# py-lidbox/lidbox

Hardware: AMD Instinct MI355X
Metric: utterances/sec (16kHz x 2s) log-mel + x-vector train step (higher is better)
Workload: dtype f32; 1 GPU; log-mel + x-vector 4-lang train step, bs=256 per GPU, fp32 (BASELINE configs[1]); reference_model=lidbox.models.xvector, global_batch=256, per_gpu_batch=256, samples_per_utt=32000, frames=198, mel=40, languages=4, optimizer=Adam(1e-3, eps=1e-7), parallelism=dp1, grad_buckets=1, grad_sync=none, hip_graph=True, resident_batches=4, feature_prefetch=False

## Files before the change

### include/lidbox_hip.h

```cpp
#ifndef LIDBOX_HIP_H
#define LIDBOX_HIP_H

#include <stddef.h>
#include <stdint.h>

#ifdef __cplusplus
extern "C" {
#endif

#define LIDBOX_HIP_ABI_VERSION 1

#define LIDBOX_OK            0
#define LIDBOX_E_INVALID    -1
#define LIDBOX_E_LAUNCH     -2
#define LIDBOX_E_ALLOC      -3

typedef void* lidbox_stream_t;
typedef struct lidbox_feat_plan lidbox_feat_plan;

int         lidbox_hip_abi_version(void);
const char* lidbox_hip_last_error(void);


int lidbox_ms_to_frames(int sample_rate, int ms);
// ... 6 lines not shown
int lidbox_hann_window(int window_length, float* out_host);


enum {
    LIDBOX_FEAT_SPECTROGRAM = 0,
    LIDBOX_FEAT_MEL         = 1,
    LIDBOX_FEAT_LOGMEL      = 2,
    LIDBOX_FEAT_MFCC        = 3
};

int  lidbox_feat_plan_create(int sample_rate, int frame_length, int frame_step, int fft_length,
                             float power, int num_mel_bins, float fmin, float fmax,
                             int coef_begin, int coef_end, lidbox_feat_plan** out_plan);
void lidbox_feat_plan_destroy(lidbox_feat_plan* plan);

int  lidbox_feat_plan_channels(const lidbox_feat_plan* plan, int kind);
int  lidbox_feat_plan_is_fused(const lidbox_feat_plan* plan, int kind, const float* signals,
                               long sig_stride);
size_t lidbox_extract_features_workspace(const lidbox_feat_plan* plan, int kind, int B, int N,
                                         const float* signals, long sig_stride);

int lidbox_extract_features_fwd(const lidbox_feat_plan* plan, int kind, const float* signals,
                                int B, int N, long sig_stride, float* out, long out_batch_stride,
                                void* workspace, size_t workspace_bytes, lidbox_stream_t stream);
int lidbox_extract_features_fwd_shadow(const lidbox_feat_plan* plan, int kind, const float* signals,
                                       int B, int N, long sig_stride, float* out, long out_batch_stride, void* out16,
                                       void* workspace, size_t workspace_bytes, lidbox_stream_t stream);

enum { LIDBOX_SRC_F32 = 0, LIDBOX_SRC_PCM16 = 1 };
int lidbox_extract_features_fwd_ex(const lidbox_feat_plan* plan, int kind, const void* signals, int src_format,
                                   int B, int N, long sig_stride, float* out, long out_batch_stride, void* out16,
                                   int* nonfinite, void* workspace, size_t workspace_bytes, lidbox_stream_t stream);
int lidbox_extract_features_fwd_pcm16(const lidbox_feat_plan* plan, int kind, const int16_t* pcm, int B, int N, long sig_stride,
                                      float* out, long out_batch_stride, int* nonfinite, lidbox_stream_t stream);


int lidbox_cmvn_fwd(const float* x, long outer, long R, long inner, int normalize_variance,
                    float* out, lidbox_stream_t stream);
int lidbox_cmvn_strided_fwd(const float* x, long outer, long R, long inner, long x_outer_stride,
                            int normalize_variance, float* out, long out_outer_stride, lidbox_stream_t stream);

int lidbox_window_norm_fwd(const float* x, int B, int T, int C, int window_len,
                           int normalize_variance, float* out, lidbox_stream_t stream);

int lidbox_minmax(const float* x, long n, float* out2, float* scratch, lidbox_stream_t stream);

int lidbox_feature_scaling_fwd(const float* x, long n, const float* minmax2, float lo, float hi,
                               float* out, lidbox_stream_t stream);
int lidbox_feature_scaling_axis_fwd(const float* x, long outer, long R, long inner, float lo, float hi, float* out,
                                    lidbox_stream_t stream);
int lidbox_log10_fwd(const float* x, long n, float* out, lidbox_stream_t stream);

int lidbox_power_to_db_fwd(const float* S, long n, const float* minmax2, float amin, float top_db,
                           float* out, lidbox_stream_t stream);


typedef struct {
    const float* base;
    long  batch_stride;
    long  row_stride;
    int   batch;
    int   rows_per_batch;
} lidbox_rows_t;

typedef struct {
    float* base;
    long  batch_stride;
    long  row_stride;
    int   batch;
    int   rows_per_batch;
} lidbox_rows_out_t;

enum {
    LIDBOX_EPI_NONE      = 0,
    LIDBOX_EPI_BIAS      = 1,
    LIDBOX_EPI_BIAS_RELU = 2,
    LIDBOX_EPI_RELU_MASK = 3,
    LIDBOX_EPI_ACCUM     = 4,
    LIDBOX_EPI_ACCUM_RELU_MASK = 5,
    LIDBOX_EPI_ACCUM_RELU = 6,
    LIDBOX_EPI_RELU      = 7,
    LIDBOX_EPI_MASK_BF16 = 0x100
};

int lidbox_gemm_plan_query(int kind, long M, int N, int K, size_t workspace_bytes, int* out4);

int lidbox_gemm_plan_waves(int kind, long M, int N, int K, size_t workspace_bytes);

int lidbox_gemm_plan_is_stream_k(int kind, long M, int N, int K, size_t workspace_bytes);

int lidbox_gemm_last_launches(int* out3);
int lidbox_gemm_last_family(void);
int lidbox_gemm_plan_stream_tail(int kind, long M, int N, int K, size_t workspace_bytes);

size_t lidbox_gemm_rows_workspace(long M, int N, int K);

int lidbox_gemm_nn(lidbox_rows_t A, const float* Bm, long ldb, lidbox_rows_out_t C,
                   int K, int N, int epilogue, const float* aux,
                   void* workspace, size_t workspace_bytes, lidbox_stream_t stream);

int lidbox_gemm_nt(lidbox_rows_t A, const float* Bm, long ldb, lidbox_rows_out_t C,
                   int K, int N, int epilogue, const float* aux,
                   void* workspace, size_t workspace_bytes, lidbox_stream_t stream);

size_t lidbox_gemm_tn_workspace(int M, int K1, int N);
int lidbox_gemm_tn(lidbox_rows_t A, lidbox_rows_t Bm, float* C, long ldc, int K1, int N,
                   int accumulate, float* bias_grad, void* workspace, size_t workspace_bytes,
                   lidbox_stream_t stream);

typedef struct lidbox_reduce_job {
    const float* partials;
    const float* bias_partials;
    float* C;
    float* bias_grad;
    long n, ldc;
    int splits, N, accumulate;
    unsigned nblocks;
} lidbox_reduce_job_t;
int lidbox_gemm_tn_partial(lidbox_rows_t A, lidbox_rows_t Bm, float* C, long ldc, int K1, int N, int accumulate,
                           float* bias_grad, void* workspace, size_t workspace_bytes, lidbox_reduce_job_t* job,
                           lidbox_stream_t stream);
int lidbox_gemm_nt_carry(lidbox_rows_t A, const float* Bm, long ldb, lidbox_rows_out_t C, int K, int N, int epilogue,
                         const float* aux, void* workspace, size_t workspace_bytes, const lidbox_reduce_job_t* jobs, int njobs,
                         lidbox_stream_t stream);
int lidbox_gemm_nt_tn_carry(lidbox_rows_t dY, const float* W, long ldb, lidbox_rows_out_t dX, int Co, int N, int epilogue,
                            const float* aux, void* ws_nt, size_t ws_nt_bytes, lidbox_rows_t X, float* dW, long ldc, int K1,
                            int accumulate, float* bias_grad, void* ws_tn, size_t ws_tn_bytes,
                            const lidbox_reduce_job_t* jobs, int njobs, lidbox_reduce_job_t* job_out, lidbox_stream_t stream);
int lidbox_reduce_jobs_run(const lidbox_reduce_job_t* jobs, int njobs, lidbox_stream_t stream);
int lidbox_gemm_last_carried(void);
int lidbox_zero_job(float* base, long batch_stride, long row_floats, int batch, lidbox_reduce_job_t* job);

int lidbox_gemm_plan_is_pair(long M, int Co, int N, int K1, size_t ws_nt_bytes, size_t ws_tn_bytes);
int lidbox_gemm_nt_tn(lidbox_rows_t dY, const float* W, long ldb, lidbox_rows_out_t dX, int Co, int N, int epilogue,
                      const float* aux, void* ws_nt, size_t ws_nt_bytes, lidbox_rows_t X, float* dW, long ldc, int K1,
                      int accumulate, float* bias_grad, void* ws_tn, size_t ws_tn_bytes, lidbox_stream_t stream);

size_t lidbox_gemm_bf16_rows_workspace(long M, int N, int K);
int lidbox_gemm_bf16_nn(lidbox_rows_t A, const float* Bm, long ldb, lidbox_rows_out_t C,
                        int K, int N, int epilogue, const float* aux,
                        void* workspace, size_t workspace_bytes, lidbox_stream_t stream);
int lidbox_gemm_bf16_nt(lidbox_rows_t A, const float* Bm, long ldb, lidbox_rows_out_t C,
                        int K, int N, int epilogue, const float* aux,
                        void* workspace, size_t workspace_bytes, lidbox_stream_t stream);
size_t lidbox_gemm_bf16_tn_workspace(int M, int K1, int N);
int lidbox_gemm_bf16_tn(lidbox_rows_t A, lidbox_rows_t Bm, float* C, long ldc, int K1, int N,
                        int accumulate, float* bias_grad, void* workspace, size_t workspace_bytes,
                        lidbox_stream_t stream);

int lidbox_gemm_bf16s_nt(lidbox_rows_t A16, const void* B16, long ldb, lidbox_rows_out_t C, void* C16,
                         int K, int N, int epilogue, const float* aux,
                         void* workspace, size_t workspace_bytes, lidbox_stream_t stream);
int lidbox_gemm_bf16s_last_variant(int* out3);
size_t lidbox_gemm_bf16s_tn_workspace(int M, int K1, int N);
int lidbox_gemm_bf16s_tn(lidbox_rows_t A16, lidbox_rows_t B16, float* C, long ldc, int K1, int N,
                         int accumulate, float* bias_grad, void* workspace, size_t workspace_bytes,
                         lidbox_stream_t stream);
int lidbox_gemm_bf16s_tn_partial(lidbox_rows_t A16, lidbox_rows_t B16, float* C, long ldc, int K1, int N, int accumulate,
                                 float* bias_grad, void* workspace, size_t workspace_bytes, lidbox_reduce_job_t* job,
                                 lidbox_stream_t stream);
int lidbox_gemm_bf16s_nt_carry(lidbox_rows_t A16, const void* B16, long ldb, lidbox_rows_out_t C, void* C16, int K, int N,
                               int epilogue, const float* aux, void* workspace, size_t workspace_bytes,
                               const lidbox_reduce_job_t* jobs, int njobs, lidbox_stream_t stream);
int lidbox_gemm_bf16s_last_carried(void);
int lidbox_gemm_bf16s_nt_pair_carry(lidbox_rows_t A16_0, const void* B16_0, long ldb0, lidbox_rows_out_t C0, void* C16_0, int K0, int N0,
                                    int epilogue0, const float* aux0, lidbox_rows_t A16_1, const void* B16_1, long ldb1,
// ... 255 lines not shown
```

### lidbox_amd/_native.py

```python
import ctypes as C
import os

import torch

_HERE = os.path.dirname(os.path.abspath(__file__))
LIB_PATH = os.environ.get("LIDBOX_HIP_LIB") or os.path.join(_HERE, "csrc", "liblidbox_hip.so")

ABI_VERSION = 1

FEAT_SPECTROGRAM, FEAT_MEL, FEAT_LOGMEL, FEAT_MFCC = 0, 1, 2, 3
SRC_F32, SRC_PCM16 = 0, 1
EPI_NONE, EPI_BIAS, EPI_BIAS_RELU, EPI_RELU_MASK, EPI_ACCUM, EPI_ACCUM_RELU_MASK, EPI_ACCUM_RELU, EPI_RELU = range(8)
EPI_MASK_BF16 = 0x100


class LidboxHipError(RuntimeError):
    pass


class Rows(C.Structure):
    _fields_ = [("base", C.c_void_p), ("batch_stride", C.c_long), ("row_stride", C.c_long),
                ("batch", C.c_int), ("rows_per_batch", C.c_int)]


class ReduceJob(C.Structure):
    _fields_ = [("partials", C.c_void_p), ("bias_partials", C.c_void_p), ("C", C.c_void_p), ("bias_grad", C.c_void_p),
                ("n", C.c_long), ("ldc", C.c_long), ("splits", C.c_int), ("N", C.c_int), ("accumulate", C.c_int),
                ("nblocks", C.c_uint)]


class WeightShadow(C.Structure):
    _fields_ = [("offset", C.c_long), ("rows", C.c_int), ("cols", C.c_int), ("dst", C.c_void_p), ("ld_dst", C.c_long),
                ("transpose", C.c_int)]


class Conv2DTaps(C.Structure):
    _fields_ = [("kt", C.c_int), ("kf", C.c_int), ("sf", C.c_int), ("pt0", C.c_int), ("pt1", C.c_int), ("pf0", C.c_int),
                ("pf1", C.c_int), ("time_first", C.c_int)]


def _load():
    if not os.path.exists(LIB_PATH):
        raise LidboxHipError(
            "liblidbox_hip.so not found at %s -- build it with `python -m lidbox_amd.build` "
            "(lidbox_amd has no CPU fallback)" % LIB_PATH)
    try:
        lib = C.CDLL(LIB_PATH)
    except OSError as e:
        raise LidboxHipError("cannot load %s: %s" % (LIB_PATH, e)) from e
    return lib


lib = _load()

_vp, _i, _l, _f, _sz = C.c_void_p, C.c_int, C.c_long, C.c_float, C.c_size_t

_SIGS = {
    "lidbox_hip_abi_version": (_i, []),
    "lidbox_hip_last_error": (C.c_char_p, []),
    "lidbox_ms_to_frames": (_i, [_i, _i]),
    "lidbox_num_frames": (_i, [_i, _i, _i]),
    "lidbox_mel_weight_matrix": (_i, [_i, _i, _i, _f, _f, _vp]),
    "lidbox_hann_window": (_i, [_i, _vp]),
    "lidbox_feat_plan_create": (_i, [_i, _i, _i, _i, _f, _i, _f, _f, _i, _i, C.POINTER(_vp)]),
    "lidbox_feat_plan_destroy": (None, [_vp]),
    "lidbox_feat_plan_channels": (_i, [_vp, _i]),
    "lidbox_feat_plan_is_fused": (_i, [_vp, _i, _vp, _l]),
    "lidbox_extract_features_workspace": (_sz, [_vp, _i, _i, _i, _vp, _l]),
    "lidbox_extract_features_fwd": (_i, [_vp, _i, _vp, _i, _i, _l, _vp, _l, _vp, _sz, _vp]),
    "lidbox_extract_features_fwd_shadow": (_i, [_vp, _i, _vp, _i, _i, _l, _vp, _l, _vp, _vp, _sz, _vp]),
    "lidbox_extract_features_fwd_ex": (_i, [_vp, _i, _vp, _i, _i, _i, _l, _vp, _l, _vp, _vp, _vp, _sz, _vp]),
    "lidbox_extract_features_fwd_pcm16": (_i, [_vp, _i, _vp, _i, _i, _l, _vp, _l, _vp, _vp]),
    "lidbox_cmvn_fwd": (_i, [_vp, _l, _l, _l, _i, _vp, _vp]),
    "lidbox_cmvn_strided_fwd": (_i, [_vp, _l, _l, _l, _l, _i, _vp, _l, _vp]),
    "lidbox_window_norm_fwd": (_i, [_vp, _i, _i, _i, _i, _i, _vp, _vp]),
    "lidbox_minmax": (_i, [_vp, _l, _vp, _vp, _vp]),
    "lidbox_feature_scaling_fwd": (_i, [_vp, _l, _vp, _f, _f, _vp, _vp]),
    "lidbox_feature_scaling_axis_fwd": (_i, [_vp, _l, _l, _l, _f, _f, _vp, _vp]),
    "lidbox_log10_fwd": (_i, [_vp, _l, _vp, _vp]),
    "lidbox_power_to_db_fwd": (_i, [_vp, _l, _vp, _f, _f, _vp, _vp]),
    "lidbox_gemm_plan_query": (_i, [_i, _l, _i, _i, _sz, _vp]),
    "lidbox_gemm_last_launches": (_i, [_vp]),
    "lidbox_gemm_last_family": (_i, []),
    "lidbox_gemm_bf16s_last_variant": (_i, [_vp]),
    "lidbox_gemm_plan_stream_tail": (_i, [_l, _i, _i, _i, _sz]),
    "lidbox_gemm_plan_waves": (_i, [_i, _l, _i, _i, _sz]),
    "lidbox_gemm_plan_is_stream_k": (_i, [_i, _l, _i, _i, _sz]),
    "lidbox_gemm_rows_workspace": (_sz, [_l, _i, _i]),
    "lidbox_gemm_nn": (_i, [Rows, _vp, _l, Rows, _i, _i, _i, _vp, _vp, _sz, _vp]),
    "lidbox_gemm_nt": (_i, [Rows, _vp, _l, Rows, _i, _i, _i, _vp, _vp, _sz, _vp]),
    "lidbox_gemm_tn_workspace": (_sz, [_i, _i, _i]),
    "lidbox_gemm_tn": (_i, [Rows, Rows, _vp, _l, _i, _i, _i, _vp, _vp, _sz, _vp]),
    "lidbox_gemm_plan_is_pair": (_i, [_l, _i, _i, _i, _sz, _sz]),
    "lidbox_gemm_nt_tn": (_i, [Rows, _vp, _l, Rows, _i, _i, _i, _vp, _vp, _sz, Rows, _vp, _l, _i, _i, _vp, _vp, _sz, _vp]),
    "lidbox_gemm_tn_partial": (_i, [Rows, Rows, _vp, _l, _i, _i, _i, _vp, _vp, _sz, C.POINTER(ReduceJob), _vp]),
    "lidbox_gemm_nt_carry": (_i, [Rows, _vp, _l, Rows, _i, _i, _i, _vp, _vp, _sz, C.POINTER(ReduceJob), _i, _vp]),
# ... 166 lines not shown
```

### lidbox_amd/csrc/gemm.hip

```cpp
#include <stdlib.h>

#include <atomic>

#include "gemm_shared.h"
#include "gemm_sk.h"
#include <string.h>
#include "gemm_dma.h"
#include "gemm_dma8.h"
#include "gemm_tuned.h"

namespace {

constexpr int BK = 16;
#define LBX_ROWS_BOUNDS(BM, BN) __launch_bounds__(256, ((BM) * (BN) >= 16384 ? 3 : ((BM) * (BN) >= 8192 ? 6 : 8)))
#define LBX_TN_BOUNDS(BM, BN) __launch_bounds__(256, ((BM) * (BN) >= 16384 ? 3 : 1))

template <int ROWS, bool ALIGNED, int NT = 256>
struct KInnerLoader {
    static constexpr int F4R = BK / 4;
    static constexpr int RPP = NT / F4R;
    static constexpr int PASSES = ROWS >= RPP ? ROWS / RPP : 1;
    static constexpr bool PARTIAL = ROWS < RPP;
    static constexpr int LD = ROWS + 8 / F4R;
    float4 v[PASSES];
// ... 546 lines not shown
    if (wgs > NUM_CU && wgs % NUM_CU != 0) {
        const double fluid = (double)wgs / NUM_CU + 0.12;
        if (fluid < per_cu) per_cu = fluid;
    }
    const double conc = per_cu < RESIDENT[c] ? (double)wgs / NUM_CU : (double)RESIDENT[c];
    return per_cu * tile_t / conc_eff(conc < 1.0 ? 1.0 : conc);
}

RowsChoice choose_rows(int kind, long M, int N, int K, size_t ws_bytes) {
    if (const TunedGemm* t = tuned_gemm(kind, M, N, K)) {
        const int kps = (int)(lbx_cdiv(lbx_cdiv(K, t->splits), BK) * BK);
        const int splits = (int)lbx_cdiv(K, kps);
        if (splits == 1 || (size_t)splits * M * N * sizeof(float) <= ws_bytes)
            return RowsChoice{t->bm, t->bn, splits, kps, t->no_tail_split != 0, (t->waves == 8 && t->bm == 128) ? 8 : 4};
    }
    RowsChoice best{128, 128, 1, K};
    double best_cost = 1e30;
    for (int c = 0; c < 4; ++c) {
        const int bm = CAND[c][0], bn = CAND[c][1];
        const long tiles = lbx_cdiv(M, bm) * lbx_cdiv(N, bn);
        for (int s = 1; s <= 64; s *= 2) {
            int kps = (int)(lbx_cdiv(lbx_cdiv(K, s), BK) * BK);
            const int splits = (int)lbx_cdiv(K, kps);
            if (s > 1 && (splits < 2 || kps < 4 * BK)) break;
            if (splits > 1 && (size_t)splits * M * N * sizeof(float) > ws_bytes) break;
            double cost = launch_cost(c, tiles * splits, (double)kps / BK);
            if (splits > 1) cost += 5.0 + (double)M * N * 4.0 * (splits + 1) / 3.0e6;
            if (cost < best_cost) { best_cost = cost; best = RowsChoice{bm, bn, splits, kps}; }
            if (splits < s) break;
        }
    }
    return best;
}

RowsChoice choose_rows_env(int kind, long M, int N, int K, size_t wsb) {
    RowsChoice ch = choose_rows(kind, M, N, K, wsb);
    if (M >= 4096) {
        if (const char* f = getenv(kind == 1 ? "LIDBOX_GEMM_NT8" : "LIDBOX_GEMM_NN8")) {
            const int bn = atoi(f);
            if (bn == 64 || bn == 128) return RowsChoice{128, bn, 1, K, false, 8};
        }
    }
    if (const char* f = getenv("LIDBOX_GEMM_PLAN")) {
        int bm = 0, bn = 0, sp = 0, wv = 4;
        if (sscanf(f, "%d,%d,%d,%d", &bm, &bn, &sp, &wv) >= 3 && (bm == 64 || bm == 128) && (bn == 64 || bn == 128) && sp >= 1) {
            const int kps = (int)(lbx_cdiv(lbx_cdiv(K, sp), BK) * BK);
            const int splits = (int)lbx_cdiv(K, kps);
            if (splits == 1 || (size_t)splits * M * N * sizeof(float) <= wsb)
                ch = RowsChoice{bm, bn, splits, kps, false, (wv == 8 && bm == 128) ? 8 : 4};
        }
    }
    return ch;
}

template <int BM, int BN, bool B_KINNER>
void launch_rows8_t(bool al, dim3 grid, hipStream_t st, RowsD Ad, const float* Bm, long ldb, RowsOutD Co, float* P,
                    long m_beg, long m_end, int K, int N, int epi, const float* aux, int tiles_n, unsigned ntiles, int kps) {
    if (al)
        hipLaunchKernelGGL((gemm_rows8_kernel<BM, BN, B_KINNER, true>), grid, dim3(512), 0, st, Ad, Bm, ldb, Co, P, m_beg,
                           m_end, K, N, epi, aux, tiles_n, ntiles, kps);
    else
        hipLaunchKernelGGL((gemm_rows8_kernel<BM, BN, B_KINNER, false>), grid, dim3(512), 0, st, Ad, Bm, ldb, Co, P, m_beg,
                           m_end, K, N, epi, aux, tiles_n, ntiles, kps);
}

template <int BM, int BN, bool B_KINNER>
void launch_rows_t(bool al, dim3 grid, hipStream_t st, RowsD Ad, const float* Bm, long ldb, RowsOutD Co, float* P,
                   long m_beg, long m_end, int K, int N, int epi, const float* aux, int tiles_n, unsigned ntiles, int kps) {
    if (al)
        hipLaunchKernelGGL((gemm_rows_kernel<BM, BN, B_KINNER, true>), grid, dim3(256), 0, st, Ad, Bm, ldb, Co, P, m_beg,
                           m_end, K, N, epi, aux, tiles_n, ntiles, kps);
    else
        hipLaunchKernelGGL((gemm_rows_kernel<BM, BN, B_KINNER, false>), grid, dim3(256), 0, st, Ad, Bm, ldb, Co, P, m_beg,
                           m_end, K, N, epi, aux, tiles_n, ntiles, kps);
}

inline int dma_mode() {
    if (const char* e = getenv("LIDBOX_GEMM_DMA")) return atoi(e);
    return 1;
}

template <int BM, int BN, bool B_KINNER>
void launch_rows_dma_t(dim3 grid, hipStream_t st, RowsD Ad, const float* Bm, long ldb, RowsOutD Co, float* P, long m_beg, long m_end,
                       int K, int N, int epi, const float* aux, int tiles_n, unsigned ntiles, int kps, const DmaStream& sp, const ReduceJobs& rj) {
    hipLaunchKernelGGL((gemm_rows_dma_kernel<BM, BN, B_KINNER>), grid, dim3(256), 0, st, Ad, Bm, ldb, Co, P, m_beg, m_end, K, N, epi,
                       aux, tiles_n, ntiles, kps, sp, rj);
}

inline long carry_cap() {
    if (const char* e = getenv("LIDBOX_GEMM_CARRY_BLOCKS")) { const long v = atol(e); if (v >= 8) return v; }
    return 96;
}
struct Carry {
    const ReduceJob* jobs = nullptr;
    int njobs = 0;
    bool carried = false;
};

constexpr int DMA_STREAM_MIN_STEPS = 8;
constexpr int DMA_STREAM_MAX_G = 8;
struct DmaStreamPlan {
    int g = 0;
    long whole = 0, rem = 0;
    size_t ws_need = 0;
};
inline DmaStreamPlan dma_stream_plan(int bm, int bn, long M, int N, int K) {
    DmaStreamPlan pl;
    int force = -1;
    if (const char* e = getenv("LIDBOX_GEMM_STREAM_TAIL")) force = atoi(e);
    if (force == 0) return pl;
    const long tiles = lbx_cdiv(M, bm) * lbx_cdiv(N, bn);
    const long rem = tiles % NUM_CU;
    if (tiles < NUM_CU || rem == 0) return pl;
    const int nk = (int)lbx_cdiv(K, SK_BK);
    int best = 1;
    double best_cost = 1.0;
    for (int g = 2; g <= DMA_STREAM_MAX_G && nk / g >= DMA_STREAM_MIN_STEPS; ++g) {
        const double cost = (double)lbx_cdiv(rem * g, (long)NUM_CU) / g + 0.03 + 0.01 * g;
        if (cost < best_cost - 1e-9) { best_cost = cost; best = g; }
    }
    if (force > 1 && nk / force >= 2 && force <= 64) best = force;
    else if (best_cost > 0.9) return pl;
    if (best < 2) return pl;
    pl.g = best; pl.rem = rem; pl.whole = tiles - rem;
    pl.ws_need = SK_COUNTER_BYTES + (size_t)rem * best * bm * bn * sizeof(float);
    return pl;
}

template <bool B_KINNER>
int launch_rows_range(const RowsChoice& ch, bool al, RowsD Ad, const float* Bm, long ldb, RowsOutD Co, long m_beg,
                      long m_end, int K, int N, int epi, const float* aux, float* P, hipStream_t st, bool dma_ok = false,
                      const DmaStreamPlan* stream = nullptr, void* ws = nullptr, Carry* carry = nullptr) {
    const long Msub = m_end - m_beg;
    if (Msub <= 0) return LIDBOX_OK;
    const int tiles_n = (int)lbx_cdiv(N, ch.bn);
    const long ntiles = lbx_cdiv(Msub, ch.bm) * tiles_n;
    dim3 grid((unsigned)ntiles, (unsigned)ch.splits);
    if (g_last_launches[0] == 0) { g_first_tile[0] = ch.bm; g_first_tile[1] = ch.bn; }
    ++g_last_launches[(ch.bm == g_first_tile[0] && ch.bn == g_first_tile[1]) ? 0 : 1];
    if (ch.splits > 1) ++g_last_launches[2];
#define LBX_ROWS(BM_, BN_) launch_rows_t<BM_, BN_, B_KINNER>(al, grid, st, Ad, Bm, ldb, Co, P, m_beg, m_end, K, N, epi, aux, tiles_n, (unsigned)ntiles, ch.k_per_split)
#define LBX_ROWS8(BM_, BN_) launch_rows8_t<BM_, BN_, B_KINNER>(al, grid, st, Ad, Bm, ldb, Co, P, m_beg, m_end, K, N, epi, aux, tiles_n, (unsigned)ntiles, ch.k_per_split)
#define LBX_ROWS_DMA(BM_, BN_) launch_rows_dma_t<BM_, BN_, B_KINNER>(grid, st, Ad, Bm, ldb, Co, P, m_beg, m_end, K, N, epi, aux, tiles_n, ntiles_k, ch.k_per_split, sp, rj)
    if (dma_ok && al && dma_mode() != 0) {
        g_last_family = 1;
        DmaStream sp;
        const bool dma8 = ch.waves == 8 && ch.bm == 128;
        ReduceJobs rj;
        if (carry && !carry->carried && carry->njobs > 0) {
            rj = pack_carry(carry->jobs, carry->njobs, carry_cap());
            carry->carried = rj.total > 0;
        }
        unsigned ntiles_k = (unsigned)ntiles;
        if (stream && stream->g > 1 && ch.splits == 1) {
            sp.pieces = (unsigned)(stream->rem * stream->g);
            sp.npad = (sp.pieces + 7u) & ~7u;
            sp.g = stream->g;
            sp.first_tile = (unsigned)stream->whole;
            sp.epoch = sk_next_epoch();
            sp.counters = (unsigned*)ws;
            sp.slabs = (float*)((char*)ws + SK_COUNTER_BYTES);
            ntiles_k = (unsigned)stream->whole;
            grid.x = sp.npad + ntiles_k;
        }
        grid.x += rj.total;
        if (dma8) {
            g_last_family = 3;
            if (ch.bn == 128)
                hipLaunchKernelGGL((gemm_rows_dma8_kernel<128, B_KINNER>), grid, dim3(512), 0, st, Ad, Bm, ldb, Co, P, m_beg, m_end, K, N, epi, aux, tiles_n,
                                   ntiles_k, ch.k_per_split, sp, rj);
            else
                hipLaunchKernelGGL((gemm_rows_dma8_kernel<64, B_KINNER>), grid, dim3(512), 0, st, Ad, Bm, ldb, Co, P, m_beg, m_end, K, N, epi, aux, tiles_n,
                                   ntiles_k, ch.k_per_split, sp, rj);
        } else
        if (ch.bm == 128 && ch.bn == 128) LBX_ROWS_DMA(128, 128);
        else if (ch.bm == 128) LBX_ROWS_DMA(128, 64);
        else if (ch.bn == 128) LBX_ROWS_DMA(64, 128);
        else LBX_ROWS_DMA(64, 64);
    } else
    if (ch.waves == 8 && ch.bm == 128 && ch.bn == 128) LBX_ROWS8(128, 128);
    else if (ch.waves == 8 && ch.bm == 128 && ch.bn == 64) LBX_ROWS8(128, 64);
    else if (ch.bm == 128 && ch.bn == 128) LBX_ROWS(128, 128);
    else if (ch.bm == 128) LBX_ROWS(128, 64);
    else if (ch.bn == 128) LBX_ROWS(64, 128);
    else LBX_ROWS(64, 64);
#undef LBX_ROWS
#undef LBX_ROWS8
    LBX_LAUNCH_OK();
    if (ch.splits > 1) {
        long g = lbx_cdiv(Msub * N, 256);
        if (g > 2048) g = 2048;
        hipLaunchKernelGGL(rows_reduce_kernel, dim3((unsigned)g), dim3(256), 0, st, (const float*)P, ch.splits, m_beg,
                           Msub, N, Co, epi, aux);
        LBX_LAUNCH_OK();
    }
    return LIDBOX_OK;
}

inline int cand_index(int bm, int bn) { return bm == 128 ? (bn == 128 ? 0 : 1) : (bn == 128 ? 2 : 3); }

template <bool B_KINNER>
int launch_rows(lidbox_rows_t A, const float* Bm, long ldb, lidbox_rows_out_t Cd, int K, int N, int epi,
                const float* aux, void* ws, size_t ws_bytes, hipStream_t st, Carry* carry = nullptr) {
    const long M = (long)A.batch * A.rows_per_batch;
    g_last_launches[0] = g_last_launches[1] = g_last_launches[2] = 0;
    g_last_family = 0;
    if (M == 0 || N == 0) return LIDBOX_OK;
    const size_t wsb = ws ? ws_bytes : 0;
    const RowsChoice ch = choose_rows_env(B_KINNER ? 1 : 0, M, N, K, wsb);
    const bool al = rows_aligned(A) && K % 4 == 0 && aligned16(Bm) && ldb % 4 == 0 &&
                    (B_KINNER ? true : N % 4 == 0);
    RowsD Ad = to_dev(A);
    RowsOutD Co{Cd.base, Cd.batch_stride, Cd.row_stride, Cd.batch, Cd.rows_per_batch};
    float* P = (float*)ws;

    if (al && !getenv("LIDBOX_GEMM_PLAN") && aligned16(ws) && !sk_tuned_out(B_KINNER ? 1 : 0, M, N, K) &&
        sk_b_extent_ok(B_KINNER, K, N, ldb)) {
        const bool has_mask_ = epi == LIDBOX_EPI_RELU_MASK || epi == LIDBOX_EPI_ACCUM_RELU_MASK;
        const bool skp_ok = skp_mode() != 0 && (Cd.batch == 1 || Cd.rows_per_batch >= 32) && N % 4 == 0 && aligned16(Cd.base) &&
                            Cd.row_stride % 4 == 0 && (Cd.batch == 1 || Cd.batch_stride % 4 == 0) && (!has_mask_ || aligned16(aux)) &&
                            skp_policy(B_KINNER ? 1 : 0, M, N, K);
        if (skp_ok) {
            const SkRows sk = sk_rows_plan(B_KINNER ? 1 : 0, M, N, K, true);
            if (sk.ok && wsb >= sk.ws_need && sk_extent_ok(A, K)) {
                sk_set_lds_attr();
                g_last_launches[0] = 1;
                g_last_family = 2;
                g_first_tile[0] = SK_BM; g_first_tile[1] = SK_BN;
                unsigned* counters = (unsigned*)ws;
                float* slabs = (float*)((char*)ws + SK_COUNTER_BYTES);
                float* dummy = slabs + (size_t)sk.P * 2 * SK_SLAB;
                const bool has_mask = epi == LIDBOX_EPI_RELU_MASK || epi == LIDBOX_EPI_ACCUM_RELU_MASK;
                const bool accum = epi == LIDBOX_EPI_ACCUM || epi == LIDBOX_EPI_ACCUM_RELU_MASK || epi == LIDBOX_EPI_ACCUM_RELU;
                const unsigned ep = sk_next_epoch();
#define LBX_SKP(MASK_, ACC_)                                                                                                \
    hipLaunchKernelGGL((gemm_skp_rows_kernel<B_KINNER, MASK_, ACC_>), dim3(sk.P), dim3(256), (MASK_ || ACC_) ? SKP_LDS_BYTES : SK_LDS_BYTES, st, Ad, Bm, ldb, Co, M, K, \
                       N, epi, aux, sk.pl, ep, counters, slabs, dummy)
                if (has_mask && accum) LBX_SKP(true, true);
                else if (has_mask) LBX_SKP(true, false);
                else if (accum) LBX_SKP(false, true);
                else LBX_SKP(false, false);
#undef LBX_SKP
                LBX_LAUNCH_OK();
                return LIDBOX_OK;
            }
        }
        const SkRows sk = sk_rows_plan(B_KINNER ? 1 : 0, M, N, K);
        if (sk.ok && wsb >= sk.ws_need && sk_extent_ok(A, K)) {
            sk_set_lds_attr();
            g_last_launches[0] = 1;
            g_last_family = 2;
            g_first_tile[0] = SK_BM; g_first_tile[1] = SK_BN;
            unsigned* counters = (unsigned*)ws;
            float* slabs = (float*)((char*)ws + SK_COUNTER_BYTES);
            hipLaunchKernelGGL((gemm_sk_rows_kernel<B_KINNER>), dim3(sk.P), dim3(256), SK_LDS_BYTES, st, Ad, Bm, ldb, Co, M, K, N, epi,
                               aux, sk.pl, sk_next_epoch(), counters, slabs);
            LBX_LAUNCH_OK();
            return LIDBOX_OK;
        }
    }

    const bool dma_ok = al && sk_extent_ok(A, K) && sk_b_extent_ok(B_KINNER, K, N, ldb);
    if (dma_ok && dma_mode() != 0 && ch.splits == 1 && aligned16(ws)) {
        const DmaStreamPlan spl = dma_stream_plan(ch.bm, ch.bn, M, N, K);
        if (spl.g > 1 && wsb >= spl.ws_need)
            return launch_rows_range<B_KINNER>(ch, al, Ad, Bm, ldb, Co, 0, M, K, N, epi, aux, P, st, dma_ok, &spl, ws, carry);
    }
    const bool no_tail_split = ch.no_tail_split || getenv("LIDBOX_GEMM_NO_TAIL_SPLIT") != nullptr;
    if (!no_tail_split && ch.splits == 1) {
        const int tiles_n = (int)lbx_cdiv(N, ch.bn);
        const long tiles_m = lbx_cdiv(M, ch.bm);
        const long wgs = tiles_m * tiles_n;
        const long rounds = wgs / NUM_CU;
        if (rounds >= 1 && wgs % NUM_CU != 0) {
            const long main_tiles_m = rounds * NUM_CU / tiles_n;
            const long m_main = main_tiles_m * ch.bm;
            const long m_rem = M - m_main;
            if (main_tiles_m >= 1 && m_rem > 0) {
                const RowsChoice rem = choose_rows(B_KINNER ? 1 : 0, m_rem, N, K, wsb);
                const int c = cand_index(ch.bm, ch.bn), cr = cand_index(rem.bm, rem.bn);
                const double ksteps = (double)lbx_cdiv(K, BK);
                const double whole = launch_cost(c, wgs, ksteps);
                double split = launch_cost(c, main_tiles_m * tiles_n, ksteps) + 4.0 +
                               launch_cost(cr, lbx_cdiv(m_rem, rem.bm) * lbx_cdiv(N, rem.bn) * rem.splits,
                                           (double)rem.k_per_split / BK);
                if (rem.splits > 1) split += 5.0 + (double)m_rem * N * 4.0 * (rem.splits + 1) / 3.0e6;
                if (split < 0.97 * whole) {
                    int rc = launch_rows_range<B_KINNER>(ch, al, Ad, Bm, ldb, Co, 0, m_main, K, N, epi, aux, P, st, dma_ok, nullptr, nullptr, carry);
                    if (rc) return rc;
                    return launch_rows_range<B_KINNER>(rem, al, Ad, Bm, ldb, Co, m_main, M, K, N, epi, aux, P, st, dma_ok);
                }
            }
        }
    }
    return launch_rows_range<B_KINNER>(ch, al, Ad, Bm, ldb, Co, 0, M, K, N, epi, aux, P, st, dma_ok, nullptr, nullptr, carry);
}

struct TnPlan {
    int bm, bn, splits;
    long rows_per_split;
};

TnPlan tn_plan(long M, int K1, int N) {
    if (const char* f = getenv("LIDBOX_GEMM_TN_PLAN")) {
        int bm = 0, bn = 0;
        long sp = 0;
        if (sscanf(f, "%d,%d,%ld", &bm, &bn, &sp) == 3 && (bm == 64 || bm == 128) && (bn == 64 || bn == 128) && sp >= 1) {
            const long rps = lbx_cdiv(lbx_cdiv(M, sp), BK) * BK;
            return TnPlan{bm, bn, (int)lbx_cdiv(M, rps), rps};
        }
    }
    if (const TunedGemm* t = tuned_gemm(2, M, N, K1)) {
        const long rps = lbx_cdiv(lbx_cdiv(M, (long)t->splits), BK) * BK;
        return TnPlan{t->bm, t->bn, (int)lbx_cdiv(M, rps), rps};
    }
    TnPlan best{128, 128, 1, M};
    double best_cost = 1e30;
    for (int c = 0; c < 4; ++c) {
        const int bm = CAND[c][0], bn = CAND[c][1];
        const long tiles = lbx_cdiv(K1, bm) * lbx_cdiv(N, bn);
        for (long target = NUM_CU; target <= 8 * NUM_CU; target += NUM_CU / 2) {
            long s = target / tiles;
            if (s < 1) s = 1;
            const long max_s = lbx_cdiv(M, 4 * BK);
            if (s > max_s) s = max_s;
            if (s < 1) s = 1;
            long rps = lbx_cdiv(lbx_cdiv(M, s), BK) * BK;
            s = lbx_cdiv(M, rps);
            double cost = launch_cost(c, tiles * s, (double)rps / BK);
            cost += 5.0 + (double)K1 * N * 4.0 * (s + 1) / 3.0e6;
            if (cost < best_cost) { best_cost = cost; best = TnPlan{bm, bn, (int)s, rps}; }
        }
    }
    return best;
}

template <int BM, int BN>
void launch_tn_t(bool al, unsigned grid, hipStream_t st, RowsD A, RowsD Bd, float* P, float* Pc, long M, int K1, int N,
                 int tiles_n, int ntiles, long rps) {
    if (al)
        hipLaunchKernelGGL((gemm_tn_kernel<BM, BN, true>), dim3(grid), dim3(256), 0, st, A, Bd, P, Pc, M, K1, N, tiles_n,
                           ntiles, rps);
    else
        hipLaunchKernelGGL((gemm_tn_kernel<BM, BN, false>), dim3(grid), dim3(256), 0, st, A, Bd, P, Pc, M, K1, N, tiles_n,
                           ntiles, rps);
}

}

extern "C" int lidbox_gemm_plan_query(int kind, long M, int N, int K, size_t workspace_bytes, int* out4) {
    LBX_ARG(out4 && M > 0 && N > 0 && K > 0 && kind >= 0 && kind <= 2, "kind in {0 nn, 1 nt, 2 tn}, positive sizes");
    if (kind == 2) {
        const TnPlan pl = tn_plan(M, K, N);
        out4[0] = pl.bm; out4[1] = pl.bn; out4[2] = pl.splits; out4[3] = (int)pl.rows_per_split;
    } else {
        const RowsChoice ch = choose_rows_env(kind, M, N, K, workspace_bytes);
        out4[0] = ch.bm; out4[1] = ch.bn; out4[2] = ch.splits; out4[3] = ch.k_per_split;
    }
    return LIDBOX_OK;
}

extern "C" int lidbox_gemm_plan_is_stream_k(int kind, long M, int N, int K, size_t workspace_bytes) {
    if (M <= 0 || N <= 0 || K <= 0 || kind < 0 || kind > 2) return 0;
    if (kind == 2) {
        const SkTn t = sk_tn_plan(M, K, N);
        return t.ok && workspace_bytes >= t.ws_need && !sk_tuned_out(2, M, N, K);
    }
    {
        const SkRows r = sk_rows_plan(kind, M, N, K);
        return r.ok && workspace_bytes >= r.ws_need && (kind == 1 || N % 4 == 0) && !sk_tuned_out(kind, M, N, K);
    }
    return LIDBOX_OK;
}

extern "C" int lidbox_gemm_plan_waves(int kind, long M, int N, int K, size_t workspace_bytes) {
    if (M <= 0 || N <= 0 || K <= 0 || kind < 0 || kind > 1) return 4;
    return choose_rows_env(kind, M, N, K, workspace_bytes).waves;
}

extern "C" int lidbox_gemm_last_family(void) { return g_last_family; }

extern "C" int lidbox_gemm_plan_stream_tail(int kind, long M, int N, int K, size_t workspace_bytes) {
    if (M <= 0 || N <= 0 || K <= 0 || kind < 0 || kind > 1 || dma_mode() == 0) return 0;
    if (!getenv("LIDBOX_GEMM_PLAN") && lidbox_gemm_plan_is_stream_k(kind, M, N, K, workspace_bytes)) return 0;
    const RowsChoice ch = choose_rows_env(kind, M, N, K, workspace_bytes);
    if (ch.splits != 1) return 0;
    const DmaStreamPlan spl = dma_stream_plan(ch.bm, ch.bn, M, N, K);
    return (spl.g > 1 && workspace_bytes >= spl.ws_need) ? spl.g : 0;
}

extern "C" int lidbox_gemm_last_launches(int* out3) {
    LBX_ARG(out3, "out3 != NULL");
    out3[0] = g_last_launches[0]; out3[1] = g_last_launches[1]; out3[2] = g_last_launches[2];
    return LIDBOX_OK;
}

extern "C" size_t lidbox_gemm_rows_workspace(long M, int N, int K) {
    if (M <= 0 || N <= 0 || K <= 0) return 0;
    size_t need = 0;
    for (int kind = 0; kind < 2; ++kind) {
        const RowsChoice ch = choose_rows(kind, M, N, K, (size_t)64 << 20);
        if (ch.splits > 1 && (size_t)ch.splits * M * N * sizeof(float) > need) need = (size_t)ch.splits * M * N * sizeof(float);
    }
    for (int bm = 64; bm <= 128; bm += 64)
        for (int bn = 64; bn <= 128; bn += 64) {
            const DmaStreamPlan spl = dma_stream_plan(bm, bn, M, N, K);
            if (spl.g > 1 && spl.ws_need > need) need = spl.ws_need;
        }
    for (int kind = 0; kind < 2; ++kind) {
        const SkRows sk = sk_rows_plan(kind, M, N, K);
        if (sk.ok && sk.ws_need > need) need = sk.ws_need;
        if (skp_mode() != 0 && skp_policy(kind, M, N, K)) {
            const SkRows skp = sk_rows_plan(kind, M, N, K, true);
            if (skp.ok && skp.ws_need > need) need = skp.ws_need;
        }
    }
    return need;
}

extern "C" int lidbox_gemm_nn(lidbox_rows_t A, const float* Bm, long ldb, lidbox_rows_out_t C, int K, int N,
                              int epilogue, const float* aux, void* workspace, size_t workspace_bytes,
                              lidbox_stream_t stream) {
    if (validate_rows_call(__func__, A, Bm, ldb, C, K, N, epilogue, aux, N)) return LIDBOX_E_INVALID;
    return launch_rows<false>(A, Bm, ldb, C, K, N, epilogue, aux, workspace, workspace_bytes, (hipStream_t)stream);
}


extern "C" int lidbox_gemm_nt(lidbox_rows_t A, const float* Bm, long ldb, lidbox_rows_out_t C, int K, int N,
                              int epilogue, const float* aux, void* workspace, size_t workspace_bytes,
                              lidbox_stream_t stream) {
    if (validate_rows_call(__func__, A, Bm, ldb, C, K, N, epilogue, aux, K)) return LIDBOX_E_INVALID;
    return launch_rows<true>(A, Bm, ldb, C, K, N, epilogue, aux, workspace, workspace_bytes, (hipStream_t)stream);
}

extern "C" size_t lidbox_gemm_tn_workspace(int M, int K1, int N) {
    if (M <= 0 || K1 <= 0 || N <= 0) return 0;
    const TnPlan pl = tn_plan(M, K1, N);
    size_t need = ((size_t)pl.splits * K1 * N + (size_t)pl.splits * N) * sizeof(float);
    const SkTn sk = sk_tn_plan(M, K1, N);
    if (sk.ok && sk.ws_need > need) need = sk.ws_need;
    return need;
}

namespace {

int tn_partial_launch(const char* fn, lidbox_rows_t A, lidbox_rows_t Bd, float* Cm, long ldc, int K1, int N, int accumulate,
                      float* bias_grad, void* workspace, size_t workspace_bytes, hipStream_t st, ReduceJob* job) {
    *job = ReduceJob{};
    if (check_rows(fn, A.base, A.batch_stride, A.row_stride, A.batch, A.rows_per_batch)) return LIDBOX_E_INVALID;
    if (check_rows(fn, Bd.base, Bd.batch_stride, Bd.row_stride, Bd.batch, Bd.rows_per_batch)) return LIDBOX_E_INVALID;
    LBX_ARG(Cm && K1 >= 1 && N >= 1 && ldc >= N, "C != NULL, K1, N >= 1, ldc >= N");
    const long M = (long)A.batch * A.rows_per_batch;
    LBX_ARG(M == (long)Bd.batch * Bd.rows_per_batch, "A and B row counts differ");
    LBX_ARG(M >= 1, "M >= 1");
    auto finish = [&](const float* P, const float* Pc, int splits) {
        const long n = (long)K1 * N;
        if (reduce_job_vec_ok(P, Pc, splits, n, N, Cm, ldc, bias_grad)) *job = make_reduce_job(P, Pc, splits, n, N, Cm, ldc, accumulate, bias_grad);
        else launch_splitk_reduce(P, Pc, splits, n, N, Cm, ldc, accumulate, bias_grad, st);
    };
    {
        const SkTn sk = sk_tn_plan(M, K1, N);
        if (sk.ok && !getenv("LIDBOX_GEMM_TN_PLAN") && !sk_tuned_out(2, M, N, K1) && workspace && aligned16(workspace) && workspace_bytes >= sk.ws_need &&
            rows_aligned(A) && rows_aligned(Bd) && sk_extent_ok(A, K1) && sk_extent_ok(Bd, N)) {
            sk_set_lds_attr();
            g_last_launches[0] = 1; g_last_launches[1] = 0; g_last_launches[2] = 1;
            g_last_family = 2;
            float* P = (float*)workspace;
            float* Pc = bias_grad ? P + (size_t)sk.splits * K1 * N : nullptr;
            hipLaunchKernelGGL(gemm_sk_tn_kernel, dim3((unsigned)(sk.ntiles * sk.splits)), dim3(256), SK_LDS_BYTES, st, to_dev(A),
                               to_dev(Bd), P, Pc, M, K1, N, sk.tiles_n, sk.ntiles, sk.rows_per_split);
            LBX_LAUNCH_OK();
            finish(P, Pc, sk.splits);
            LBX_LAUNCH_OK();
            return LIDBOX_OK;
        }
    }
    const TnPlan pl = tn_plan(M, K1, N);
    const size_t need = ((size_t)pl.splits * K1 * N + (size_t)pl.splits * N) * sizeof(float);
    LBX_ARG(workspace && workspace_bytes >= need, "workspace too small (lidbox_gemm_tn_workspace)");
    g_last_launches[0] = 1; g_last_launches[1] = 0; g_last_launches[2] = 1;
    g_last_family = 0;
    const int tiles_n = (int)lbx_cdiv(N, pl.bn);
    const int ntiles = (int)(lbx_cdiv(K1, pl.bm) * tiles_n);
    const bool al = rows_aligned(A) && rows_aligned(Bd) && K1 % 4 == 0 && N % 4 == 0;
    float* P = (float*)workspace;
    float* Pc = bias_grad ? P + (size_t)pl.splits * K1 * N : nullptr;
    const unsigned grid = (unsigned)(ntiles * pl.splits);
    if (al && dma_mode() != 0 && sk_extent_ok(A, K1) && sk_extent_ok(Bd, N) && pl.rows_per_split % SK_BK == 0) {
        g_last_family = 1;
#define LBX_TN_DMA(BM_, BN_) hipLaunchKernelGGL((gemm_tn_dma_kernel<BM_, BN_>), dim3(grid), dim3(256), 0, st, to_dev(A), to_dev(Bd), P, Pc, M, K1, N, tiles_n, ntiles, pl.rows_per_split)
        if (pl.bm == 128 && pl.bn == 128) LBX_TN_DMA(128, 128);
        else if (pl.bm == 128) LBX_TN_DMA(128, 64);
        else if (pl.bn == 128) LBX_TN_DMA(64, 128);
        else LBX_TN_DMA(64, 64);
#undef LBX_TN_DMA
        LBX_LAUNCH_OK();
        finish(P, Pc, pl.splits);
        LBX_LAUNCH_OK();
        return LIDBOX_OK;
    }
#define LBX_TN(BM_, BN_) launch_tn_t<BM_, BN_>(al, grid, st, to_dev(A), to_dev(Bd), P, Pc, M, K1, N, tiles_n, ntiles, pl.rows_per_split)
    if (pl.bm == 128 && pl.bn == 128) LBX_TN(128, 128);
    else if (pl.bm == 128) LBX_TN(128, 64);
    else if (pl.bn == 128) LBX_TN(64, 128);
    else LBX_TN(64, 64);
#undef LBX_TN
    LBX_LAUNCH_OK();
    finish(P, Pc, pl.splits);
    LBX_LAUNCH_OK();
    return LIDBOX_OK;
}

static_assert(sizeof(lidbox_reduce_job_t) == sizeof(ReduceJob), "lidbox_reduce_job_t mirrors ReduceJob");
inline ReduceJob job_in(const lidbox_reduce_job_t* j) {
    ReduceJob r;
    if (j) memcpy(&r, j, sizeof r);
    return r;
}
inline int jobs_in(const lidbox_reduce_job_t* jobs, int njobs, ReduceJob (&out)[MAX_CARRY]) {
    int m = 0;
    for (int i = 0; jobs && i < njobs; ++i) {
        if (jobs[i].nblocks == 0) continue;
        if (m == MAX_CARRY) return -1;
        out[m++] = job_in(jobs + i);
    }
    return m;
}

int run_reduce_jobs(const ReduceJob* jobs, int njobs, hipStream_t st) {
    ReduceJobs js;
    for (int i = 0, m = 0; i < njobs && m < MAX_CARRY; ++i) {
        if (jobs[i].nblocks == 0) continue;
        js.j[m++] = jobs[i];
        js.total += jobs[i].nblocks;
    }
    if (js.total == 0) return LIDBOX_OK;
    hipLaunchKernelGGL(splitk_reduce4_kernel, dim3(js.total), dim3(256), 0, st, js);
    LBX_LAUNCH_OK();
    return LIDBOX_OK;
}

}

extern "C" int lidbox_gemm_tn(lidbox_rows_t A, lidbox_rows_t Bd, float* Cm, long ldc, int K1, int N,
                              int accumulate, float* bias_grad, void* workspace, size_t workspace_bytes,
                              lidbox_stream_t stream) {
    ReduceJob job;
    int rc = tn_partial_launch(__func__, A, Bd, Cm, ldc, K1, N, accumulate, bias_grad, workspace, workspace_bytes, (hipStream_t)stream, &job);
    if (rc) return rc;
    return run_reduce_jobs(&job, 1, (hipStream_t)stream);
}

extern "C" int lidbox_gemm_tn_partial(lidbox_rows_t A, lidbox_rows_t Bd, float* Cm, long ldc, int K1, int N, int accumulate,
                                      float* bias_grad, void* workspace, size_t workspace_bytes, lidbox_reduce_job_t* job,
                                      lidbox_stream_t stream) {
    LBX_ARG(job, "job != NULL");
    ReduceJob j;
    int rc = tn_partial_launch(__func__, A, Bd, Cm, ldc, K1, N, accumulate, bias_grad, workspace, workspace_bytes, (hipStream_t)stream, &j);
    memcpy(job, &j, sizeof j);
    return rc;
}

extern "C" int lidbox_zero_job(float* base, long batch_stride, long row_floats, int batch, lidbox_reduce_job_t* job) {
    LBX_ARG(job && base && batch >= 1 && row_floats >= 4 && batch_stride >= row_floats, "base, job != NULL; batch >= 1; row_floats >= 4");
    LBX_ARG(aligned16(base) && row_floats % 4 == 0 && batch_stride % 4 == 0 && row_floats <= 0x7fffffffL,
            "16-byte aligned base, row_floats and batch_stride multiples of 4");
    ReduceJob j;
    j.Cm = base; j.n = (long)batch * row_floats; j.N = (int)row_floats; j.ldc = batch_stride; j.splits = 0; j.accumulate = 0;
    long g = lbx_cdiv(j.n / 4, 256);
    if (g > 2048) g = 2048;
    j.nblocks = (unsigned)g;
    memcpy(job, &j, sizeof j);
    return LIDBOX_OK;
}

extern "C" int lidbox_reduce_jobs_run(const lidbox_reduce_job_t* jobs, int njobs, lidbox_stream_t stream) {
    LBX_ARG(njobs >= 0 && (jobs || njobs == 0), "jobs != NULL");
    ReduceJob js[MAX_CARRY];
    const int m = jobs_in(jobs, njobs, js);
    LBX_ARG(m >= 0, "at most 2 non-empty jobs per call");
    return run_reduce_jobs(js, m, (hipStream_t)stream);
}

extern "C" int lidbox_gemm_nt_carry(lidbox_rows_t A, const float* Bm, long ldb, lidbox_rows_out_t C, int K, int N, int epilogue,
                                    const float* aux, void* workspace, size_t workspace_bytes, const lidbox_reduce_job_t* jobs,
                                    int njobs, lidbox_stream_t stream) {
    if (validate_rows_call(__func__, A, Bm, ldb, C, K, N, epilogue, aux, K)) return LIDBOX_E_INVALID;
    ReduceJob js[MAX_CARRY];
    const int m = jobs_in(jobs, njobs, js);
    LBX_ARG(m >= 0, "at most 2 non-empty jobs per call");
    for (int i = 0; i < m; ++i) LBX_ARG(js[i].splits >= 0, "an optimizer-prepare job runs through lidbox_reduce_jobs_run only");
    for (int i = 0; i < m; ++i) LBX_ARG((const void*)js[i].P != workspace, "a job's slices live in this call's workspace");
    Carry carry;
    carry.jobs = js;
    carry.njobs = (m > 0 && getenv("LIDBOX_GEMM_NO_CARRY") == nullptr) ? m : 0;
    int rc = launch_rows<true>(A, Bm, ldb, C, K, N, epilogue, aux, workspace, workspace_bytes, (hipStream_t)stream, &carry);
    if (rc) return rc;
    g_last_carried = carry.carried ? m : 0;
    if (!carry.carried) return run_reduce_jobs(js, m, (hipStream_t)stream);
    return LIDBOX_OK;
}

extern "C" int lidbox_gemm_last_carried(void) { return g_last_carried; }

inline long pair_max_blocks() {
    if (const char* e = getenv("LIDBOX_GEMM_PAIR_MAX_BLOCKS")) return atol(e);
    return 12L * NUM_CU;
}

bool pair_plan(long M, int Co, int N, int K1, size_t ws_nt_bytes, size_t ws_tn_bytes, RowsChoice* ch_out, TnPlan* pl_out) {
    if (dma_mode() == 0 || getenv("LIDBOX_GEMM_NO_PAIR") != nullptr || M < 1 || N < 1 || K1 < 1 || Co < 1) return false;
    if (Co % 4 != 0 || K1 % 4 != 0) return false;
    const RowsChoice ch = choose_rows_env(1, M, N, Co, ws_nt_bytes);
    const TnPlan pl = tn_plan(M, K1, Co);
    const SkTn sk = sk_tn_plan(M, K1, Co);
    const bool sk_rows = !getenv("LIDBOX_GEMM_PLAN") && lidbox_gemm_plan_is_stream_k(1, M, N, Co, ws_nt_bytes);
    const bool sk_tn = sk.ok && !getenv("LIDBOX_GEMM_TN_PLAN") && !sk_tuned_out(2, M, Co, K1) && ws_tn_bytes >= sk.ws_need;
    const size_t tn_need = ((size_t)pl.splits * K1 * Co + (size_t)pl.splits * Co) * sizeof(float);
    const long rows_blocks = lbx_cdiv(M, 64L) * lbx_cdiv((long)N, 64L) * ch.splits;
    const long tn_blocks = lbx_cdiv((long)K1, 64L) * lbx_cdiv((long)Co, 64L) * pl.splits;
    if (!(ch.bm == 64 && ch.bn == 64 && ch.waves == 4 && pl.bm == 64 && pl.bn == 64 && !sk_rows && !sk_tn && ws_tn_bytes >= tn_need &&
          (ch.splits == 1 || (size_t)ch.splits * M * N * sizeof(float) <= ws_nt_bytes) && rows_blocks + tn_blocks <= pair_max_blocks()))
        return false;
    if (ch_out) *ch_out = ch;
    if (pl_out) *pl_out = pl;
    return true;
}

extern "C" int lidbox_gemm_nt_tn_carry(lidbox_rows_t dY, const float* W, long ldb, lidbox_rows_out_t dX, int Co, int N, int epilogue,
                                       const float* aux, void* ws_nt, size_t ws_nt_bytes, lidbox_rows_t X, float* dW, long ldc, int K1,
                                       int accumulate, float* bias_grad, void* ws_tn, size_t ws_tn_bytes,
                                       const lidbox_reduce_job_t* jobs, int njobs, lidbox_reduce_job_t* job_out, lidbox_stream_t stream) {
    hipStream_t st = (hipStream_t)stream;
    if (job_out) memset(job_out, 0, sizeof *job_out);
    ReduceJob pend[MAX_CARRY];
    const int npend = jobs_in(jobs, njobs, pend);
    LBX_ARG(npend >= 0 && npend < MAX_CARRY, "at most 1 non-empty pending job per call");
    for (int i = 0; i < npend; ++i)
        LBX_ARG((const void*)pend[i].P != ws_nt && (const void*)pend[i].P != ws_tn, "a pending job's slices live in this call's workspaces");
    for (int i = 0; i < npend; ++i) LBX_ARG(pend[i].splits >= 0, "an optimizer-prepare job runs through lidbox_reduce_jobs_run only");
    const long M = (long)dY.batch * dY.rows_per_batch;
    bool pair = dma_mode() != 0 && getenv("LIDBOX_GEMM_NO_PAIR") == nullptr && M >= 1 && N >= 1 && K1 >= 1 && Co >= 1 && W && dW && ws_tn &&
                ws_nt != ws_tn;
    if (pair) {
        if (validate_rows_call(__func__, dY, W, ldb, dX, Co, N, epilogue, aux, Co)) return LIDBOX_E_INVALID;
        if (check_rows(__func__, X.base, X.batch_stride, X.row_stride, X.batch, X.rows_per_batch)) return LIDBOX_E_INVALID;
        LBX_ARG((long)X.batch * X.rows_per_batch == M && ldc >= Co, "X and dY row counts differ, or ldc < Co");
    }
    RowsChoice ch{};
    TnPlan pl{};
    if (pair) {
        const size_t wsb = ws_nt ? ws_nt_bytes : 0;
        const bool al_rows = rows_aligned(dY) && aligned16(W) && ldb % 4 == 0 && sk_extent_ok(dY, Co) && sk_b_extent_ok(true, Co, N, ldb) &&
                             aligned16(ws_nt);
        const bool al_tn = rows_aligned(X) && sk_extent_ok(X, K1) && aligned16(ws_tn);
        pair = al_rows && al_tn && pair_plan(M, Co, N, K1, wsb, ws_tn_bytes, &ch, &pl);
    }
    if (!pair) {
        lidbox_reduce_job_t all[MAX_CARRY];
        for (int i = 0; i < npend; ++i) memcpy(&all[i], &pend[i], sizeof(ReduceJob));
        int rc = lidbox_gemm_tn_partial(X, dY, dW, ldc, K1, Co, accumulate, bias_grad, ws_tn, ws_tn_bytes, &all[npend], stream);
        if (rc) return rc;
        if (ws_nt == ws_tn) {
            rc = lidbox_reduce_jobs_run(all, npend + 1, stream);
            if (rc) return rc;
            return lidbox_gemm_nt(dY, W, ldb, dX, Co, N, epilogue, aux, ws_nt, ws_nt_bytes, stream);
        }
        return lidbox_gemm_nt_carry(dY, W, ldb, dX, Co, N, epilogue, aux, ws_nt, ws_nt_bytes, all, npend + 1, stream);
    }
    PairRows r;
    r.A = to_dev(dY); r.Bm = W; r.ldb = ldb;
    r.Cd = RowsOutD{dX.base, dX.batch_stride, dX.row_stride, dX.batch, dX.rows_per_batch};
    r.P = (float*)ws_nt; r.M = M; r.K = Co; r.N = N; r.epi = epilogue; r.aux = aux;
    r.tiles_n = (int)lbx_cdiv((long)N, 64L);
    r.ntiles = (unsigned)(lbx_cdiv(M, 64L) * r.tiles_n);
    r.k_per_split = ch.k_per_split; r.nx = r.ntiles; r.partial = ch.splits > 1 ? 1 : 0;
    if (ch.splits == 1 && ws_nt) {
        const DmaStreamPlan spl = dma_stream_plan(64, 64, M, N, Co);
        if (spl.g > 1 && ws_nt_bytes >= spl.ws_need) {
            r.sp.pieces = (unsigned)(spl.rem * spl.g);
            r.sp.npad = (r.sp.pieces + 7u) & ~7u;
            r.sp.g = spl.g;
            r.sp.first_tile = (unsigned)spl.whole;
            r.sp.epoch = sk_next_epoch();
            r.sp.counters = (unsigned*)ws_nt;
            r.sp.slabs = (float*)((char*)ws_nt + SK_COUNTER_BYTES);
            r.ntiles = (unsigned)spl.whole;
            r.nx = r.sp.npad + r.ntiles;
        }
    }
    PairTn t;
    t.A = to_dev(X); t.Bd = to_dev(dY);
    t.P = (float*)ws_tn; t.Pc = bias_grad ? t.P + (size_t)pl.splits * K1 * Co : nullptr;
    t.M = M; t.K1 = K1; t.N = Co; t.tiles_n = (int)lbx_cdiv((long)Co, 64L);
    t.ntiles = (int)(lbx_cdiv((long)K1, 64L) * t.tiles_n);
    t.rows_per_split = pl.rows_per_split;
    const unsigned rows_blocks = r.nx * (unsigned)ch.splits;
    ReduceJobs rj;
    if (npend > 0 && getenv("LIDBOX_GEMM_NO_CARRY") == nullptr) rj = pack_carry(pend, npend, carry_cap());
    const unsigned grid = rj.total + rows_blocks + (unsigned)(t.ntiles * pl.splits);
    g_last_launches[0] = 1; g_last_launches[1] = 0; g_last_launches[2] = (job_out ? 0 : 1) + (ch.splits > 1 ? 1 : 0);
    g_last_family = 1;
    g_last_carried = rj.total > 0 ? npend : 0;
    hipLaunchKernelGGL(gemm_nt_tn_pair_kernel, dim3(grid), dim3(256), 0, st, r, t, rows_blocks, rj);
    LBX_LAUNCH_OK();
    if (npend > 0 && rj.total == 0) {
        int rc = run_reduce_jobs(pend, npend, st);
        if (rc) return rc;
    }
    if (ch.splits > 1) {
        long g = lbx_cdiv(M * N, 256);
        if (g > 2048) g = 2048;
        hipLaunchKernelGGL(rows_reduce_kernel, dim3((unsigned)g), dim3(256), 0, st, (const float*)r.P, ch.splits, 0L, M, N, r.Cd, epilogue,
                           aux);
        LBX_LAUNCH_OK();
    }
    if (job_out && reduce_job_vec_ok(t.P, t.Pc, pl.splits, (long)K1 * Co, Co, dW, ldc, bias_grad)) {
// ... 47 lines not shown
```

### lidbox_amd/csrc/gemm_dma.h

```cpp
#pragma once

#include "gemm_sk.h"

namespace {

constexpr int DMA_STAGES = 3;

template <int ROWS>
struct DmaInner {
    static constexpr int PW = ROWS / 64;
    const float* sb;
    unsigned vo[PW];
    int rd;
    __device__ __forceinline__ void init(const float* base, const long (&roff)[PW], int k0, int lane, int wsub) {
        sb = sk_uniform(base + k0);
        const int chunk = (lane & 3) ^ ((lane >> 4) & 3);
#pragma unroll
        for (int i = 0; i < PW; ++i) vo[i] = (unsigned)((roff[i] + chunk * 4) * 4);
        rd = (wsub * (ROWS / 2) + (lane & 31)) * 16;
    }
    __device__ __forceinline__ void issue(int i, unsigned dst) const { sk_dma_s(sb, vo[i], dst); }
    __device__ __forceinline__ void issue_tail(int i, unsigned dst, int kvalid, int lane) const {
        const int chunk = (lane & 3) ^ ((lane >> 4) & 3);
        const float* p = reinterpret_cast<const float*>(reinterpret_cast<const char*>(sb) + vo[i]);
// ... 21 lines not shown
    long step;
    int rd;
    __device__ __forceinline__ void init(const float* base, long ld, int col0, int ncols, int k0, int lane, int wv, int wsub) {
        sb = sk_uniform(base + (long)k0 * ld + col0);
        int c = (lane % LPR) * 4;
        if (col0 + c >= ncols) c = 0;
#pragma unroll
        for (int i = 0; i < PW; ++i) vo[i] = (unsigned)(((long)(RPP * (wv * PW + i) + lane / LPR) * ld + c) * 4);
        step = (long)SK_BK * ld;
        rd = (4 * (lane >> 5)) * COLS + wsub * (COLS / 2) + (lane & 31);
    }
    __device__ __forceinline__ void issue(int i, unsigned dst) const { sk_dma_s(sb, vo[i], dst); }
    __device__ __forceinline__ void issue_tail(int i, unsigned dst, int kvalid, int lane, int wv) const {
        const float* p = reinterpret_cast<const float*>(reinterpret_cast<const char*>(sb) + vo[i]);
        sk_dma_f(RPP * (wv * PW + i) + lane / LPR < kvalid ? p : g_sk_zero, dst);
    }
    __device__ __forceinline__ void advance() { sb += step; }
    template <int NB>
    __device__ __forceinline__ void read(const float* st, int lane, int s2, float (&v)[NB][4]) const {
#pragma unroll
        for (int b = 0; b < NB; ++b)
#pragma unroll
            for (int j = 0; j < 4; ++j) v[b][j] = st[rd + (8 * s2 + j) * COLS + b * 32];
    }
};

template <int MI, int NJ, int J0, int J1>
__device__ __forceinline__ void dma_mma(const float (&a)[MI][4], const float (&b)[NJ][4], f32x16 (&acc)[MI][NJ]) {
#pragma unroll
    for (int j = J0; j < J1; ++j)
#pragma unroll
        for (int bi = 0; bi < MI; ++bi)
#pragma unroll
            for (int bj = 0; bj < NJ; ++bj)
                acc[bi][bj] = __builtin_amdgcn_mfma_f32_32x32x2f32(a[bi][j], b[bj][j], acc[bi][bj], 0, 0, 0);
}

struct DmaStream {
    unsigned npad = 0;
    unsigned pieces = 0;
    int g = 1;
    unsigned first_tile = 0;
    unsigned epoch = 0;
    unsigned* counters = nullptr;
    float* slabs = nullptr;
};

template <int MI, int NJ>
__device__ __forceinline__ void dma_slab_store(float* slab, const f32x16 (&acc)[MI][NJ], int wv, int lane) {
    const __amdgpu_buffer_rsrc_t r = __builtin_amdgcn_make_buffer_rsrc(const_cast<float*>(sk_uniform(slab)), 0, MI * NJ * 4096 * 4, 0x00020000);
#pragma unroll
    for (int bi = 0; bi < MI; ++bi)
#pragma unroll
        for (int bj = 0; bj < NJ; ++bj)
#pragma unroll
            for (int r4 = 0; r4 < 4; ++r4) {
                const f32x4_t x = {acc[bi][bj][4 * r4], acc[bi][bj][4 * r4 + 1], acc[bi][bj][4 * r4 + 2], acc[bi][bj][4 * r4 + 3]};
                __builtin_amdgcn_raw_buffer_store_b128(__builtin_bit_cast(u32x4_t, x), r,
                                                       ((((wv * (MI * NJ) + bi * NJ + bj) * 4 + r4) * 64 + lane) * 4) * 4, 0,  16);
            }
}
template <int MI, int NJ>
__device__ __forceinline__ void dma_slab_add(const float* slab, f32x16 (&acc)[MI][NJ], int wv, int lane) {
    const __amdgpu_buffer_rsrc_t r = __builtin_amdgcn_make_buffer_rsrc(const_cast<float*>(sk_uniform(slab)), 0, MI * NJ * 4096 * 4, 0x00020000);
#pragma unroll
    for (int bi = 0; bi < MI; ++bi)
#pragma unroll
        for (int bj = 0; bj < NJ; ++bj) {
#pragma unroll
            for (int r4 = 0; r4 < 4; ++r4) {
                const f32x4_t x = __builtin_bit_cast(
                    f32x4_t, __builtin_amdgcn_raw_buffer_load_b128(r, ((((wv * (MI * NJ) + bi * NJ + bj) * 4 + r4) * 64 + lane) * 4) * 4, 0,  16));
#pragma unroll
                for (int j = 0; j < 4; ++j) acc[bi][bj][4 * r4 + j] += x[j];
            }
            __builtin_amdgcn_sched_barrier(0);
        }
}

template <int BM, int BN, bool B_KINNER>
__device__ __forceinline__ void rows_dma_body(const RowsD& A, const float* __restrict__ Bm, long ldb, const RowsOutD& Cd, float* __restrict__ P,
                                              long m_beg, long M, int K, int N, int epi, const float* __restrict__ aux, int tiles_n,
                                              unsigned ntiles, int k_per_split, const DmaStream& sp, unsigned bx, unsigned by, int partial,
                                              float* smem) {
    constexpr int MI = BM / 64, NJ = BN / 64;
    constexpr int A_ST = BM * SK_BK, B_ST = SK_BK * BN, ST = A_ST + B_ST;
    constexpr int PA = BM / 64, PB = BN / 64;

    const int tid = threadIdx.x, lane = tid & 63;
    const int wv = __builtin_amdgcn_readfirstlane(tid >> 6);
    const int wm = wv >> 1, wn = wv & 1;
    const unsigned lds0 = __builtin_amdgcn_readfirstlane((unsigned)(size_t)(__attribute__((address_space(3))) void*)smem);
    const int split = (int)by;
    unsigned chunk;
    int kbeg, kend, part = -1;
    unsigned rem_t = 0;
    if (bx < sp.npad) {
        if (bx >= sp.pieces) return;
        rem_t = bx / (unsigned)sp.g;
        part = (int)(bx - rem_t * (unsigned)sp.g);
        chunk = sp.first_tile + rem_t;
        const int nk = (K + SK_BK - 1) / SK_BK;
        kbeg = (part * nk / sp.g) * SK_BK;
        kend = min(K, ((part + 1) * nk / sp.g) * SK_BK);
    } else {
        chunk = xcd_chunk_id(bx - sp.npad, ntiles);
        kbeg = split * k_per_split;
        kend = min(K, kbeg + k_per_split);
    }
    const int tn = chunk % tiles_n;
    const long m0 = m_beg + (long)(chunk / tiles_n) * BM;
    const int n0 = tn * BN;
    const int n = (kend - kbeg + SK_BK - 1) / SK_BK;
    const int ktail = kend - kbeg - (n - 1) * SK_BK;

    DmaInner<BM> oa;
    {
        long roff[PA];
#pragma unroll
        for (int i = 0; i < PA; ++i) {
            long r = m0 + 16 * (wv * PA + i) + (lane >> 2);
            if (r >= M) r = m0;
            roff[i] = row_offset(A, (unsigned)r);
        }
        oa.init(A.base, roff, kbeg, lane, wm);
    }
    DmaInner<BN> obi;
    DmaOuter<BN> obo;
    if (B_KINNER) {
        long roff[PB];
#pragma unroll
        for (int i = 0; i < PB; ++i) {
            long r = n0 + 16 * (wv * PB + i) + (lane >> 2);
            if (r >= N) r = n0;
            roff[i] = r * ldb;
        }
        obi.init(Bm, roff, kbeg, lane, wn);
    } else {
        obo.init(Bm, ldb, n0, N, kbeg, lane, wv, wn);
    }
    f32x16 acc[MI][NJ];
#pragma unroll
    for (int i = 0; i < MI; ++i)
#pragma unroll
        for (int j = 0; j < NJ; ++j)
#pragma unroll
            for (int r = 0; r < 16; ++r) acc[i][j][r] = 0.f;

    auto issue = [&](int pc, int step, int stage) {
        const bool tail = step == n - 1 && ktail < SK_BK;
        if (pc < PA) {
            const unsigned d = lds0 + (unsigned)((stage * ST + (wv * PA + pc) * 256) * 4);
            if (tail) oa.issue_tail(pc, d, ktail, lane);
            else oa.issue(pc, d);
        } else {
            const int q = pc - PA;
            const unsigned d = lds0 + (unsigned)((stage * ST + A_ST + (wv * PB + q) * 256) * 4);
            if (B_KINNER) { if (tail) obi.issue_tail(q, d, ktail, lane); else obi.issue(q, d); }
            else { if (tail) obo.issue_tail(q, d, ktail, lane, wv); else obo.issue(q, d); }
        }
    };
    auto next = [&]() {
        oa.advance();
        if (B_KINNER) obi.advance();
        else obo.advance();
    };
    auto ra = [&](const float* st, int s2, float (&v)[MI][4]) { oa.template read<MI>(st, lane, s2, v); };
    auto rb = [&](const float* st, int s2, float (&v)[NJ][4]) {
        if (B_KINNER) obi.template read<NJ>(st, lane, s2, v);
        else obo.template read<NJ>(st, lane, s2, v);
    };
    constexpr int NP = PA + PB;
#pragma unroll
    for (int s = 0; s < DMA_STAGES - 1; ++s)
        if (s < n) {
#pragma unroll
            for (int pc = 0; pc < NP; ++pc) issue(pc, s, s);
            next();
        }
    if (n >= DMA_STAGES - 1) sk_wait_vm<(DMA_STAGES - 2) * NP>();
    else sk_wait_vm<0>();
    __builtin_amdgcn_s_barrier();
    float a0[MI][4], b0[NJ][4], a1[MI][4], b1[NJ][4];
    if (n > 0) {
        ra(smem, 0, a0);
        rb(smem + A_ST, 0, b0);
    }
    int cur = 0;
    for (int t = 0; t < n; ++t) {
        if (t + 1 < n) {
            if (DMA_STAGES >= 4 && t + DMA_STAGES - 2 < n) sk_wait_vm<(DMA_STAGES >= 4 ? (DMA_STAGES - 3) * NP : 0)>();
            else sk_wait_vm<0>();
        }
        __builtin_amdgcn_s_barrier();
        int nxt = cur + 1;
        if (nxt == DMA_STAGES) nxt = 0;
        const bool more = t + DMA_STAGES - 1 < n;
        int tgt = cur + DMA_STAGES - 1;
        if (tgt >= DMA_STAGES) tgt -= DMA_STAGES;
        const float* st = smem + cur * ST;
        dma_mma<MI, NJ, 0, 1>(a0, b0, acc);
        __builtin_amdgcn_sched_barrier(0);
        ra(st, 1, a1);
        rb(st + A_ST, 1, b1);
        __builtin_amdgcn_sched_barrier(0);
        dma_mma<MI, NJ, 1, 2>(a0, b0, acc);
        if (more) issue(0, t + DMA_STAGES - 1, tgt);
        __builtin_amdgcn_sched_barrier(0);
        dma_mma<MI, NJ, 2, 3>(a0, b0, acc);
        if (more) issue(1, t + DMA_STAGES - 1, tgt);
        __builtin_amdgcn_sched_barrier(0);
        dma_mma<MI, NJ, 3, 4>(a0, b0, acc);
        if (more && NP > 2) issue(2, t + DMA_STAGES - 1, tgt);
        __builtin_amdgcn_sched_barrier(0);
        dma_mma<MI, NJ, 0, 1>(a1, b1, acc);
        if (more) {
            if (NP > 3) issue(3, t + DMA_STAGES - 1, tgt);
            next();
        }
        __builtin_amdgcn_sched_barrier(0);
        if (t + 1 < n) {
            const float* sn = smem + nxt * ST;
            ra(sn, 0, a0);
            rb(sn + A_ST, 0, b0);
        }
        __builtin_amdgcn_sched_barrier(0);
        dma_mma<MI, NJ, 1, 4>(a1, b1, acc);
        cur = nxt;
    }
    if (part >= 0) {
        constexpr int SLAB = BM * BN;
        dma_slab_store<MI, NJ>(sp.slabs + (size_t)bx * SLAB, acc, wv, lane);
        asm volatile("s_waitcnt vmcnt(0)" ::: "memory");
        __syncthreads();
        unsigned* flag = reinterpret_cast<unsigned*>(smem);
        if (tid == 0) {
            unsigned old = __hip_atomic_load(sp.counters + rem_t, __ATOMIC_RELAXED, __HIP_MEMORY_SCOPE_AGENT);
            unsigned cnt;
            for (;;) {
                cnt = (old >> 8) == sp.epoch ? (old & 255u) : 0u;
                if (__hip_atomic_compare_exchange_strong(sp.counters + rem_t, &old, (sp.epoch << 8) | (cnt + 1u), __ATOMIC_RELAXED,
                                                         __ATOMIC_RELAXED, __HIP_MEMORY_SCOPE_AGENT))
                    break;
            }
            *flag = cnt;
        }
        __syncthreads();
        if (*flag != (unsigned)(sp.g - 1)) return;
#pragma unroll
        for (int i = 0; i < MI; ++i)
#pragma unroll
            for (int j = 0; j < NJ; ++j)
#pragma unroll
                for (int r = 0; r < 16; ++r) acc[i][j][r] = 0.f;
        for (int q = 0; q < sp.g; ++q)
            dma_slab_add<MI, NJ>(sp.slabs + ((size_t)rem_t * sp.g + q) * SLAB, acc, wv, lane);
        if (tid == 0) __hip_atomic_store(sp.counters + rem_t, 0u, __ATOMIC_RELAXED, __HIP_MEMORY_SCOPE_AGENT);
    }
    store_rows_tile<MI, NJ>(acc, m0, n0, wm, wn, lane, m_beg, M, N, epi, aux, Cd, P, split, 0ull, false, nullptr, nullptr, partial);
}

template <int BM, int BN>
constexpr int dma_stage_floats() { return (BM + BN) * SK_BK; }

template <int BM, int BN, bool B_KINNER>
__global__ __launch_bounds__(256, (BM * BN >= 16384 ? 3 : (BM * BN >= 8192 ? 4 : 6))) void gemm_rows_dma_kernel(
    RowsD A, const float* __restrict__ Bm, long ldb, RowsOutD Cd, float* __restrict__ P, long m_beg, long M, int K, int N, int epi,
    const float* __restrict__ aux, int tiles_n, unsigned ntiles, int k_per_split, DmaStream sp, ReduceJobs rj) {
    __shared__ __attribute__((aligned(16))) float smem[DMA_STAGES * dma_stage_floats<BM, BN>()];
    if (blockIdx.x < rj.total) {
        if (blockIdx.y == 0) reduce_jobs_run(rj, blockIdx.x);
        return;
    }
    rows_dma_body<BM, BN, B_KINNER>(A, Bm, ldb, Cd, P, m_beg, M, K, N, epi, aux, tiles_n, ntiles, k_per_split, sp, blockIdx.x - rj.total,
                                    blockIdx.y, gridDim.y > 1 ? 1 : 0, smem);
}

template <int COLS>
struct DmaOuterRows {
    static constexpr int PW = COLS / 64;
    static constexpr int LPR = COLS / 4;
    static constexpr int RPP = 64 / LPR;
    const float* sb;
    int off[PW];
    unsigned tt[PW];
    int a_step, a_wrap;
    unsigned rpb;
    int mleft[PW];
    int rd;

    __device__ __forceinline__ void init(const RowsD& X, int col0, int ncols, long mbeg, long mend, int lane, int wv, int wsub) {
        sb = sk_uniform(X.base + col0);
        int c = (lane % LPR) * 4;
        if (col0 + c >= ncols) c = 0;
        a_step = (int)(SK_BK * X.rs);
        a_wrap = X.batch == 1 ? 0 : (int)(X.bs - (long)X.rpb * X.rs);
        rpb = X.batch == 1 ? 0xffffffffu : (unsigned)X.rpb;
#pragma unroll
        for (int i = 0; i < PW; ++i) {
            const long m = mbeg + RPP * (wv * PW + i) + lane / LPR;
            const unsigned bq = X.batch == 1 ? 0u : (unsigned)m / rpb;
            tt[i] = (unsigned)m - (X.batch == 1 ? 0u : bq * rpb);
            off[i] = (int)((long)bq * X.bs + (long)tt[i] * X.rs) + c;
            mleft[i] = (int)(mend - m);
        }
        rd = (4 * (lane >> 5)) * COLS + wsub * (COLS / 2) + (lane & 31);
    }
    __device__ __forceinline__ void issue(int i, unsigned dst, bool tail) {
        if (!tail) {
            sk_dma_s(sb, (unsigned)off[i] * 4u, dst);
        } else {
            const float* p = reinterpret_cast<const float*>(reinterpret_cast<const char*>(sb) + (size_t)((unsigned)off[i] * 4u));
            sk_dma_f(mleft[i] > 0 ? p : g_sk_zero, dst);
        }
        mleft[i] -= SK_BK;
        tt[i] += SK_BK;
        off[i] += a_step;
        while (tt[i] >= rpb) { tt[i] -= rpb; off[i] += a_wrap; }
    }
    template <int NB>
    __device__ __forceinline__ void read(const float* st, int lane, int s2, float (&v)[NB][4]) const {
#pragma unroll
        for (int b = 0; b < NB; ++b)
#pragma unroll
            for (int j = 0; j < 4; ++j) v[b][j] = st[rd + (8 * s2 + j) * COLS + b * 32];
    }
};

template <int BM, int BN>
__device__ __forceinline__ void tn_dma_body(const RowsD& A, const RowsD& Bd, float* __restrict__ P, float* __restrict__ Pc, long M, int K1, int N,
                                            int tiles_n, int ntiles, long rows_per_split, unsigned bx, unsigned nblk, float* smem) {
    constexpr int MI = BM / 64, NJ = BN / 64;
    constexpr int A_ST = SK_BK * BM, B_ST = SK_BK * BN, ST = A_ST + B_ST;
    constexpr int PA = BM / 64, PB = BN / 64, NP = PA + PB;

    const int tid = threadIdx.x, lane = tid & 63;
    const int wv = __builtin_amdgcn_readfirstlane(tid >> 6);
    const int wm = wv >> 1, wn = wv & 1;
    const unsigned lds0 = __builtin_amdgcn_readfirstlane((unsigned)(size_t)(__attribute__((address_space(3))) void*)smem);
    const unsigned vb = xcd_chunk_id(bx, nblk);
    const int tile = (int)(vb % (unsigned)ntiles);
    const int split = (int)(vb / (unsigned)ntiles);
    const int tn = tile % tiles_n, tk = tile / tiles_n;
    const int i0 = tk * BM, n0 = tn * BN;
    const long mbeg = (long)split * rows_per_split;
    long mend = mbeg + rows_per_split;
    if (mend > M) mend = M;
    const int n = (int)((mend - mbeg + SK_BK - 1) / SK_BK);
    const int tail_step = ((mend - mbeg) % SK_BK != 0) ? n - 1 : -1;

    DmaOuterRows<BM> oa;
    DmaOuterRows<BN> ob;
    oa.init(A, i0, K1, mbeg, mend, lane, wv, wm);
    ob.init(Bd, n0, N, mbeg, mend, lane, wv, wn);
    f32x16 acc[MI][NJ];
#pragma unroll
    for (int i = 0; i < MI; ++i)
#pragma unroll
// ... 30 lines not shown
        rb(smem + A_ST, 0, b0);
    }
    int cur = 0;
    for (int t = 0; t < n; ++t) {
        if (t + 1 < n) sk_wait_vm<0>();
        __builtin_amdgcn_s_barrier();
        int nxt = cur + 1;
        if (nxt == DMA_STAGES) nxt = 0;
        const bool more = t + DMA_STAGES - 1 < n;
        int tgt = cur + DMA_STAGES - 1;
        if (tgt >= DMA_STAGES) tgt -= DMA_STAGES;
        const float* st = smem + cur * ST;
        dma_mma<MI, NJ, 0, 1>(a0, b0, acc);
        __builtin_amdgcn_sched_barrier(0);
        ra(st, 1, a1);
        rb(st + A_ST, 1, b1);
        __builtin_amdgcn_sched_barrier(0);
        dma_mma<MI, NJ, 1, 2>(a0, b0, acc);
        if (more) issue(0, t + DMA_STAGES - 1, tgt);
        __builtin_amdgcn_sched_barrier(0);
        dma_mma<MI, NJ, 2, 3>(a0, b0, acc);
        if (more) issue(1, t + DMA_STAGES - 1, tgt);
        __builtin_amdgcn_sched_barrier(0);
        dma_mma<MI, NJ, 3, 4>(a0, b0, acc);
        if (more && NP > 2) issue(2, t + DMA_STAGES - 1, tgt);
        __builtin_amdgcn_sched_barrier(0);
        dma_mma<MI, NJ, 0, 1>(a1, b1, acc);
        if (more && NP > 3) issue(3, t + DMA_STAGES - 1, tgt);
        __builtin_amdgcn_sched_barrier(0);
        if (t + 1 < n) {
            const float* sn = smem + nxt * ST;
            ra(sn, 0, a0);
            rb(sn + A_ST, 0, b0);
        }
        __builtin_amdgcn_sched_barrier(0);
        dma_mma<MI, NJ, 1, 4>(a1, b1, acc);
        cur = nxt;
    }
    float* Pd = P + (long)split * K1 * N;
    store_partial_blocks<MI, NJ>(Pd, acc, i0, n0, wm, wn, lane, K1, N);
    if (do_csum && n0 + tid < N) Pc[(long)split * N + n0 + tid] = csum;
}

template <int BM, int BN>
__global__ __launch_bounds__(256, (BM * BN >= 16384 ? 3 : (BM * BN >= 8192 ? 4 : 6))) void gemm_tn_dma_kernel(
    RowsD A, RowsD Bd, float* __restrict__ P, float* __restrict__ Pc, long M, int K1, int N, int tiles_n, int ntiles, long rows_per_split) {
    __shared__ __attribute__((aligned(16))) float smem[DMA_STAGES * dma_stage_floats<BM, BN>()];
    tn_dma_body<BM, BN>(A, Bd, P, Pc, M, K1, N, tiles_n, ntiles, rows_per_split, blockIdx.x, gridDim.x, smem);
}

struct PairRows {
    RowsD A;
    const float* Bm;
    long ldb;
    RowsOutD Cd;
    float* P;
    long M;
    int K, N, epi;
    const float* aux;
    int tiles_n;
    unsigned ntiles;
    int k_per_split;
    unsigned nx;
    int partial;
    DmaStream sp;
};
struct PairTn {
    RowsD A, Bd;
    float* P;
    float* Pc;
    long M;
    int K1, N, tiles_n, ntiles;
    long rows_per_split;
};
__global__ __launch_bounds__(256, 6) void gemm_nt_tn_pair_kernel(PairRows r, PairTn t, unsigned rows_blocks, ReduceJobs rj) {
    __shared__ __attribute__((aligned(16))) float smem[DMA_STAGES * dma_stage_floats<64, 64>()];
    if (blockIdx.x < rj.total) {
        reduce_jobs_run(rj, blockIdx.x);
        return;
    }
    const unsigned bx = blockIdx.x - rj.total, nb = gridDim.x - rj.total;
    if (bx < rows_blocks) {
        rows_dma_body<64, 64, true>(r.A, r.Bm, r.ldb, r.Cd, r.P, 0, r.M, r.K, r.N, r.epi, r.aux, r.tiles_n, r.ntiles, r.k_per_split, r.sp,
                                    bx % r.nx, bx / r.nx, r.partial, smem);
    } else {
        tn_dma_body<64, 64>(t.A, t.Bd, t.P, t.Pc, t.M, t.K1, t.N, t.tiles_n, t.ntiles, t.rows_per_split, bx - rows_blocks, nb - rows_blocks, smem);
    }
}

}
```

### lidbox_amd/csrc/gemm_dma8.h

```cpp
#pragma once

#include "gemm_dma.h"

namespace {

template <int ROWS>
struct DmaInner8 {
    static constexpr int NPIECE = ROWS / 16;
    const float* sb;
    unsigned vo;
    int rd;
    bool mine;
    __device__ __forceinline__ void init(const float* base, long roff, int k0, int lane, int wv, int wsub, int rows_per_wave) {
        sb = sk_uniform(base + k0);
        const int chunk = (lane & 3) ^ ((lane >> 4) & 3);
        vo = (unsigned)((roff + chunk * 4) * 4);
        rd = (wsub * rows_per_wave + (lane & 31)) * 16;
        mine = wv < NPIECE;
    }
    __device__ __forceinline__ void issue(unsigned dst) const { sk_dma_s(sb, vo, dst); }
    __device__ __forceinline__ void issue_tail(unsigned dst, int kvalid, int lane) const {
        const int chunk = (lane & 3) ^ ((lane >> 4) & 3);
        const float* p = reinterpret_cast<const float*>(reinterpret_cast<const char*>(sb) + vo);
        sk_dma_f(chunk * 4 < kvalid ? p : g_sk_zero, dst);
    }
    __device__ __forceinline__ void advance() { sb += SK_BK; }
    template <int NB>
    __device__ __forceinline__ void read(const float* st, int lane, int s2, float (&v)[NB][4]) const {
        const int slot = (2 * s2 + (lane >> 5)) ^ ((lane >> 2) & 3);
#pragma unroll
        for (int b = 0; b < NB; ++b) {
            const f32x4_t x = *reinterpret_cast<const f32x4_t*>(st + rd + b * 32 * 16 + slot * 4);
            v[b][0] = x[0]; v[b][1] = x[1]; v[b][2] = x[2]; v[b][3] = x[3];
        }
    }
};

template <int COLS>
struct DmaOuter8 {
    static constexpr int NPIECE = COLS / 16;
    static constexpr int LPR = COLS / 4;
    static constexpr int RPP = 64 / LPR;
    const float* sb;
    unsigned vo;
    long step;
    int rd;
    int krow;
    bool mine;
    __device__ __forceinline__ void init(const float* base, long ld, int col0, int ncols, int k0, int lane, int wv, int wsub) {
        sb = sk_uniform(base + (long)k0 * ld + col0);
        int c = (lane % LPR) * 4;
        if (col0 + c >= ncols) c = 0;
        const int p = wv % NPIECE;
        krow = RPP * p + lane / LPR;
        vo = (unsigned)(((long)krow * ld + c) * 4);
        step = (long)SK_BK * ld;
        rd = (4 * (lane >> 5)) * COLS + wsub * (COLS / 2) + (lane & 31);
        mine = wv < NPIECE;
    }
    __device__ __forceinline__ void issue(unsigned dst) const { sk_dma_s(sb, vo, dst); }
    __device__ __forceinline__ void issue_tail(unsigned dst, int kvalid, int lane) const {
        const float* p = reinterpret_cast<const float*>(reinterpret_cast<const char*>(sb) + vo);
        sk_dma_f(krow < kvalid ? p : g_sk_zero, dst);
    }
    __device__ __forceinline__ void advance() { sb += step; }
    template <int NB>
    __device__ __forceinline__ void read(const float* st, int lane, int s2, float (&v)[NB][4]) const {
#pragma unroll
        for (int b = 0; b < NB; ++b)
#pragma unroll
            for (int j = 0; j < 4; ++j) v[b][j] = st[rd + (8 * s2 + j) * COLS + b * 32];
    }
};

template <int NJ>
__device__ __forceinline__ void dma8_slab_store(float* slab, const f32x16 (&acc)[1][NJ], int wv, int lane) {
    const __amdgpu_buffer_rsrc_t r = __builtin_amdgcn_make_buffer_rsrc(const_cast<float*>(sk_uniform(slab)), 0, 8 * NJ * 4096, 0x00020000);
#pragma unroll
    for (int bj = 0; bj < NJ; ++bj)
#pragma unroll
        for (int r4 = 0; r4 < 4; ++r4) {
            const f32x4_t x = {acc[0][bj][4 * r4], acc[0][bj][4 * r4 + 1], acc[0][bj][4 * r4 + 2], acc[0][bj][4 * r4 + 3]};
            __builtin_amdgcn_raw_buffer_store_b128(__builtin_bit_cast(u32x4_t, x), r, ((((wv * NJ + bj) * 4 + r4) * 64 + lane) * 4) * 4, 0,  16);
        }
}
template <int NJ>
__device__ __forceinline__ void dma8_slab_add(const float* slab, f32x16 (&acc)[1][NJ], int wv, int lane) {
    const __amdgpu_buffer_rsrc_t r = __builtin_amdgcn_make_buffer_rsrc(const_cast<float*>(sk_uniform(slab)), 0, 8 * NJ * 4096, 0x00020000);
#pragma unroll
    for (int bj = 0; bj < NJ; ++bj) {
#pragma unroll
        for (int r4 = 0; r4 < 4; ++r4) {
            const f32x4_t x =
                __builtin_bit_cast(f32x4_t, __builtin_amdgcn_raw_buffer_load_b128(r, ((((wv * NJ + bj) * 4 + r4) * 64 + lane) * 4) * 4, 0,  16));
#pragma unroll
            for (int j = 0; j < 4; ++j) acc[0][bj][4 * r4 + j] += x[j];
        }
        __builtin_amdgcn_sched_barrier(0);
    }
}

template <int BN, bool B_KINNER>
__global__ __launch_bounds__(512, BN == 64 ? 8 : 4) void gemm_rows_dma8_kernel(RowsD A, const float* __restrict__ Bm, long ldb, RowsOutD Cd,
                                                                              float* __restrict__ P, long m_beg, long M, int K, int N, int epi,
                                                                              const float* __restrict__ aux, int tiles_n, unsigned ntiles,
                                                                              int k_per_split, DmaStream sp, ReduceJobs rj) {
    constexpr int BM = 128, NJ = BN / 64;
    constexpr int A_ST = BM * SK_BK, B_ST = SK_BK * BN, ST = A_ST + B_ST;
    __shared__ __attribute__((aligned(16))) float smem[DMA_STAGES * ST];
    if (blockIdx.x < rj.total) {
        if (blockIdx.y == 0 && threadIdx.x < 256) reduce_jobs_run(rj, blockIdx.x);
        return;
    }
    const unsigned bx = blockIdx.x - rj.total;
    const int tid = threadIdx.x, lane = tid & 63;
    const int wv = __builtin_amdgcn_readfirstlane(tid >> 6);
    const int wm = wv >> 1, wn = wv & 1;
    const unsigned lds0 = __builtin_amdgcn_readfirstlane((unsigned)(size_t)(__attribute__((address_space(3))) void*)smem);
    const int split = (int)blockIdx.y;
    unsigned chunk;
    int kbeg, kend, part = -1;
    unsigned rem_t = 0;
    if (bx < sp.npad) {
        if (bx >= sp.pieces) return;
        rem_t = bx / (unsigned)sp.g;
        part = (int)(bx - rem_t * (unsigned)sp.g);
        chunk = sp.first_tile + rem_t;
        const int nk = (K + SK_BK - 1) / SK_BK;
        kbeg = (part * nk / sp.g) * SK_BK;
        kend = min(K, ((part + 1) * nk / sp.g) * SK_BK);
    } else {
        chunk = xcd_chunk_id(bx - sp.npad, ntiles);
        kbeg = split * k_per_split;
        kend = min(K, kbeg + k_per_split);
    }
    const int tn = chunk % tiles_n;
    const long m0 = m_beg + (long)(chunk / tiles_n) * BM;
    const int n0 = tn * BN;
    const int n = (kend - kbeg + SK_BK - 1) / SK_BK;
    const int ktail = kend - kbeg - (n - 1) * SK_BK;

    DmaInner8<BM> oa;
    {
        long r = m0 + 16 * wv + (lane >> 2);
        if (r >= M) r = m0;
        oa.init(A.base, row_offset(A, (unsigned)r), kbeg, lane, wv, wm, 32);
    }
    DmaInner8<BN> obi;
    DmaOuter8<BN> obo;
    if (B_KINNER) {
        long r = n0 + 16 * (wv % (BN / 16)) + (lane >> 2);
        if (r >= N) r = n0;
        obi.init(Bm, r * ldb, kbeg, lane, wv, wn, 32 * NJ);
    } else {
        obo.init(Bm, ldb, n0, N, kbeg, lane, wv, wn);
    }
    const bool has_b = B_KINNER ? obi.mine : obo.mine;
    f32x16 acc[1][NJ];
#pragma unroll
    for (int j = 0; j < NJ; ++j)
#pragma unroll
        for (int r = 0; r < 16; ++r) acc[0][j][r] = 0.f;

    auto issue_a = [&](int step, int stage) {
        const unsigned d = lds0 + (unsigned)((stage * ST + wv * 256) * 4);
        if (step == n - 1 && ktail < SK_BK) oa.issue_tail(d, ktail, lane);
        else oa.issue(d);
    };
    auto issue_b = [&](int step, int stage) {
        const unsigned d = lds0 + (unsigned)((stage * ST + A_ST + wv * 256) * 4);
        const bool tail = step == n - 1 && ktail < SK_BK;
        if (B_KINNER) { if (tail) obi.issue_tail(d, ktail, lane); else obi.issue(d); }
        else { if (tail) obo.issue_tail(d, ktail, lane); else obo.issue(d); }
    };
    auto adv_b = [&]() { if (B_KINNER) obi.advance(); else obo.advance(); };
    auto rb = [&](const float* stg, int s2, float (&v)[NJ][4]) {
        if (B_KINNER) obi.template read<NJ>(stg, lane, s2, v);
        else obo.template read<NJ>(stg, lane, s2, v);
    };
#pragma unroll
    for (int s = 0; s < DMA_STAGES - 1; ++s)
        if (s < n) {
            issue_a(s, s);
            if (has_b) issue_b(s, s);
            oa.advance();
            adv_b();
        }
    if (n >= DMA_STAGES - 1) {
        if (has_b) sk_wait_vm<(DMA_STAGES - 2) * 2>();
        else sk_wait_vm<(DMA_STAGES - 2) * 1>();
    } else {
        sk_wait_vm<0>();
    }
    __builtin_amdgcn_s_barrier();
    float a0[1][4], b0[NJ][4], a1[1][4], b1[NJ][4];
    if (n > 0) {
        oa.template read<1>(smem, lane, 0, a0);
        rb(smem + A_ST, 0, b0);
    }
    int cur = 0;
    for (int t = 0; t < n; ++t) {
        if (t + 1 < n) sk_wait_vm<0>();
        __builtin_amdgcn_s_barrier();
        int nxt = cur + 1;
        if (nxt == DMA_STAGES) nxt = 0;
        const bool more = t + DMA_STAGES - 1 < n;
        int tgt = cur + DMA_STAGES - 1;
        if (tgt >= DMA_STAGES) tgt -= DMA_STAGES;
        const float* st = smem + cur * ST;
        dma_mma<1, NJ, 0, 1>(a0, b0, acc);
        __builtin_amdgcn_sched_barrier(0);
        oa.template read<1>(st, lane, 1, a1);
        rb(st + A_ST, 1, b1);
        __builtin_amdgcn_sched_barrier(0);
        dma_mma<1, NJ, 1, 2>(a0, b0, acc);
        if (more) issue_a(t + DMA_STAGES - 1, tgt);
        __builtin_amdgcn_sched_barrier(0);
        dma_mma<1, NJ, 2, 3>(a0, b0, acc);
        if (more && has_b) issue_b(t + DMA_STAGES - 1, tgt);
        __builtin_amdgcn_sched_barrier(0);
        dma_mma<1, NJ, 3, 4>(a0, b0, acc);
        if (more) {
            oa.advance();
            adv_b();
        }
        __builtin_amdgcn_sched_barrier(0);
        dma_mma<1, NJ, 0, 1>(a1, b1, acc);
        __builtin_amdgcn_sched_barrier(0);
        if (t + 1 < n) {
            const float* sn = smem + nxt * ST;
            oa.template read<1>(sn, lane, 0, a0);
            rb(sn + A_ST, 0, b0);
        }
        __builtin_amdgcn_sched_barrier(0);
        dma_mma<1, NJ, 1, 4>(a1, b1, acc);
        cur = nxt;
    }
    if (part >= 0) {
        constexpr int SLAB = BM * BN;
        dma8_slab_store<NJ>(sp.slabs + (size_t)bx * SLAB, acc, wv, lane);
        asm volatile("s_waitcnt vmcnt(0)" ::: "memory");
        __syncthreads();
        unsigned* flag = reinterpret_cast<unsigned*>(smem);
        if (tid == 0) {
            unsigned old = __hip_atomic_load(sp.counters + rem_t, __ATOMIC_RELAXED, __HIP_MEMORY_SCOPE_AGENT);
            unsigned cnt;
            for (;;) {
                cnt = (old >> 8) == sp.epoch ? (old & 255u) : 0u;
                if (__hip_atomic_compare_exchange_strong(sp.counters + rem_t, &old, (sp.epoch << 8) | (cnt + 1u), __ATOMIC_RELAXED, __ATOMIC_RELAXED,
                                                         __HIP_MEMORY_SCOPE_AGENT))
                    break;
            }
            *flag = cnt;
        }
        __syncthreads();
        if (*flag != (unsigned)(sp.g - 1)) return;
#pragma unroll
        for (int j = 0; j < NJ; ++j)
// ... 10 lines not shown
```

### lidbox_amd/csrc/gemm_sk.h

```cpp
#pragma once

#include "gemm_shared.h"
#include "lds_dma.h"

namespace {

constexpr int SK_BM = 128, SK_BN = 128, SK_BK = 16;
constexpr int SK_A_STAGE = SK_BM * SK_BK, SK_B_STAGE = SK_BK * SK_BN, SK_STAGE = SK_A_STAGE + SK_B_STAGE;
constexpr int SK_STAGES = 3;
constexpr int SK_WGCU = 3;
constexpr int SK_SLAB = SK_BM * SK_BN;
constexpr size_t SK_COUNTER_BYTES = 16384;
constexpr size_t SK_LDS_BYTES = (size_t)SK_STAGES * SK_STAGE * sizeof(float);

struct SkPlan {
    int tiles_n, ntiles;
    int nk;
    int ktail;
    int dp_rounds;
    int sk_tiles, sk_first;
    int parts;
};

struct SkInner {
    const float* sb;
    unsigned vo[2];
    int rd;

    __device__ __forceinline__ void init(const float* base, const long (&roff)[2], int k0, int lane, int wsub) {
        sb = sk_uniform(base + k0);
        const int chunk = (lane & 3) ^ ((lane >> 4) & 3);
#pragma unroll
        for (int i = 0; i < 2; ++i) vo[i] = (unsigned)((roff[i] + chunk * 4) * 4);
        rd = (wsub * 64 + (lane & 31)) * 16;
    }
    __device__ __forceinline__ void issue(int i, unsigned dst) const { sk_dma_s(sb, vo[i], dst); }
    __device__ __forceinline__ void issue_tail(int i, unsigned dst, int kvalid, int lane) const {
        const int chunk = (lane & 3) ^ ((lane >> 4) & 3);
        const float* p = reinterpret_cast<const float*>(reinterpret_cast<const char*>(sb) + vo[i]);
        sk_dma_f(chunk * 4 < kvalid ? p : g_sk_zero, dst);
    }
    __device__ __forceinline__ void advance() { sb += SK_BK; }
    __device__ __forceinline__ void read(const float* st, int lane, int s2, float (&v)[2][4]) const {
        const int slot = (2 * s2 + (lane >> 5)) ^ ((lane >> 2) & 3);
#pragma unroll
        for (int b = 0; b < 2; ++b) {
            const f32x4_t x = *reinterpret_cast<const f32x4_t*>(st + rd + b * 32 * 16 + slot * 4);
            v[b][0] = x[0]; v[b][1] = x[1]; v[b][2] = x[2]; v[b][3] = x[3];
        }
    }
};

struct SkOuter {
    const float* sb;
    unsigned vo[2];
    long step;
    int rd;

    __device__ __forceinline__ void init(const float* base, long ld, int col0, int ncols, int k0, int lane, int wv, int wsub) {
        sb = sk_uniform(base + (long)k0 * ld + col0);
        int c = (lane & 31) * 4;
        if (col0 + c >= ncols) c = 0;
#pragma unroll
        for (int i = 0; i < 2; ++i) vo[i] = (unsigned)(((long)(2 * (wv * 2 + i) + (lane >> 5)) * ld + c) * 4);
        step = (long)SK_BK * ld;
        rd = (4 * (lane >> 5)) * 128 + wsub * 64 + (lane & 31);
    }
    __device__ __forceinline__ void issue(int i, unsigned dst) const { sk_dma_s(sb, vo[i], dst); }
    __device__ __forceinline__ void issue_tail(int i, unsigned dst, int kvalid, int lane, int wv) const {
        const float* p = reinterpret_cast<const float*>(reinterpret_cast<const char*>(sb) + vo[i]);
        sk_dma_f(2 * (wv * 2 + i) + (lane >> 5) < kvalid ? p : g_sk_zero, dst);
    }
    __device__ __forceinline__ void advance() { sb += step; }
    __device__ __forceinline__ void read(const float* st, int lane, int s2, float (&v)[2][4]) const {
#pragma unroll
        for (int b = 0; b < 2; ++b)
#pragma unroll
            for (int j = 0; j < 4; ++j) v[b][j] = st[rd + (8 * s2 + j) * 128 + b * 32];
    }
};

struct SkOuterRows {
    const float* sb;
    int off[2];
    unsigned tt[2];
    int a_step, a_wrap;
    unsigned rpb;
    int mleft[2];
    int rd;

    __device__ __forceinline__ void init(const RowsD& X, int col0, int ncols, long mbeg, long mend, int lane, int wv, int wsub) {
        sb = sk_uniform(X.base + col0);
        int c = (lane & 31) * 4;
        if (col0 + c >= ncols) c = 0;
        a_step = (int)(SK_BK * X.rs);
        a_wrap = X.batch == 1 ? 0 : (int)(X.bs - (long)X.rpb * X.rs);
        rpb = X.batch == 1 ? 0xffffffffu : (unsigned)X.rpb;
#pragma unroll
        for (int i = 0; i < 2; ++i) {
            const long m = mbeg + 2 * (wv * 2 + i) + (lane >> 5);
            const unsigned bq = X.batch == 1 ? 0u : (unsigned)m / rpb;
            tt[i] = (unsigned)m - (X.batch == 1 ? 0u : bq * rpb);
            off[i] = (int)((long)bq * X.bs + (long)tt[i] * X.rs) + c;
            mleft[i] = (int)(mend - m);
        }
        rd = (4 * (lane >> 5)) * 128 + wsub * 64 + (lane & 31);
    }
    __device__ __forceinline__ void issue(int i, unsigned dst, bool tail) {
        if (!tail) {
            sk_dma_s(sb, (unsigned)off[i] * 4u, dst);
        } else {
            const float* p = reinterpret_cast<const float*>(reinterpret_cast<const char*>(sb) + (size_t)((unsigned)off[i] * 4u));
            sk_dma_f(mleft[i] > 0 ? p : g_sk_zero, dst);
        }
        mleft[i] -= SK_BK;
        tt[i] += SK_BK;
        off[i] += a_step;
        while (tt[i] >= rpb) { tt[i] -= rpb; off[i] += a_wrap; }
    }
    __device__ __forceinline__ void read(const float* st, int lane, int s2, float (&v)[2][4]) const {
#pragma unroll
        for (int b = 0; b < 2; ++b)
#pragma unroll
            for (int j = 0; j < 4; ++j) v[b][j] = st[rd + (8 * s2 + j) * 128 + b * 32];
    }
};

template <int J0, int J1>
__device__ __forceinline__ void sk_mma(const float (&a)[2][4], const float (&b)[2][4], f32x16 (&acc)[2][2]) {
#pragma unroll
    for (int j = J0; j < J1; ++j)
#pragma unroll
// ... 63 lines not shown
        }
        sk_mma<0, 1>(a0, b0, acc);
        drain(0);
        __builtin_amdgcn_sched_barrier(0);
        ra(st, 1, a1);
        rb(st + SK_A_STAGE, 1, b1);
        __builtin_amdgcn_sched_barrier(0);
        sk_mma<1, 2>(a0, b0, acc);
        if (more) issue(0, t + STAGES - 1, dst(tgt, 0));
        drain(1);
        __builtin_amdgcn_sched_barrier(0);
        sk_mma<2, 3>(a0, b0, acc);
        if (more) issue(1, t + STAGES - 1, dst(tgt, 1));
        drain(2);
        __builtin_amdgcn_sched_barrier(0);
        sk_mma<3, 4>(a0, b0, acc);
        if (more) issue(2, t + STAGES - 1, dst(tgt, 2));
        drain(3);
        __builtin_amdgcn_sched_barrier(0);
        sk_mma<0, 1>(a1, b1, acc);
        if (more) {
            issue(3, t + STAGES - 1, dst(tgt, 3));
            next();
        }
        drain(4);
        __builtin_amdgcn_sched_barrier(0);
        if (t + 1 < n) {
            const float* sn = smem + nxt * SK_STAGE;
            ra(sn, 0, a0);
            rb(sn + SK_A_STAGE, 0, b0);
        }
        __builtin_amdgcn_sched_barrier(0);
        sk_mma<1, 2>(a1, b1, acc);
        drain(5);
        __builtin_amdgcn_sched_barrier(0);
        sk_mma<2, 3>(a1, b1, acc);
        drain(6);
        __builtin_amdgcn_sched_barrier(0);
        sk_mma<3, 4>(a1, b1, acc);
        drain(7);
        step_end();
        cur = nxt;
    }
    if (WGCU > 0) __builtin_amdgcn_s_setprio(0);
}

__device__ __forceinline__ __amdgpu_buffer_rsrc_t sk_slab_rsrc(const float* slab) {
    return __builtin_amdgcn_make_buffer_rsrc(const_cast<float*>(sk_uniform(slab)), 0, SK_SLAB * 4, 0x00020000);
}
__device__ __forceinline__ void sk_slab_store(float* slab, const f32x16 (&acc)[2][2], int wv, int lane) {
    const __amdgpu_buffer_rsrc_t r = sk_slab_rsrc(slab);
#pragma unroll
    for (int bi = 0; bi < 2; ++bi)
#pragma unroll
        for (int bj = 0; bj < 2; ++bj)
#pragma unroll
            for (int r4 = 0; r4 < 4; ++r4) {
                const f32x4_t x = {acc[bi][bj][4 * r4], acc[bi][bj][4 * r4 + 1], acc[bi][bj][4 * r4 + 2], acc[bi][bj][4 * r4 + 3]};
                __builtin_amdgcn_raw_buffer_store_b128(__builtin_bit_cast(u32x4_t, x), r,
                                                       ((((wv * 4 + bi * 2 + bj) * 4 + r4) * 64 + lane) * 4) * 4, 0,  16);
            }
}
__device__ __forceinline__ void sk_slab_add(const float* slab, f32x16 (&acc)[2][2], int wv, int lane) {
    const __amdgpu_buffer_rsrc_t r = sk_slab_rsrc(slab);
#pragma unroll
    for (int bi = 0; bi < 2; ++bi)
#pragma unroll
        for (int bj = 0; bj < 2; ++bj) {
#pragma unroll
            for (int r4 = 0; r4 < 4; ++r4) {
                const f32x4_t x = __builtin_bit_cast(
                    f32x4_t, __builtin_amdgcn_raw_buffer_load_b128(r, ((((wv * 4 + bi * 2 + bj) * 4 + r4) * 64 + lane) * 4) * 4, 0,  16));
#pragma unroll
                for (int j = 0; j < 4; ++j) acc[bi][bj][4 * r4 + j] += x[j];
            }
            __builtin_amdgcn_sched_barrier(0);
        }
}

template <bool B_KINNER>
__global__ __launch_bounds__(256, SK_WGCU) void gemm_sk_rows_kernel(RowsD A, const float* __restrict__ Bm, long ldb, RowsOutD Cd,
                                                                    long M, int K, int N, int epi, const float* __restrict__ aux,
                                                                    SkPlan pl, unsigned epoch, unsigned* __restrict__ counters,
                                                                    float* __restrict__ slabs) {
    extern __shared__ __attribute__((aligned(16))) float sk_smem[];
    const int tid = threadIdx.x, lane = tid & 63;
    const int wv = __builtin_amdgcn_readfirstlane(tid >> 6);
    const int wm = wv >> 1, wn = wv & 1;
    const unsigned P = gridDim.x;
    const unsigned pid = xcd_chunk_id(blockIdx.x, P);
    const int prio_slot = (int)(blockIdx.x >> 8);
    const unsigned lds0 = __builtin_amdgcn_readfirstlane((unsigned)(size_t)(__attribute__((address_space(3))) void*)sk_smem);
    const int nk = pl.nk;
    const long total = (long)pl.sk_tiles * nk;

    auto run_item = [&](int tile, int kb, int ke, f32x16 (&acc)[2][2], long& m0, int& n0) {
        const int tn = tile % pl.tiles_n, tm = tile / pl.tiles_n;
        m0 = (long)tm * SK_BM;
        n0 = tn * SK_BN;
        SkInner oa;
        {
            long roff[2];
#pragma unroll
            for (int i = 0; i < 2; ++i) {
                long r = m0 + 16 * (wv * 2 + i) + (lane >> 2);
                if (r >= M) r = m0;
                roff[i] = row_offset(A, (unsigned)r);
            }
            oa.init(A.base, roff, kb * SK_BK, lane, wm);
        }
        SkInner obi;
        SkOuter obo;
        if (B_KINNER) {
            long roff[2];
#pragma unroll
            for (int i = 0; i < 2; ++i) {
                long r = n0 + 16 * (wv * 2 + i) + (lane >> 2);
                if (r >= N) r = n0;
                roff[i] = r * ldb;
            }
            obi.init(Bm, roff, kb * SK_BK, lane, wn);
        } else {
            obo.init(Bm, ldb, n0, N, kb * SK_BK, lane, wv, wn);
        }
#pragma unroll
        for (int i = 0; i < 2; ++i)
#pragma unroll
            for (int j = 0; j < 2; ++j)
#pragma unroll
                for (int r = 0; r < 16; ++r) acc[i][j][r] = 0.f;
        const int n = ke - kb;
        const int tail_step = (ke == nk && pl.ktail < SK_BK) ? n - 1 : -1;
        auto issue = [&](int pc, int step, unsigned d) {
            if (step == tail_step) {
                if (pc < 2) oa.issue_tail(pc, d, pl.ktail, lane);
                else if (B_KINNER) obi.issue_tail(pc - 2, d, pl.ktail, lane);
                else obo.issue_tail(pc - 2, d, pl.ktail, lane, wv);
            } else {
                if (pc < 2) oa.issue(pc, d);
                else if (B_KINNER) obi.issue(pc - 2, d);
                else obo.issue(pc - 2, d);
            }
        };
        auto next = [&]() {
            oa.advance();
            if (B_KINNER) obi.advance();
            else obo.advance();
        };
        auto ra = [&](const float* st, int s2, float (&v)[2][4]) { oa.read(st, lane, s2, v); };
        auto rb = [&](const float* st, int s2, float (&v)[2][4]) {
            if (B_KINNER) obi.read(st, lane, s2, v);
            else obo.read(st, lane, s2, v);
        };
        sk_kloop<SK_STAGES, SK_WGCU>(sk_smem, lds0, wv, n, prio_slot, issue, next, ra, rb, acc, SkNoDrain{}, [] {}, SkNoEpiOps{});
    };

    f32x16 acc[2][2];
    long m0;
    int n0;

    long it = 0, end = 0;
    const int g = pl.parts;
    int pt_tile = -1, pt_part = 0;
    if (pl.sk_tiles > 0) {
        if (g == 0) {
            it = (long)pid * total / P;
            end = (long)(pid + 1) * total / P;
        } else {
            const int xcd = blockIdx.x & 7, idx = blockIdx.x >> 3;
            const int t = (idx / g) * 8 + xcd;
            if (t < pl.sk_tiles) { pt_tile = t; pt_part = idx % g; }
        }
    }
    int which = 0, d = 0;
    for (;;) {
        int tile, kb, ke, t = 0;
        if (pt_tile >= 0) {
            t = pt_tile;
            pt_tile = -1;
            kb = (int)((long)pt_part * nk / g);
            ke = (int)((long)(pt_part + 1) * nk / g);
            tile = pl.sk_first + t;
        } else if (it < end) {
            t = (int)(it / nk);
            kb = (int)(it - (long)t * nk);
            ke = kb + (int)(end - it);
            if (ke > nk) ke = nk;
            it += ke - kb;
            tile = pl.sk_first + t;
        } else if (d < pl.dp_rounds) {
            tile = d * (int)P + (int)pid;
            kb = 0;
            ke = nk;
            ++d;
        } else {
            break;
        }
        run_item(tile, kb, ke, acc, m0, n0);
        int lane_e = lane, wm_e = wm, wn_e = wn, wv_e = wv;
        RowsOutD Cd_e = Cd;
        asm volatile("" : "+v"(lane_e), "+s"(wm_e), "+s"(wn_e), "+s"(wv_e), "+s"(Cd_e.rs), "+s"(Cd_e.bs));
        bool finish = kb == 0 && ke == nk;
        bool reducer = false;
        if (!finish) {
            const long my_slab = g == 0 ? (long)pid * 2 + which : (long)blockIdx.x * 2;
            sk_slab_store(slabs + my_slab * SK_SLAB, acc, wv_e, lane_e);
            ++which;
            asm volatile("s_waitcnt vmcnt(0)" ::: "memory");
            __syncthreads();
            unsigned* flag = reinterpret_cast<unsigned*>(sk_smem);
            if (tid == 0) {
                unsigned old = __hip_atomic_load(counters + t, __ATOMIC_RELAXED, __HIP_MEMORY_SCOPE_AGENT);
                unsigned cnt;
                for (;;) {
                    cnt = (old >> 8) == epoch ? (old & 255u) : 0u;
                    if (__hip_atomic_compare_exchange_strong(counters + t, &old, (epoch << 8) | (cnt + 1u), __ATOMIC_RELAXED,
                                                             __ATOMIC_RELAXED, __HIP_MEMORY_SCOPE_AGENT))
                        break;
                }
                *flag = cnt;
            }
            __syncthreads();
            const unsigned ticket = *flag;
            long pa = 0, pb = g - 1;
            if (g == 0) {
                const long ib = (long)t * nk, ie = ib + nk;
                pa = ib * P / total;
                while (pa > 0 && pa * total / P > ib) --pa;
                while ((pa + 1) * total / P <= ib) ++pa;
// ... 52 lines not shown
    unsigned t_wrap;
    float bias0, bias1;
    float* dummy;
    float* stage;
    unsigned stage_lds;
};

__device__ __forceinline__ void skp_extract(const f32x16 (&acc)[2][2], int g, float (&val)[8]) {
#define SKP_CASE(G)                                                                        \
    case G:                                                                                \
        _Pragma("unroll") for (int i = 0; i < 8; ++i) val[i] = acc[(G) >> 2][((G) >> 1) & 1][8 * ((G) & 1) + i]; \
        break;
    switch (g) {
        SKP_CASE(0) SKP_CASE(1) SKP_CASE(2) SKP_CASE(3) SKP_CASE(4) SKP_CASE(5) SKP_CASE(6) SKP_CASE(7)
        default: break;
    }
#undef SKP_CASE
}

__device__ __forceinline__ long skp_row_off(long rb, int dr, const SkEpiCtx& c) {
    long o;
    const unsigned rbu = (unsigned)__builtin_amdgcn_readfirstlane((int)rb);
    if (c.Cd.batch != 1) {
        const unsigned b0 = rbu / (unsigned)c.Cd.rpb;
        const unsigned t0 = rbu - b0 * (unsigned)c.Cd.rpb;
        o = ((long)b0 * c.Cd.bs + (long)t0 * c.Cd.rs) + (long)dr * c.Cd.rs + (t0 + (unsigned)dr >= c.t_wrap ? c.wrap : 0);
    } else {
        o = (long)(rbu + (unsigned)dr) * c.Cd.rs;
    }
    return (long)rbu + dr < c.M ? o : -1;
}

template <bool HAS_MASK, bool ACCUM>
__device__ __forceinline__ void skp_issue_loads(const SkPend& pd, int g, const SkEpiCtx& c, int wm, int wn, int lane) {
    const int bi = g >> 2, bj = (g >> 1) & 1;
    const int i = lane >> 3, chunk = lane & 7;
    const int dr = (i & 3) + 8 * (i >> 2) + 16 * (g & 1);
    const int col = pd.n0 + wn * 64 + bj * 32 + chunk * 4;
    const long rb = pd.m0 + wm * 64 + bi * 32;
#pragma unroll
    for (int h = 0; h < 2; ++h) {
        const long o = skp_row_off(rb, dr + 4 * h, c);
        const long a = (o >= 0 && col < c.N) ? o + col : 0;
        const unsigned dst = c.stage_lds + (unsigned)((((g & 1) * 2) * SKP_STAGE_FLOATS + h * 256) * 4);
        if (HAS_MASK) sk_dma_f(c.aux + a, dst);
        if (ACCUM) sk_dma_f(c.Cd.base + a, dst + SKP_STAGE_FLOATS * 4);
    }
}

template <bool HAS_MASK, bool ACCUM>
__device__ __forceinline__ void skp_read_stage(int g, const SkEpiCtx& c, int lane, float (&mv)[8], float (&ov)[8]) {
    const float* st = c.stage + ((g & 1) * 2) * SKP_STAGE_FLOATS + (lane >> 5) * 256 + (lane & 31);
#pragma unroll
    for (int i = 0; i < 8; ++i) {
        if (HAS_MASK) mv[i] = st[i * 32];
        if (ACCUM) ov[i] = st[SKP_STAGE_FLOATS + i * 32];
    }
}

template <bool HAS_MASK, bool ACCUM>
__device__ __forceinline__ void skp_store4(const SkPend& pd, int g, int i0, const SkEpiCtx& c, int wm, int wn, int lane,
                                           const float (&val)[8], const float (&mv)[8], const float (&ov)[8]) {
    const int bi = g >> 2, bj = (g >> 1) & 1;
    const int col = pd.n0 + wn * 64 + bj * 32 + (lane & 31);
    const float bias = bj ? c.bias1 : c.bias0;
    const long rb = pd.m0 + wm * 64 + bi * 32;
#pragma unroll
    for (int i = i0; i < i0 + 4; ++i) {
        const int dr = (i & 3) + 8 * (i >> 2) + 16 * (g & 1) + 4 * (lane >> 5);
        const long o = skp_row_off(rb, dr, c);
        float x = val[i] + bias;
        if (HAS_MASK) x = mv[i] > 0.f ? x : 0.f;
        if (ACCUM) x += ov[i];
        if (c.do_relu) x = fmaxf(x, 0.f);
        float* dst = (o >= 0 && col < c.N) ? c.Cd.base + o + col : c.dummy;
        *dst = x;
    }
}

template <bool B_KINNER, bool HAS_MASK, bool ACCUM>
__global__ __launch_bounds__(256, SKP_WGCU) void gemm_skp_rows_kernel(RowsD A, const float* __restrict__ Bm, long ldb, RowsOutD Cd,
                                                                      long M, int K, int N, int epi, const float* __restrict__ aux,
                                                                      SkPlan pl, unsigned epoch, unsigned* __restrict__ counters,
                                                                      float* __restrict__ slabs, float* __restrict__ dummy) {
    extern __shared__ __attribute__((aligned(16))) float sk_smem[];
    const int tid = threadIdx.x, lane = tid & 63;
    const int wv = __builtin_amdgcn_readfirstlane(tid >> 6);
    const int wm = wv >> 1, wn = wv & 1;
    const unsigned P = gridDim.x;
    const unsigned pid = xcd_chunk_id(blockIdx.x, P);
    const unsigned lds0 = __builtin_amdgcn_readfirstlane((unsigned)(size_t)(__attribute__((address_space(3))) void*)sk_smem);
    const int nk = pl.nk;
    const long total = (long)pl.sk_tiles * nk;

    SkEpiCtx ec;
    ec.Cd = Cd; ec.M = M; ec.N = N; ec.aux = aux;
    ec.has_bias = epi == LIDBOX_EPI_BIAS || epi == LIDBOX_EPI_BIAS_RELU;
    ec.do_relu = epi == LIDBOX_EPI_BIAS_RELU || epi == LIDBOX_EPI_ACCUM_RELU || epi == LIDBOX_EPI_RELU;
    ec.wrap = Cd.batch != 1 ? Cd.bs - (long)Cd.rpb * Cd.rs : 0;
    ec.t_wrap = Cd.batch != 1 ? (unsigned)Cd.rpb : 0xffffffffu;
    ec.bias0 = ec.bias1 = 0.f;
    ec.dummy = dummy + (long)blockIdx.x * 256 + tid;
    ec.stage = sk_smem + SK_STAGES * SK_STAGE + wv * 4 * SKP_STAGE_FLOATS;
    ec.stage_lds = lds0 + (unsigned)((SK_STAGES * SK_STAGE + wv * 4 * SKP_STAGE_FLOATS) * 4);

    SkPend pd;
    pd.s = 10;
    pd.m0 = 0; pd.n0 = 0;
    float val[8], mv[8], ov[8];
#pragma unroll
    for (int i = 0; i < 8; ++i) { val[i] = 0.f; mv[i] = 0.f; ov[i] = 0.f; }
    auto drain_piece = [&](int which, const f32x16 (&prev)[2][2]) {
        const int ds = __builtin_amdgcn_readfirstlane(pd.s);
        if (ds >= 10) return;
        if (which == -1) {
            if (ds >= 2) {
                skp_read_stage<HAS_MASK, ACCUM>(ds - 2, ec, lane, mv, ov);
                skp_extract(prev, ds - 2, val);
            }
        } else if (which == 0) {
            if ((HAS_MASK || ACCUM) && ds >= 2) asm volatile("s_waitcnt lgkmcnt(0)" ::: "memory");
            if (ds < 8) skp_issue_loads<HAS_MASK, ACCUM>(pd, ds, ec, wm, wn, lane);
        } else if (ds >= 2) {
            skp_store4<HAS_MASK, ACCUM>(pd, ds - 2, which == 1 ? 0 : 4, ec, wm, wn, lane, val, mv, ov);
        }
    };
    auto drain_ops = [&]() -> int {
        const int ds = __builtin_amdgcn_readfirstlane(pd.s);
        if (ds >= 10) return 0;
        return (ds < 8 ? 2 * ((HAS_MASK ? 1 : 0) + (ACCUM ? 1 : 0)) : 0) + (ds >= 2 ? 8 : 0);
    };
    auto flush = [&](const f32x16 (&prev)[2][2]) {
        while (pd.s < 10) {
            asm volatile("s_waitcnt vmcnt(0)" ::: "memory");
            drain_piece(-1, prev);
            drain_piece(0, prev);
            drain_piece(1, prev);
            drain_piece(2, prev);
            ++pd.s;
        }
    };

    long it = 0, end = 0;
    const int g = pl.parts;
    int pt_tile = -1, pt_part = 0;
    if (pl.sk_tiles > 0) {
        if (g == 0) {
            it = (long)pid * total / P;
            end = (long)(pid + 1) * total / P;
        } else {
            const int xcd = blockIdx.x & 7, idx = blockIdx.x >> 3;
            const int t = (idx / g) * 8 + xcd;
            if (t < pl.sk_tiles) { pt_tile = t; pt_part = idx % g; }
        }
    }
    int which = 0, d = 0;

    f32x16 cur[2][2], prev[2][2];
#pragma unroll
    for (int i = 0; i < 2; ++i)
#pragma unroll
        for (int j = 0; j < 2; ++j)
#pragma unroll
            for (int r = 0; r < 16; ++r) prev[i][j][r] = 0.f;
    for (;;) {
        int tile, kb, ke, t = 0;
        if (pt_tile >= 0) {
            t = pt_tile;
            pt_tile = -1;
            kb = (int)((long)pt_part * nk / g);
            ke = (int)((long)(pt_part + 1) * nk / g);
            tile = pl.sk_first + t;
        } else if (it < end) {
            t = (int)(it / nk);
            kb = (int)(it - (long)t * nk);
            ke = kb + (int)(end - it);
            if (ke > nk) ke = nk;
            it += ke - kb;
            tile = pl.sk_first + t;
        } else if (d < pl.dp_rounds) {
            tile = d * (int)P + (int)pid;
            kb = 0;
            ke = nk;
            ++d;
        } else {
            break;
        }
        const int tn = tile % pl.tiles_n, tm = tile / pl.tiles_n;
        const long m0 = (long)tm * SK_BM;
        const int n0 = tn * SK_BN;
        SkInner oa;
        {
            long roff[2];
#pragma unroll
            for (int i = 0; i < 2; ++i) {
                long r = m0 + 16 * (wv * 2 + i) + (lane >> 2);
                if (r >= M) r = m0;
                roff[i] = row_offset(A, (unsigned)r);
            }
            oa.init(A.base, roff, kb * SK_BK, lane, wm);
        }
        SkInner obi;
        SkOuter obo;
        if (B_KINNER) {
            long roff[2];
#pragma unroll
            for (int i = 0; i < 2; ++i) {
                long r = n0 + 16 * (wv * 2 + i) + (lane >> 2);
                if (r >= N) r = n0;
                roff[i] = r * ldb;
            }
            obi.init(Bm, roff, kb * SK_BK, lane, wn);
        } else {
            obo.init(Bm, ldb, n0, N, kb * SK_BK, lane, wv, wn);
        }
#pragma unroll
        for (int i = 0; i < 2; ++i)
#pragma unroll
            for (int j = 0; j < 2; ++j)
#pragma unroll
                for (int r = 0; r < 16; ++r) cur[i][j][r] = 0.f;
        const int n = ke - kb;
        const int tail_step = (ke == nk && pl.ktail < SK_BK) ? n - 1 : -1;
        auto issue = [&](int pc, int step, unsigned dd) {
            if (step == tail_step) {
                if (pc < 2) oa.issue_tail(pc, dd, pl.ktail, lane);
                else if (B_KINNER) obi.issue_tail(pc - 2, dd, pl.ktail, lane);
                else obo.issue_tail(pc - 2, dd, pl.ktail, lane, wv);
            } else {
                if (pc < 2) oa.issue(pc, dd);
                else if (B_KINNER) obi.issue(pc - 2, dd);
                else obo.issue(pc - 2, dd);
            }
        };
        auto next = [&]() {
            oa.advance();
            if (B_KINNER) obi.advance();
            else obo.advance();
        };
        auto ra = [&](const float* st, int s2, float (&v)[2][4]) { oa.read(st, lane, s2, v); };
        auto rb = [&](const float* st, int s2, float (&v)[2][4]) {
            if (B_KINNER) obi.read(st, lane, s2, v);
            else obo.read(st, lane, s2, v);
        };
        auto drain = [&](int i) {
            if (i >= 4) drain_piece(i - 5, prev);
        };
        auto step_end = [&]() {
            if (pd.s < 10) ++pd.s;
        };
        sk_kloop<SK_STAGES, 0>(sk_smem, lds0, wv, n, 0, issue, next, ra, rb, cur, drain, step_end, drain_ops);
        flush(prev);
        if (kb == 0 && ke == nk) {
#pragma unroll
            for (int i = 0; i < 2; ++i)
#pragma unroll
                for (int j = 0; j < 2; ++j) prev[i][j] = cur[i][j];
            pd.s = 0;
            pd.m0 = m0;
            pd.n0 = n0;
            if (ec.has_bias) {
                const int c0 = n0 + wn * 64 + (lane & 31);
                ec.bias0 = c0 < N ? aux[c0] : 0.f;
                ec.bias1 = c0 + 32 < N ? aux[c0 + 32] : 0.f;
            }
            continue;
        }
#pragma unroll
        for (int i = 0; i < 2; ++i)
#pragma unroll
            for (int j = 0; j < 2; ++j)
#pragma unroll
                for (int r = 0; r < 16; ++r) prev[i][j][r] = 0.f;
#pragma unroll
        for (int i = 0; i < 8; ++i) { val[i] = 0.f; mv[i] = 0.f; ov[i] = 0.f; }
        int lane_e = lane, wv_e = wv;
        asm volatile("" : "+v"(lane_e), "+s"(wv_e));
        const long my_slab = g == 0 ? (long)pid * 2 + which : (long)blockIdx.x * 2;
        sk_slab_store(slabs + my_slab * SK_SLAB, cur, wv_e, lane_e);
        ++which;
        asm volatile("s_waitcnt vmcnt(0)" ::: "memory");
        __syncthreads();
        unsigned* flag = reinterpret_cast<unsigned*>(sk_smem);
        if (tid == 0) {
            unsigned old = __hip_atomic_load(counters + t, __ATOMIC_RELAXED, __HIP_MEMORY_SCOPE_AGENT);
            unsigned cnt;
            for (;;) {
                cnt = (old >> 8) == epoch ? (old & 255u) : 0u;
                if (__hip_atomic_compare_exchange_strong(counters + t, &old, (epoch << 8) | (cnt + 1u), __ATOMIC_RELAXED,
                                                         __ATOMIC_RELAXED, __HIP_MEMORY_SCOPE_AGENT))
                    break;
            }
            *flag = cnt;
        }
        __syncthreads();
        const unsigned ticket = *flag;
        long pa = 0, pb = g - 1;
        if (g == 0) {
            const long ib = (long)t * nk, ie = ib + nk;
            pa = ib * P / total;
            while (pa > 0 && pa * total / P > ib) --pa;
            while ((pa + 1) * total / P <= ib) ++pa;
            pb = (ie - 1) * P / total;
            while (pb + 1 < (long)P && (pb + 1) * total / P < ie) ++pb;
            while (pb * total / P >= ie) --pb;
        }
        __syncthreads();
        if (ticket == (unsigned)(pb - pa)) {
#pragma unroll
            for (int i = 0; i < 2; ++i)
#pragma unroll
                for (int j = 0; j < 2; ++j)
#pragma unroll
                    for (int r = 0; r < 16; ++r) cur[i][j][r] = 0.f;
            for (long p = pa; p <= pb; ++p) {
                long sl;
                if (g == 0) {
                    const long b = p * total / P, e = (p + 1) * total / P;
                    const long t0 = b / nk;
                    const bool first_partial = !(b == t0 * nk && e >= (t0 + 1) * nk);
// ... 78 lines not shown
```

### lidbox_amd/csrc/gemm_tuned.h

```cpp
#pragma once

namespace {

struct TunedGemm {
    int kind;
    long M;
    int N, K, bm, bn, splits, no_tail_split, waves;
};

const TunedGemm TUNED_GEMM[] = {
    {1, 8448, 512, 1500, 128, 64, 1, 0, 8},
    {1, 25344, 1024, 512, 64, 128, 1, 1, 4},
    {1, 25344, 1000, 500, 128, 64, 1, 0, 8},
    {0, 50688, 512, 200, 64, 64, 1, 0, 4},
    {1, 25344, 512, 512, 64, 64, 1, 1, 4},
    {0, 8448, 512, 1536, 64, 64, 1, 1, 4},
    {1, 8448, 1536, 512, 64, 128, 1, 1, 4},
    {2, 8448, 512, 512, 64, 64, 24, 0, 4},
    {0, 8448, 1500, 512, 64, 64, 1, 1, 4},
    {1, 50688, 1024, 512, 64, 64, 1, 1, 4},
    {0, 16896, 512, 1536, 64, 64, 1, 1, 4},
    {1, 16896, 1536, 512, 64, 128, 1, 1, 4},
    {1, 512, 3000, 512, 64, 64, 1, 1, 4},
    {0, 512, 4, 512, 64, 64, 8, 0, 4},
    {2, 512, 4, 512, 64, 64, 8, 0, 4},
    {0, 25344, 512, 200, 64, 64, 1, 1, 4},
    {2, 25344, 512, 200, 64, 64, 48, 0, 4},
    {0, 12672, 512, 1536, 64, 64, 1, 0, 4},
    {1, 12672, 1024, 512, 64, 64, 1, 0, 4},
    {0, 4224, 512, 1536, 64, 64, 1, 0, 4},
    {2, 4224, 512, 512, 64, 64, 16, 0, 4},
    {1, 4224, 512, 1500, 64, 64, 1, 0, 4},
    {2, 12672, 512, 200, 64, 64, 32, 0, 4},
    {0, 6336, 512, 1536, 64, 64, 1, 0, 4},
    {0, 2112, 512, 1536, 64, 64, 4, 0, 4},
    {2, 2112, 512, 1536, 64, 64, 8, 0, 4},
    {0, 2112, 512, 512, 64, 64, 1, 1, 4},
    {2, 2112, 512, 512, 64, 64, 12, 0, 4},
    {1, 2112, 512, 512, 64, 64, 1, 1, 4},
    {2, 2112, 1500, 512, 64, 64, 8, 0, 4},
    {0, 202752, 512, 200, 64, 128, 1, 0, 4},
    {0, 101376, 512, 1536, 128, 128, 1, 1, 4},
    {1, 101376, 1024, 512, 64, 128, 1, 0, 4},
    {0, 33792, 512, 1536, 64, 128, 1, 1, 4},
    {1, 33792, 1536, 512, 128, 128, 1, 0, 4},
    {0, 33792, 512, 512, 64, 64, 1, 0, 4},
    {1, 33792, 512, 512, 64, 64, 1, 0, 4},
    {0, 33792, 1500, 512, 128, 128, 1, 1, 4},
    {2, 1024, 512, 3000, 64, 64, 4, 0, 4},
    {0, 1024, 512, 512, 64, 64, 1, 1, 4},
    {1, 1024, 512, 512, 64, 64, 2, 0, 4},
    {0, 50688, 500, 60, 64, 64, 1, 0, 4},
    {2, 25344, 500, 3500, 128, 64, 9, 0, 4},
    {0, 25344, 3000, 500, 128, 64, 1, 1, 4},
    {1, 25344, 500, 500, 64, 64, 1, 0, 4},
    {0, 25344, 500, 500, 64, 128, 1, 1, 4},
    {1, 25344, 500, 3000, 128, 128, 1, 0, 4},
    {0, 25344, 500, 60, 64, 64, 1, 1, 4},
    {0, 12672, 500, 3500, 128, 64, 1, 1, 4},
    {2, 12672, 500, 3500, 128, 128, 13, 0, 4},
    {1, 12672, 1000, 500, 64, 64, 1, 1, 4},
    {1, 12672, 500, 3000, 128, 64, 1, 0, 4},
    {0, 101376, 500, 60, 64, 128, 1, 1, 4},
    {2, 101376, 500, 60, 64, 64, 128, 0, 4},
    {0, 50688, 500, 3500, 128, 128, 1, 0, 4},
    {2, 50688, 500, 3500, 128, 128, 27, 0, 4},
    {1, 50688, 1000, 500, 128, 128, 1, 1, 4},
    {0, 50688, 3000, 500, 128, 128, 1, 0, 4},
    {1, 50688, 500, 3000, 128, 128, 1, 0, 4},
    {0, 512, 1500, 3000, 64, 64, 4, 0, 4},
    {0, 512, 600, 1500, 64, 64, 6, 0, 4},
    {2, 512, 600, 1500, 64, 64, 3, 0, 4},
    {1, 512, 1500, 600, 64, 64, 2, 0, 4},
    {0, 512, 4, 600, 64, 64, 8, 0, 4},
    {2, 512, 4, 600, 64, 64, 8, 0, 4},
};

inline const TunedGemm* tuned_gemm(int kind, long M, int N, int K) {
    if (getenv("LIDBOX_GEMM_NO_TUNED")) return nullptr;
    for (const TunedGemm& t : TUNED_GEMM)
        if (t.kind == kind && t.M == M && t.N == N && t.K == K) return &t;
    return nullptr;
}

}
```

### lidbox_amd/models/tdnn.py

```python
import ctypes
import os
import math

import numpy as np
import torch

from .. import _native as nv
from .flat import FlatParams, Workspace, _align4, _rows


class ConvSpec:

    PADDINGS = ("causal", "valid", "same")

    def __init__(self, name, filters, kernel_size, strides, relu=True, dilation_rate=1, dense_kernel=False, padding="causal"):
        self.name, self.filters, self.k, self.s, self.relu = name, int(filters), int(kernel_size), int(strides), relu
        self.padding = str(padding).lower()
        if self.padding not in self.PADDINGS:
            raise ValueError("padding must be one of %s, got %r" % (self.PADDINGS, padding))
        self.dense_kernel = bool(dense_kernel) and int(kernel_size) == 1
        self.d = int(dilation_rate) if int(kernel_size) > 1 else 1
        if self.d < 1 or self.k < 1 or self.s < 1:
            raise ValueError("kernel_size, strides and dilation_rate must be >= 1")
        if self.d > 1 and self.s > 1:
# ... 6 lines not shown
    def geometry(self, T):
        ke = (self.k - 1) * self.d + 1
        if T <= 0:
            return (ke - 1 if self.padding == "causal" else 0), 0, 0
        if self.padding == "causal":
            return ke - 1, 0, (T - 1) // self.s + 1
        if self.padding == "valid":
            return 0, 0, ((T - ke) // self.s + 1 if T >= ke else 0)
        To = -(-T // self.s)
        total = max((To - 1) * self.s + ke - T, 0)
        return total // 2, total - total // 2, To


class FreqAttentionSpec:

    def __init__(self, d_a=64, d_f=16):
        self.d_a, self.d_f = int(d_a), int(d_f)
        if not 1 <= self.d_f <= 64:
            raise ValueError("frequency attention supports 1 <= d_f <= 64 bins")


class FreqConvSpec:

    def __init__(self, name, filters, kernel_width, stride, momentum=0.99, epsilon=1e-3, dropout_rate=None):
        self.name, self.filters, self.k, self.s = name, int(filters), int(kernel_width), int(stride)
        self.momentum, self.epsilon = float(momentum), float(epsilon)
        self.dropout_rate = float(dropout_rate or 0.0)
        if not 0.0 <= self.dropout_rate < 1.0:
            raise ValueError("dropout_rate must be in [0, 1)")
        if self.k < 1 or self.s < 1 or self.filters < 1:
            raise ValueError("filters, kernel width and stride must be >= 1")


def freq_out_len(F, k, s):
    return (F - k) // s + 1 if F >= k else 0


class DenseSpec:
    def __init__(self, name, units, relu=True):
        self.name, self.units, self.relu = name, int(units), relu


def conv_out_len(T, s):
    return (T - 1) // s + 1 if T > 0 else 0


class _GemmFamily:

    _PREFIX = {"float32": "lidbox_gemm_", "bfloat16": "lidbox_gemm_bf16_"}

    def __init__(self, compute_dtype):
        if compute_dtype in ("float32", "fp32", "f32", torch.float32):
            self.name = "float32"
        elif compute_dtype in ("bfloat16", "bf16", torch.bfloat16):
            self.name = "bfloat16"
        else:
            raise ValueError("compute_dtype must be 'float32' or 'bfloat16', got %r" % (compute_dtype,))
        self._prefix = self._PREFIX[self.name]

    def __getattr__(self, op):
        if op.startswith("_"):
            raise AttributeError(op)
        return getattr(nv.lib, self._prefix + op)


class _Workspace(Workspace):

    def __init__(self, model, B, T):
        dev = model.device
        self.B, self.T = B, T
        f32 = dict(dtype=torch.float32, device=dev)
        convs = model.convs
        self.Ts = [T]
        self.pads, self.rpads = [], []
        for c in convs:
            pl, pr, To = c.geometry(self.Ts[-1])
            self.pads.append(pl)
            self.rpads.append(pr)
            self.Ts.append(To)
        self.pads.append(0)
        self.rpads.append(0)
        chans = [model.input_dim] + [c.filters for c in convs]
        self.trail = [0] * len(chans)
        if model.bf16_storage:
            for i in range(1, len(convs) - 1):
                self.trail[i + 1] = model._dgrad_trail(i, self.Ts[i])
        self.act = [torch.zeros((B, self.pads[i] + self.Ts[i] + self.rpads[i] + self.trail[i], chans[i]), **f32) for i in range(len(chans))]
        self.dact = [None] + [torch.zeros_like(a) for a in self.act[1:]]
        self.act16 = [None] * len(self.act)
        self.dact16 = [None] * len(self.act)
        self.d16_fresh = set()
        if model.bf16_storage:
            for i, c in enumerate(convs):
                if model.shadow_fwd_ok(i):
                    self.act16[i] = torch.zeros(self.act[i].shape, dtype=torch.bfloat16, device=dev)
                if (i >= 1 and model.shadow_dgrad_ok(i)) or model.shadow_wgrad_ok(i):
                    shp = self.act[i + 1].shape
                    self.dact16[i + 1] = torch.zeros((shp[0], shp[1], (shp[2] + 7) // 8 * 8), dtype=torch.bfloat16, device=dev)
        self.last16 = None
        if (model.bf16_storage and model.bf16_only and model.pool == "stats" and model.attention is None and 1 <= self.Ts[-1] <= 40
                and chans[-1] % 4 == 0 and model.shadow_fwd_ok(len(convs) - 1) and convs[-1].d == 1
                and os.environ.get("LIDBOX_BF16_POOL_FP32", "0") != "1"):
            self.last16 = torch.zeros((B, self.Ts[-1], (chans[-1] + 7) // 8 * 8), dtype=torch.bfloat16, device=dev)
            self.act[-1].fill_(float("nan"))
            self.dact[-1].fill_(float("nan"))
        fe = model.frontend
        if fe:
            self.dact[0] = torch.zeros_like(self.act[0])
            self.fe_in = torch.zeros((B, T, model.model_input_dim), **f32)
            self.fe_R = [B * T * model.fe_dims[i + 1] for i in range(len(fe))]
            self.fe_a = [torch.zeros((self.fe_R[i], l.filters), **f32) for i, l in enumerate(fe)]
            self.fe_dz = [torch.zeros_like(a) for a in self.fe_a]
            self.fe_y = [torch.zeros_like(a) for a in self.fe_a[:-1]]
            self.fe_dy = [torch.zeros_like(a) for a in self.fe_a[:-1]]
            self.fe_consts = [torch.zeros((4, l.filters), **f32) for l in fe]
            bn_bytes = max(int(nv.lib.lidbox_bn_workspace(self.fe_R[i], l.filters)) for i, l in enumerate(fe))
            self.bn_ws = torch.empty(max(16, bn_bytes), dtype=torch.uint8, device=dev)
        C_last = chans[-1]
        att = model.attention
        if att is not None:
            n = B * self.Ts[-1]
            self.fa_x1 = torch.zeros((n, att.d_a), **f32)
            self.fa_F = torch.zeros((n, att.d_f), **f32)
            self.hw = torch.zeros_like(self.act[-1])
            self.d_hw = torch.zeros_like(self.act[-1])
            self.d_logit = torch.zeros((n, att.d_f), **f32)
            self.d_x1 = torch.zeros((n, att.d_a), **f32)
        P = 2 * C_last if model.pool == "stats" else C_last
        self.pooled = torch.zeros((B, P), **f32)
        self.dpooled = torch.zeros((B, P), **f32)
        self.h = [torch.zeros((B, d.units), **f32) for d in model.denses]
        self.dh = [torch.zeros((B, d.units), **f32) for d in model.denses]
        self.logp = torch.zeros((B, model.denses[-1].units), **f32)
        self.emb = torch.zeros((B, model.denses[0].units), **f32)
        self.loss = torch.zeros(4, **f32)
        ws_bytes = 16
        g = model.gemm
        if fe:
            cin_f = 1
            for i, l in enumerate(fe):
                gf = model.fe_gemm(i)
                M, kk = self.fe_R[i], l.k * cin_f
                if M > 0:
                    ws_bytes = max(ws_bytes, gf.tn_workspace(M, kk, l.filters), gf.rows_workspace(M, l.filters, kk),
                                   gf.rows_workspace(M, kk, l.filters))
                cin_f = l.filters
        cin = model.input_dim
        for i, c in enumerate(convs):
            M = B * self.Ts[i + 1]
            if M > 0:
                kk = cin if c.d > 1 else c.k * cin
                ws_bytes = max(ws_bytes, g.tn_workspace(M, kk, c.filters),
                               g.rows_workspace(M, c.filters, kk), g.rows_workspace(M, kk, c.filters))
                if model.bf16_storage and model.shadow_wgrad_ok(i):
                    ws_bytes = max(ws_bytes, nv.lib.lidbox_gemm_bf16s_tn_workspace(M, kk, c.filters))
            cin = c.filters
        if att is not None and B * self.Ts[-1] > 0:
            n = B * self.Ts[-1]
            for (kk, nn_) in ((C_last, att.d_a), (att.d_a, att.d_f)):
                ws_bytes = max(ws_bytes, g.tn_workspace(n, kk, nn_), g.rows_workspace(n, nn_, kk), g.rows_workspace(n, kk, nn_))
        din = P
        for d in model.denses:
            for gd in {g, model.dense_gemm}:
                ws_bytes = max(ws_bytes, gd.tn_workspace(B, din, d.units), gd.rows_workspace(B, d.units, din),
                               gd.rows_workspace(B, din, d.units))
            din = d.units
        self.gemm_ws = torch.empty(ws_bytes, dtype=torch.uint8, device=dev)
        self.gemm_ws2 = torch.empty(ws_bytes, dtype=torch.uint8, device=dev)
        self.tn_regions = (torch.empty(ws_bytes, dtype=torch.uint8, device=dev), torch.empty(ws_bytes, dtype=torch.uint8, device=dev))
# ... 94 lines not shown
                self.state_layout[l.name + suffix] = (soff, (l.filters,)); soff = _align4(soff + l.filters)
        self.state = torch.zeros(max(soff, 4), dtype=torch.float32, device=self.device)
        self._init_weights(seed)
        self.bf16_storage = self.compute_dtype == "bfloat16" and os.environ.get("LIDBOX_BF16_STORAGE", "1") != "0" \
            and attention is None and not self.frontend and all(c.padding == "causal" for c in self.convs)
        if self.bf16_storage and not any(self.shadow_fwd_ok(i) for i in range(len(self.convs))):
            self.bf16_storage = False
        if self.bf16_storage:
            self.flat16 = torch.zeros(self.num_flat, dtype=torch.bfloat16, device=self.device)
            cin = self.input_dim
            self.w16t = []
            self.wd16 = []
            n = len(self.convs)
            self.bf16_only = os.environ.get("LIDBOX_BF16_FP32_COPIES", "0") != "1" and self.pool == "stats" and all(
                self.shadow_wgrad_ok(i) and (i == 0 or (self.shadow_dgrad_ok(i) and (self.convs[i].k <= self.convs[i].s or i < n - 1)))
                for i in range(n))
            bf = dict(dtype=torch.bfloat16, device=self.device)
            for i, c in enumerate(self.convs):
                self.w16t.append(torch.zeros((c.filters, c.k * cin), **bf) if self.shadow_fwd_ok(i) else None)
                img = {}
                if i >= 1 and self.shadow_dgrad_ok(i):
                    cp = (c.filters + 7) // 8 * 8
                    if c.k > c.s and i < len(self.convs) - 1:
                        for rho, Q, _, _ in self._dgrad_residues(i, 1 << 20):
                            img[rho] = torch.zeros((cin, Q * cp), **bf)
                    elif c.k <= c.s and cp != c.filters:
                        img["fused"] = torch.zeros((c.k * cin, cp), **bf)
                self.wd16.append(img)
                cin = c.filters
        if not self.bf16_storage:
            self.bf16_only = False
        self._ws = {}
        self.wgrad_stream = None
        self.head_wgrad_stream = None

    def _init_weights(self, seed):
        rng = np.random.default_rng(seed)
        host = np.zeros(self.num_flat, np.float32)
        for name, (off, shape) in self.layout.items():
            if name.endswith(".W"):
                if len(shape) == 4:
                    _, k, ci, co = shape
                    fan_in, fan_out = k * ci, k * co
                elif len(shape) == 3:
                    k, ci, co = shape
                    fan_in, fan_out = k * ci, k * co
                else:
                    fan_in, fan_out = shape
                limit = math.sqrt(6.0 / (fan_in + fan_out))
                n = int(np.prod(shape))
                host[off:off + n] = rng.uniform(-limit, limit, size=n).astype(np.float32)
            elif name.endswith("_bn.gamma"):
                host[off:off + shape[0]] = 1.0
        self.flat.copy_(torch.from_numpy(host))
        for name, (off, shape) in self.state_layout.items():
            self.state[off:off + shape[0]] = 1.0 if name.endswith("moving_variance") else 0.0

    def _cin(self, i):
        return self.input_dim if i == 0 else self.convs[i - 1].filters

    def shadow_fwd_ok(self, i):
        c = self.convs[i]
        return c.d == 1 and self._cin(i) % 8 == 0

    def shadow_wgrad_ok(self, i):
        c = self.convs[i]
        return c.d == 1 and self._cin(i) % 8 == 0 and c.filters % 4 == 0

    def shadow_dgrad_ok(self, i):
        c = self.convs[i]
        return c.d == 1 and c.filters % 4 == 0 and self._cin(i) % 8 == 0

    def _dgrad_residues(self, i, T):
        c = self.convs[i]
        res = []
        for rho in range(min(c.s, c.k)):
            Q = (c.k - rho + c.s - 1) // c.s
            u_min = -((rho - c.pad) // c.s)
            u_max = (c.pad + T - 1 - rho) // c.s
            if T > 0 and u_max >= u_min:
                res.append((rho, Q, u_min, u_max))
        return res

    def _dgrad_trail(self, i, T):
        c = self.convs[i]
        if not (c.d == 1 and c.k > c.s and self.shadow_dgrad_ok(i)) or T <= 0:
            return 0
        To = conv_out_len(T, c.s)
        return max(0, max(u_max for _, _, _, u_max in self._dgrad_residues(i, T)) - (To - 1))

    def _refresh_bf16_weights(self):
        mats = getattr(self, "_w16t_descs", None)
        if mats is None:
            items = []
            live = self._flat16_live = set()
            for i, c in enumerate(self.convs):
                off, cin, co = self.layout[c.name + ".W"][0], self._cin(i), c.filters
                if self.w16t[i] is not None:
                    items.append((off, c.k * cin, co, self.w16t[i].data_ptr(), c.k * cin, 1))
                if i >= 1 and self.shadow_dgrad_ok(i) and not self.wd16[i]:
                    items.append((off, c.k * cin, co, self.flat16.data_ptr() + 2 * off, co, 0))
                    live.add(c.name + ".W")
                for key, img in self.wd16[i].items():
                    if key == "fused":
                        items.append((off, c.k * cin, co, img.data_ptr(), img.shape[1], 0))
                        continue
                    Q = (c.k - key + c.s - 1) // c.s
                    cp = img.shape[1] // Q
                    for q in range(Q):
                        items.append((off + (key + q * c.s) * cin * co, cin, co, img.data_ptr() + 2 * (Q - 1 - q) * cp,
                                      img.shape[1], 0))
            mats = (nv.WeightShadow * max(1, len(items)))(*[nv.WeightShadow(*it) for it in items])
            self._w16t_descs, self._w16t_n = mats, len(items)
        nv.check(nv.lib.lidbox_refresh_bf16_weights(nv.ptr(self.flat), None, self.num_flat, mats, self._w16t_n, nv.current_stream()))

    def _p16(self, name):
        if name not in getattr(self, "_flat16_live", ()):
            raise RuntimeError("flat16 holds no refreshed image of %r (refreshed: %s)" % (name, sorted(getattr(self, "_flat16_live", ()))))
        off, _ = self.layout[name]
        return ctypes.c_void_p(self.flat16.data_ptr() + 2 * off)

    @staticmethod
    def _rows16(view_rows, t32, t16):
        off = (view_rows.base - t32.data_ptr()) // 4
        C, C16 = t32.shape[-1], t16.shape[-1]
        if C16 == C:
            return nv.Rows(t16.data_ptr() + 2 * off, view_rows.batch_stride, view_rows.row_stride, view_rows.batch,
                           view_rows.rows_per_batch)
        assert view_rows.batch_stride % C == 0 and view_rows.row_stride % C == 0
        r, col = divmod(off, C)
        return nv.Rows(t16.data_ptr() + 2 * (r * C16 + col), view_rows.batch_stride // C * C16, view_rows.row_stride // C * C16,
                       view_rows.batch, view_rows.rows_per_batch)

    def fe_gemm(self, i):
        return self.gemm if i > 0 else _GemmFamily("float32")

    def _conv_rows_in(self, ws, i):
        a = ws.act[i]
        c = self.convs[i]
        Tp, C = a.shape[1], a.shape[2]
        return _rows(a.data_ptr(), Tp * C, c.s * C, ws.B, ws.Ts[i + 1])

    def _tap_rows(self, buf, ws, i, j):
        c = self.convs[i]
        Tp, C = buf.shape[1], buf.shape[2]
        return _rows(buf.data_ptr() + 4 * j * c.d * C, Tp * C, C, ws.B, ws.Ts[i + 1])

    def _tap_weight(self, c, cin, j, grad=False):
        return ctypes.c_void_p(self._p(c.name + ".W", grad).value + 4 * j * cin * c.filters)

    def _rows_out(self, buf, ws, i):
        Tp, C = buf.shape[1], buf.shape[2]
        return _rows(buf.data_ptr() + 4 * ws.pads[i] * C, Tp * C, C, ws.B, ws.Ts[i])

    def _fe_rows_in(self, ws, i):
        l = self.frontend[i]
        cin = 1 if i == 0 else self.frontend[i - 1].filters
        src = ws.fe_in if i == 0 else ws.fe_y[i - 1]
        return _rows(src.data_ptr(), self.fe_dims[i] * cin, l.s * cin, ws.B * ws.T, self.fe_dims[i + 1])

    def _fe_last_rows(self, buf, ws):
        Tp, C = buf.shape[1], buf.shape[2]
        return _rows(buf.data_ptr() + 4 * ws.pads[0] * C, Tp * C, self.frontend[-1].filters, ws.B, ws.T * self.fe_dims[-1])

    def _forward_frontend(self, ws, training, update_moving):
        st, lib = nv.current_stream(), nv.lib
        cin = 1
        for i, l in enumerate(self.frontend):
            R, Co, K = ws.fe_R[i], l.filters, l.k * cin
# ... 48 lines not shown
                                       self._p(l.name + "_bn.beta", True), nv.ptr(ws.fe_dz[i]), nv.ptr(ws.bn_ws), ws.bn_ws.numel(), st))
            dz = _rows(ws.fe_dz[i].data_ptr(), 0, Co, 1, R)
            A_rows = self._fe_rows_in(ws, i)
            self._launch_wgrad(ws, lambda w, nb, s_, A_rows=A_rows, dz=dz, l=l, K=K, Co=Co, g=g: nv.check(g.tn(
                A_rows, dz, self._p(l.name + "_conv.W", True), Co, K, Co, 0, self._p(l.name + "_conv.b", True), w, nb, s_)))
            if i == 0:
                continue
            dprev = ws.fe_dy[i - 1]
            Fi, Fo, BT = self.fe_dims[i], self.fe_dims[i + 1], ws.B * ws.T
            if l.k < l.s:
                nv.check(lib.lidbox_zero_2d(nv.ptr(dprev), 4 * dprev.numel(), 4 * dprev.numel(), 1, st))
            elif Fo * l.s < Fi:
                nv.check(lib.lidbox_zero_2d(ctypes.c_void_p(dprev.data_ptr() + 4 * Fo * l.s * cin), 4 * Fi * cin,
                                            4 * (Fi - Fo * l.s) * cin, BT, st))
            for grp in range((l.k + l.s - 1) // l.s):
                ntaps = min(l.s, l.k - grp * l.s)
                Cd = _rows(dprev.data_ptr() + 4 * grp * l.s * cin, Fi * cin, l.s * cin, BT, Fo)
                Wg = ctypes.c_void_p(self._p(l.name + "_conv.W").value + 4 * grp * l.s * cin * Co)
                nv.check(g.nt(dz, Wg, Co, Cd, Co, ntaps * cin, nv.EPI_NONE if grp == 0 else nv.EPI_ACCUM, None, gws, gws_n, st))
        self.join_wgrad()

    def _before_conv(self, ws, i, training, update_moving):
        """layers a subclass runs between conv i-1 and conv i in forward_ws (models/clstm.py: its 2-D front-end before
        conv 0, its LSTM before frame4); none here"""

    def fused_output_ok(self):
        if self.output_activation != "log_softmax" or len(self.denses) < 2 or self.denses[-1].relu:
            return False
        if self.dense_gemm.name != "float32":
            return False
        return bool(nv.lib.lidbox_softmax_head_supported(self.denses[-2].units, self.denses[-1].units))

    def forward_ws(self, ws, upto_embedding=False, training=False, update_moving=True, stop_before_output=False):
        st = nv.current_stream()
        lib = nv.lib
        if self.frontend:
            self._forward_frontend(ws, training, update_moving)
        if self.bf16_storage:
            self._refresh_bf16_weights()
            if ws.act16[0] is not None and not ws.__dict__.pop("input16_fresh", False):
                nv.check(lib.lidbox_f32_to_bf16(nv.ptr(ws.act[0]), nv.ptr(ws.act16[0]), ws.act[0].numel(), st))
        cin = self.input_dim
        fresh16 = False
        for i, c in enumerate(self.convs):
            self._before_conv(ws, i, training, update_moving)
            if ws.B * ws.Ts[i + 1] > 0 and c.d == 1 and ws.act16[i] is not None:
                if i > 0 and not fresh16:
                    nv.check(lib.lidbox_f32_to_bf16(nv.ptr(ws.act[i]), nv.ptr(ws.act16[i]), ws.act[i].numel(), st))
                fresh16 = ws.act16[i + 1] is not None
                out_rows = self._rows_out(ws.act[i + 1], ws, i + 1)
                nxt = ws.act16[i + 1]
                sh = None if nxt is None else ctypes.c_void_p(nxt.data_ptr() + (out_rows.base - ws.act[i + 1].data_ptr()) // 2)
                if self.bf16_only and nxt is not None and i + 1 < len(self.convs):
                    out_rows = nv.Rows(None, out_rows.batch_stride, out_rows.row_stride, out_rows.batch, out_rows.rows_per_batch)
                elif ws.last16 is not None and i + 1 == len(self.convs):
                    l16 = ws.last16
                    out_rows = nv.Rows(None, l16.shape[1] * l16.shape[2], l16.shape[2], out_rows.batch, out_rows.rows_per_batch)
                    sh = nv.ptr(l16)
                nv.check(lib.lidbox_gemm_bf16s_nt(self._rows16(self._conv_rows_in(ws, i), ws.act[i], ws.act16[i]),
                                                  nv.ptr(self.w16t[i]), c.k * cin, out_rows, sh, c.k * cin, c.filters,
                                                  nv.EPI_BIAS_RELU if c.relu else nv.EPI_BIAS, self._p(c.name + ".b"),
                                                  nv.ptr(ws.gemm_ws), ws.gemm_ws.numel(), st))
            elif ws.B * ws.Ts[i + 1] > 0 and c.d == 1:
                fresh16 = False
                nv.check(self.gemm.nn(self._conv_rows_in(ws, i), self._p(c.name + ".W"), c.filters,
                                            self._rows_out(ws.act[i + 1], ws, i + 1), c.k * cin, c.filters,
                                            nv.EPI_BIAS_RELU if c.relu else nv.EPI_BIAS, self._p(c.name + ".b"),
                                            nv.ptr(ws.gemm_ws), ws.gemm_ws.numel(), st))
            elif ws.B * ws.Ts[i + 1] > 0:
                fresh16 = False
                out = self._rows_out(ws.act[i + 1], ws, i + 1)
                for j in range(c.k):
                    if j == 0:
                        epi = nv.EPI_BIAS
                    elif j < c.k - 1 or not c.relu:
                        epi = nv.EPI_ACCUM
                    else:
                        epi = nv.EPI_ACCUM_RELU
                    nv.check(self.gemm.nn(self._tap_rows(ws.act[i], ws, i, j), self._tap_weight(c, cin, j), c.filters,
                                          out, cin, c.filters, epi, self._p(c.name + ".b") if j == 0 else None,
                                          nv.ptr(ws.gemm_ws), ws.gemm_ws.numel(), st))
            cin = c.filters
        last = ws.act[-1]
        T, C = last.shape[1], last.shape[2]
        att = self.attention
        if att is not None and ws.B * T > 0:
            n = ws.B * T
            gws, gws_n = nv.ptr(ws.gemm_ws), ws.gemm_ws.numel()
            nv.check(self.gemm.nn(_rows(last.data_ptr(), 0, C, 1, n), self._p("Wf_1.W"), att.d_a,
                                  _rows(ws.fa_x1.data_ptr(), 0, att.d_a, 1, n), C, att.d_a, nv.EPI_RELU, None, gws, gws_n, st))
            nv.check(self.gemm.nn(_rows(ws.fa_x1.data_ptr(), 0, att.d_a, 1, n), self._p("Wf_2.W"), att.d_f,
                                  _rows(ws.fa_F.data_ptr(), 0, att.d_f, 1, n), att.d_a, att.d_f, nv.EPI_NONE, None, gws, gws_n, st))
            nv.check(lib.lidbox_freq_attention_fwd(nv.ptr(last), nv.ptr(ws.fa_F), n, C, att.d_f, nv.ptr(ws.fa_F),
                                                   nv.ptr(ws.hw), st))
            last = ws.hw
        if ws.last16 is not None:
            C16 = ws.last16.shape[2]
            nv.check(lib.lidbox_stats_pool_fwd_bf16(nv.ptr(ws.last16), ws.B, T, C, T * C16, C16, nv.ptr(ws.pooled), st))
        else:
            fn = lib.lidbox_stats_pool_fwd if self.pool == "stats" else lib.lidbox_avg_pool_fwd
            nv.check(fn(nv.ptr(last), ws.B, T, C, T * C, C, nv.ptr(ws.pooled), st))
        x, din = ws.pooled, ws.pooled.shape[1]
        for j, d in enumerate(self.denses):
            if stop_before_output and j == len(self.denses) - 1:
                return x
            emb = upto_embedding and j == 0
            out = ws.emb if emb else ws.h[j]
            epi = nv.EPI_BIAS_RELU if (d.relu and not emb) else nv.EPI_BIAS
            nv.check(self.dense_gemm.nn(_rows(x.data_ptr(), 0, din, 1, ws.B), self._p(d.name + ".W"), d.units,
                                        _rows(out.data_ptr(), 0, d.units, 1, ws.B), din, d.units, epi,
                                        self._p(d.name + ".b"), nv.ptr(ws.gemm_ws), ws.gemm_ws.numel(), st))
            if emb:
                return ws.emb
            x, din = out, d.units
        if self.output_activation is None:
            return ws.h[-1]
        if self.output_activation == "softmax":
            nv.check(lib.lidbox_softmax_fwd(nv.ptr(ws.h[-1]), ws.B, din, nv.ptr(ws.logp), st))
            return ws.logp
        nv.check(lib.lidbox_log_softmax_fwd(nv.ptr(ws.h[-1]), ws.B, din, nv.ptr(ws.logp), st))
        return ws.logp

    def _tn_region(self, ws):
        busy = {r for _, r in ws.pending}
        for r in (0, 1):
            if r not in busy:
                return r
        self.flush_reduce_jobs(ws)
        return 0

    def _take_jobs(self, ws, limit):
        if len(ws.pending) > limit:
            keep = ws.pending[len(ws.pending) - limit:] if limit > 0 else []
            ws.pending = ws.pending[:len(ws.pending) - limit]
            self.flush_reduce_jobs(ws)
            ws.pending = keep
        n = len(ws.pending)
        arr = (nv.ReduceJob * max(1, n))(*[j for j, _ in ws.pending])
        ws.pending = []
        return arr, n

    def flush_reduce_jobs(self, ws):
        while ws.pending:
            chunk, ws.pending = ws.pending[:2], ws.pending[2:]
            arr = (nv.ReduceJob * len(chunk))(*[j for j, _ in chunk])
            nv.check(nv.lib.lidbox_reduce_jobs_run(arr, len(chunk), nv.current_stream()))

    def _dgrad_wgrad(self, ws, dy, W, ldb, dX, Co, N, epi, aux, X, dW, ldc, K1, db):
        r = self._tn_region(ws)
        jobs, n = self._take_jobs(ws, 1)
        out = nv.ReduceJob()
        tws = ws.tn_regions[r]
        nv.check(nv.lib.lidbox_gemm_nt_tn_carry(dy, W, ldb, dX, Co, N, epi, aux, nv.ptr(ws.gemm_ws), ws.gemm_ws.numel(), X, dW, ldc, K1, 0, db,
                                                nv.ptr(tws), tws.numel(), jobs, n, ctypes.byref(out), nv.current_stream()))
        if out.nblocks:
            ws.pending.append((out, r))

    def _launch_wgrad(self, ws, launch, head=False):
        side = self.wgrad_stream
        if side is None and head:
            side = self.head_wgrad_stream
        if side is None:
            launch(nv.ptr(ws.gemm_ws), ws.gemm_ws.numel(), nv.current_stream())
            return
        side.wait_stream(torch.cuda.current_stream())
        with torch.cuda.stream(side):
            launch(nv.ptr(ws.gemm_ws2), ws.gemm_ws2.numel(), nv.current_stream())

    def join_wgrad(self):
        if self.wgrad_stream is not None:
            torch.cuda.current_stream().wait_stream(self.wgrad_stream)
        if self.head_wgrad_stream is not None:
            torch.cuda.current_stream().wait_stream(self.head_wgrad_stream)

    def backward_ws(self, ws):
        self.backward_head_ws(ws)
        for i in range(len(self.convs) - 1, -1, -1):
            self.backward_conv_ws(ws, i)
        self.flush_reduce_jobs(ws)
        self.join_wgrad()

    def backward_head_ws(self, ws):
        st = nv.current_stream()
        lib = nv.lib
        B = ws.B
        ws.d16_fresh = set()
        ws.pending = []
        gws, gws_n = nv.ptr(ws.gemm_ws), ws.gemm_ws.numel()
        top = len(self.denses) - 1
        if getattr(ws, "output_layer_done", False):
            ws.output_layer_done = False
            top -= 1
        for j in range(top, -1, -1):
            d = self.denses[j]
            x = ws.pooled if j == 0 else ws.h[j - 1]
            din = x.shape[1]
            dy = _rows(ws.dh[j].data_ptr(), 0, d.units, 1, B)
            A_rows = _rows(x.data_ptr(), 0, din, 1, B)
            dst = ws.dpooled if j == 0 else ws.dh[j - 1]
            relu_prev = j > 0 and self.denses[j - 1].relu
            epi, aux = (nv.EPI_RELU_MASK, nv.ptr(x)) if relu_prev else (nv.EPI_NONE, None)
            dst_rows = _rows(dst.data_ptr(), 0, din, 1, B)
            if self.dense_gemm.name == "float32" and self.wgrad_stream is None and self.head_wgrad_stream is None:
                self._dgrad_wgrad(ws, dy, self._p(d.name + ".W"), d.units, dst_rows, d.units, din, epi, aux,
                                  A_rows, self._p(d.name + ".W", True), d.units, din, self._p(d.name + ".b", True))
                continue
            self._launch_wgrad(ws, lambda w, n, s_, A_rows=A_rows, dy=dy, d=d, din=din: nv.check(self.dense_gemm.tn(
                A_rows, dy, self._p(d.name + ".W", True), d.units, din, d.units, 0, self._p(d.name + ".b", True), w, n, s_)),
                head=True)
            nv.check(self.dense_gemm.nt(dy, self._p(d.name + ".W"), d.units, dst_rows, d.units, din, epi, aux, gws, gws_n, st))
        att = self.attention
        last = ws.act[-1] if att is None else ws.hw
        dlast = ws.dact[-1] if att is None else ws.d_hw
        T, C = last.shape[1], last.shape[2]
        relu_last = 1 if self.convs[-1].relu else 0
        pool_mask = relu_last if att is None else 0
        d16 = ws.dact16[-1] if att is None else None
        if ws.last16 is not None and d16 is not None and B * T > 0:
            C16 = ws.last16.shape[2]
            nv.check(lib.lidbox_stats_pool_bwd_bf16(nv.ptr(ws.last16), nv.ptr(ws.pooled), nv.ptr(ws.dpooled), B, T, C, T * C16, C16,
                                                    pool_mask, nv.ptr(d16), T * d16.shape[2], d16.shape[2], st))
            ws.d16_fresh.add(len(self.convs))
        elif self.pool == "stats" and d16 is not None and B * T > 0:
            nv.check(lib.lidbox_stats_pool_bwd_shadow(nv.ptr(last), nv.ptr(ws.pooled), nv.ptr(ws.dpooled), B, T, C, T * C, C,
                                                      pool_mask, None if self.bf16_only else nv.ptr(dlast), nv.ptr(d16),
                                                      T * d16.shape[2], d16.shape[2], st))
            ws.d16_fresh.add(len(self.convs))
        elif self.pool == "stats":
            nv.check(lib.lidbox_stats_pool_bwd(nv.ptr(last), nv.ptr(ws.pooled), nv.ptr(ws.dpooled), B, T, C, T * C, C,
                                               pool_mask, nv.ptr(dlast), st))
        else:
            nv.check(lib.lidbox_avg_pool_bwd(nv.ptr(last), nv.ptr(ws.dpooled), B, T, C, T * C, C, pool_mask,
                                             nv.ptr(dlast), st))
        if att is None or B * T == 0:
            return
        n = B * T
        H = ws.act[-1]
        nv.check(lib.lidbox_freq_attention_bwd(nv.ptr(H), nv.ptr(ws.fa_F), nv.ptr(ws.d_hw), n, C, att.d_f, relu_last,
                                               nv.ptr(ws.d_logit), nv.ptr(ws.dact[-1]), st))
        x1r, dlr = _rows(ws.fa_x1.data_ptr(), 0, att.d_a, 1, n), _rows(ws.d_logit.data_ptr(), 0, att.d_f, 1, n)
        Hr, dx1r = _rows(H.data_ptr(), 0, C, 1, n), _rows(ws.d_x1.data_ptr(), 0, att.d_a, 1, n)
        self._launch_wgrad(ws, lambda w, n_, s_: nv.check(self.gemm.tn(
            x1r, dlr, self._p("Wf_2.W", True), att.d_f, att.d_a, att.d_f, 0, None, w, n_, s_)))
        nv.check(self.gemm.nt(dlr, self._p("Wf_2.W"), att.d_f, dx1r, att.d_f, att.d_a, nv.EPI_RELU_MASK,
                              nv.ptr(ws.fa_x1), gws, gws_n, st))
        self._launch_wgrad(ws, lambda w, n_, s_: nv.check(self.gemm.tn(
            Hr, dx1r, self._p("Wf_1.W", True), att.d_a, C, att.d_a, 0, None, w, n_, s_)))
        nv.check(self.gemm.nt(dx1r, self._p("Wf_1.W"), att.d_a, _rows(ws.dact[-1].data_ptr(), 0, C, 1, n), att.d_a, C,
                              nv.EPI_ACCUM_RELU_MASK if relu_last else nv.EPI_ACCUM, nv.ptr(H) if relu_last else None,
                              gws, gws_n, st))

    def backward_conv_ws(self, ws, i):
        st = nv.current_stream()
        lib = nv.lib
        B = ws.B
        gws, gws_n = nv.ptr(ws.gemm_ws), ws.gemm_ws.numel()
        c = self.convs[i]
        cin = self.input_dim if i == 0 else self.convs[i - 1].filters
        K = c.k * cin
        To = ws.Ts[i + 1]
        if B * To == 0:
            self.param(c.name + ".W", True).zero_()
            self.param(c.name + ".b", True).zero_()
            return
        dy = self._rows_out(ws.dact[i + 1], ws, i + 1)
        if c.d > 1:
            self._backward_dilated(ws, i, dy)
            return
        A_rows = self._conv_rows_in(ws, i)
        pair_wgrad = False
        dy16 = ws.dact16[i + 1] if self.bf16_storage else None
        if dy16 is not None and (i + 1) not in ws.d16_fresh:
            if dy16.shape == ws.dact[i + 1].shape:
                nv.check(lib.lidbox_f32_to_bf16(nv.ptr(ws.dact[i + 1]), nv.ptr(dy16), ws.dact[i + 1].numel(), st))
                ws.d16_fresh.add(i + 1)
            else:
                dy16 = None
        if dy16 is not None and ws.act16[i] is not None and self.shadow_wgrad_ok(i):
            A16, B16 = self._rows16(A_rows, ws.act[i], ws.act16[i]), self._rows16(dy, ws.dact[i + 1], dy16)
            if self.wgrad_stream is None:
                r = self._tn_region(ws)
                job, tws = nv.ReduceJob(), ws.tn_regions[r]
                nv.check(lib.lidbox_gemm_bf16s_tn_partial(A16, B16, self._p(c.name + ".W", True), c.filters, K, c.filters, 0,
                                                          self._p(c.name + ".b", True), nv.ptr(tws), tws.numel(), ctypes.byref(job), st))
                if job.nblocks:
                    ws.pending.append((job, r))
            else:
                self._launch_wgrad(ws, lambda w, n, s_: nv.check(lib.lidbox_gemm_bf16s_tn(
                    A16, B16, self._p(c.name + ".W", True), c.filters, K, c.filters, 0, self._p(c.name + ".b", True), w, n, s_)))
        elif (self.gemm.name == "float32" and self.wgrad_stream is None and not self.bf16_storage and
              not (i == 0 and not self.frontend)):
            pair_wgrad = True
        elif self.gemm.name == "float32" and self.wgrad_stream is None and not self.bf16_storage:
            r = self._tn_region(ws)
            job, tws = nv.ReduceJob(), ws.tn_regions[r]
            nv.check(lib.lidbox_gemm_tn_partial(A_rows, dy, self._p(c.name + ".W", True), c.filters, K, c.filters, 0,
                                                self._p(c.name + ".b", True), nv.ptr(tws), tws.numel(), ctypes.byref(job), st))
            if job.nblocks:
                ws.pending.append((job, r))
        else:
            self._launch_wgrad(ws, lambda w, n, s_: nv.check(self.gemm.tn(
                A_rows, dy, self._p(c.name + ".W", True), c.filters, K, c.filters, 0, self._p(c.name + ".b", True), w, n, s_)))
        if i == 0 and not self.frontend:
            return
        dprev, aprev = ws.dact[i], ws.act[i]
        Tp = dprev.shape[1]
        relu_prev = self.convs[i - 1].relu if i > 0 else False
        ngroups = (c.k + c.s - 1) // c.s
        use16 = self.bf16_storage and dy16 is not None and self.shadow_dgrad_ok(i)
        d16 = ws.dact16[i] if use16 else None
        only16 = self.bf16_only and use16 and d16 is not None
        if use16 and ngroups > 1 and self.wd16[i]:
            Tp2, cp = dy16.shape[1], dy16.shape[2]
            calls = []
            for rho, Q, u_min, u_max in self._dgrad_residues(i, ws.Ts[i]):
                nu, p0 = u_max - u_min + 1, u_min * c.s + rho
                A16 = nv.Rows(dy16.data_ptr() + 2 * (ws.pads[i + 1] + u_min - Q + 1) * cp, Tp2 * cp, cp, B, nu)
                Cd = _rows(None if only16 else dprev.data_ptr() + 4 * p0 * cin, Tp * cin, c.s * cin, B, nu)
                epi, mask = nv.EPI_NONE, None
                if relu_prev and only16:
                    epi, mask = nv.EPI_RELU_MASK | nv.EPI_MASK_BF16, ctypes.c_void_p(ws.act16[i].data_ptr() + 2 * p0 * cin)
                elif relu_prev:
                    epi, mask = nv.EPI_RELU_MASK, ctypes.c_void_p(aprev.data_ptr() + 4 * p0 * cin)
                sh = None if d16 is None else ctypes.c_void_p(d16.data_ptr() + 2 * p0 * cin)
                calls.append((A16, nv.ptr(self.wd16[i][rho]), Q * cp, Cd, sh, Q * cp, cin, epi, mask))
            if len(calls) == 2:
                jobs, nj = self._take_jobs(ws, 2)
                nv.check(lib.lidbox_gemm_bf16s_nt_pair_carry(*calls[0], *calls[1], gws, gws_n, jobs, nj, st))
            else:
                for call in calls:
                    jobs, nj = self._take_jobs(ws, 2)
                    nv.check(lib.lidbox_gemm_bf16s_nt_carry(*call, gws, gws_n, jobs, nj, st))
            if d16 is not None:
                ws.d16_fresh.add(i)
            return
        if use16 and (ngroups > 1 or "fused" not in self.wd16[i]) and c.filters % 8 != 0:
            use16, d16 = False, None
        if ngroups > 1 and To * c.s < Tp:
            if pair_wgrad and ((Tp - To * c.s) * cin) % 4 == 0 and (Tp * cin) % 4 == 0 and dprev.data_ptr() % 16 == 0 and (To * c.s * cin) % 4 == 0:
                zj = nv.ReduceJob()
                nv.check(lib.lidbox_zero_job(ctypes.c_void_p(dprev.data_ptr() + 4 * To * c.s * cin), Tp * cin, (Tp - To * c.s) * cin, B,
                                             ctypes.byref(zj)))
                self.flush_reduce_jobs(ws)
                ws.pending.append((zj, -1))
            else:
                nv.check(lib.lidbox_zero_2d(ctypes.c_void_p(dprev.data_ptr() + 4 * To * c.s * cin), 4 * Tp * cin,
                                            4 * (Tp - To * c.s) * cin, B, st))
            if d16 is not None:
                nv.check(lib.lidbox_zero_2d(ctypes.c_void_p(d16.data_ptr() + 2 * To * c.s * cin), 2 * Tp * cin,
                                            2 * (Tp - To * c.s) * cin, B, st))
        if d16 is not None:
            ws.d16_fresh.add(i)
        fused16 = self.wd16[i].get("fused") if use16 else None
        for g in range(ngroups):
            ntaps = min(c.s, c.k - g * c.s)
            base_off = 4 * g * c.s * cin
            Cd = _rows(dprev.data_ptr() + base_off, Tp * cin, c.s * cin, B, To)
            Wg = ctypes.c_void_p(self._p(c.name + ".W").value + 4 * g * c.s * cin * c.filters)
            mask = ctypes.c_void_p(aprev.data_ptr() + base_off) if relu_prev else None
            if g == 0:
                epi = nv.EPI_RELU_MASK if relu_prev else nv.EPI_NONE
            else:
                epi = nv.EPI_ACCUM_RELU_MASK if relu_prev else nv.EPI_ACCUM
            if use16:
                sh = None if d16 is None else ctypes.c_void_p(d16.data_ptr() + base_off // 2)
                A16 = self._rows16(dy, ws.dact[i + 1], dy16)
                if only16 and ngroups == 1:
                    Cd = _rows(None, Tp * cin, c.s * cin, B, To)
                    if relu_prev:
                        epi, mask = epi | nv.EPI_MASK_BF16, ctypes.c_void_p(ws.act16[i].data_ptr() + base_off // 2)
                jobs, nj = self._take_jobs(ws, 2)
                if fused16 is not None:
                    cp = fused16.shape[1]
                    nv.check(lib.lidbox_gemm_bf16s_nt_carry(A16, nv.ptr(fused16), cp, Cd, sh, cp, ntaps * cin, epi, mask, gws, gws_n, jobs, nj, st))
                else:
                    Wg16 = ctypes.c_void_p(self._p16(c.name + ".W").value + 2 * g * c.s * cin * c.filters)
                    nv.check(lib.lidbox_gemm_bf16s_nt_carry(A16, Wg16, c.filters, Cd, sh, c.filters, ntaps * cin, epi, mask, gws, gws_n,
                                                            jobs, nj, st))
            elif pair_wgrad and g == 0:
                self._dgrad_wgrad(ws, dy, Wg, c.filters, Cd, c.filters, ntaps * cin, epi, mask,
                                  A_rows, self._p(c.name + ".W", True), c.filters, K, self._p(c.name + ".b", True))
            else:
                nv.check(self.gemm.nt(dy, Wg, c.filters, Cd, c.filters, ntaps * cin, epi, mask, gws, gws_n, st))
        if i == 0:
            self._backward_frontend(ws)

    def _backward_dilated(self, ws, i, dy):
        st = nv.current_stream()
        gws, gws_n = nv.ptr(ws.gemm_ws), ws.gemm_ws.numel()
        c = self.convs[i]
        cin = self.input_dim if i == 0 else self.convs[i - 1].filters
        for j in range(c.k):
            A_rows = self._tap_rows(ws.act[i], ws, i, j)
            self._launch_wgrad(ws, lambda w, n, s_, A_rows=A_rows, j=j: nv.check(self.gemm.tn(
                A_rows, dy, self._tap_weight(c, cin, j, True), c.filters, cin, c.filters, 0,
                self._p(c.name + ".b", True) if j == 0 else None, w, n, s_)))
        if i == 0:
            return
        dprev, aprev = ws.dact[i], ws.act[i]
        relu_prev = self.convs[i - 1].relu
        To = ws.Ts[i + 1]
        if To < dprev.shape[1]:
            Tp = dprev.shape[1]
            nv.check(nv.lib.lidbox_zero_2d(ctypes.c_void_p(dprev.data_ptr() + 4 * To * cin), 4 * Tp * cin,
                                           4 * (Tp - To) * cin, ws.B, st))
        for j in range(c.k):
            mask = ctypes.c_void_p(aprev.data_ptr() + 4 * j * c.d * cin) if relu_prev else None
            if j == 0:
                epi = nv.EPI_RELU_MASK if relu_prev else nv.EPI_NONE
            else:
                epi = nv.EPI_ACCUM_RELU_MASK if relu_prev else nv.EPI_ACCUM
            nv.check(self.gemm.nt(dy, self._tap_weight(c, cin, j), c.filters, self._tap_rows(dprev, ws, i, j), c.filters,
                                  cin, epi, mask, gws, gws_n, st))

    def _load_input(self, ws, x, training):
        x = nv.require_gpu_tensor(x, "x", torch.float32)
        if x.dim() != 3 or x.shape[2] != self.model_input_dim:
            raise ValueError("expected input [B, T, %d], got %s" % (self.model_input_dim, tuple(x.shape)))
        if x.stride(2) != 1 or x.stride(1) != x.shape[2]:
            x = x.contiguous()
        st = nv.current_stream()
        in_ptr, in_bs, _, C = ws.input_target()
        nv.check(nv.lib.lidbox_copy_2d(in_ptr, 4 * in_bs, nv.ptr(x), 4 * (x.stride(0) if ws.B > 1 else ws.T * C),
                                       4 * ws.T * C, ws.B, st))
        if training and self.channel_dropout_rate > 0:
            self._dropout_calls += 1
            nv.check(nv.lib.lidbox_spatial_dropout(in_ptr, ws.B, ws.T, C, in_bs, self.channel_dropout_rate,
                                                   (self.dropout_seed + 0x51ED27 * self._dropout_calls) & (2 ** 64 - 1),
                                                   None, None, st))

    def __call__(self, x, training=False):
        with torch.cuda.device(self.device):
            ws = self.workspace(x.shape[0], x.shape[1])
            self._load_input(ws, x, training)
            return self.forward_ws(ws, training=training).clone()

    def embed(self, x):
        with torch.cuda.device(self.device):
            ws = self.workspace(x.shape[0], x.shape[1])
            self._load_input(ws, x, False)
            return self.forward_ws(ws, upto_embedding=True).clone()

    predict = __call__


class EmbeddingExtractor:

    def __init__(self, model):
        self.model = model
        self.name = model.name + ":" + model.embedding_layer

    def __call__(self, x, training=False):
        return self.model.embed(x)
```

Before: 120,600 utterances/s.

## Add segmented-K fp32 dgrad path for strided TDNN convs via residue GEMMs

Adds an EPI_SEGMENTS encoding so the NT GEMM kernels can walk the weight operand in Q segments with a negative stride. This lets the fp32 conv backward compute data gradients per output-phase residue as dense GEMMs over trailing-padded activations, rather than grouped GEMMs with a zero-fill. It also retunes several GEMM table entries and pads the fp32 activations with trailing space so the new path applies. The cost is more launches and added validation, and the change touches pooling strides to account for the padded layouts.

Measured after the change: 120,500 utterances/s. About the same (-0.2%).

```diff
diff --git a/include/lidbox_hip.h b/include/lidbox_hip.h
--- a/include/lidbox_hip.h
+++ b/include/lidbox_hip.h
@@ -112,6 +112,7 @@
     LIDBOX_EPI_RELU      = 7,
     LIDBOX_EPI_MASK_BF16 = 0x100
 };
+#define LIDBOX_EPI_SEGMENTS(Q, s) ((int)(((unsigned)(Q) | ((unsigned)(s) << 4)) << 16))
 
 int lidbox_gemm_plan_query(int kind, long M, int N, int K, size_t workspace_bytes, int* out4);
 
diff --git a/lidbox_amd/_native.py b/lidbox_amd/_native.py
--- a/lidbox_amd/_native.py
+++ b/lidbox_amd/_native.py
@@ -12,6 +12,12 @@
 SRC_F32, SRC_PCM16 = 0, 1
 EPI_NONE, EPI_BIAS, EPI_BIAS_RELU, EPI_RELU_MASK, EPI_ACCUM, EPI_ACCUM_RELU_MASK, EPI_ACCUM_RELU, EPI_RELU = range(8)
 EPI_MASK_BF16 = 0x100
+GEMM_K_STEP = 16
+
+
+def EPI_SEGMENTS(Q, s):
+    assert 1 <= Q <= 8 and 1 <= s <= 8
+    return (Q | (s << 4)) << 16
 
 
 class LidboxHipError(RuntimeError):
diff --git a/lidbox_amd/csrc/gemm.hip b/lidbox_amd/csrc/gemm.hip
--- a/lidbox_amd/csrc/gemm.hip
+++ b/lidbox_amd/csrc/gemm.hip
@@ -652,9 +652,10 @@
 
 template <int BM, int BN, bool B_KINNER>
 void launch_rows_dma_t(dim3 grid, hipStream_t st, RowsD Ad, const float* Bm, long ldb, RowsOutD Co, float* P, long m_beg, long m_end,
-                       int K, int N, int epi, const float* aux, int tiles_n, unsigned ntiles, int kps, const DmaStream& sp, const ReduceJobs& rj) {
+                       int K, int N, int epi, const float* aux, int tiles_n, unsigned ntiles, int kps, const DmaStream& sp, const ReduceJobs& rj,
+                       const KSegD& seg) {
     hipLaunchKernelGGL((gemm_rows_dma_kernel<BM, BN, B_KINNER>), grid, dim3(256), 0, st, Ad, Bm, ldb, Co, P, m_beg, m_end, K, N, epi,
-                       aux, tiles_n, ntiles, kps, sp, rj);
+                       aux, tiles_n, ntiles, kps, sp, rj, seg);
 }
 
 inline long carry_cap() {
@@ -700,7 +701,7 @@
 template <bool B_KINNER>
 int launch_rows_range(const RowsChoice& ch, bool al, RowsD Ad, const float* Bm, long ldb, RowsOutD Co, long m_beg,
                       long m_end, int K, int N, int epi, const float* aux, float* P, hipStream_t st, bool dma_ok = false,
-                      const DmaStreamPlan* stream = nullptr, void* ws = nullptr, Carry* carry = nullptr) {
+                      const DmaStreamPlan* stream = nullptr, void* ws = nullptr, Carry* carry = nullptr, const KSegD& seg = KSegD{}) {
     const long Msub = m_end - m_beg;
     if (Msub <= 0) return LIDBOX_OK;
     const int tiles_n = (int)lbx_cdiv(N, ch.bn);
@@ -711,7 +712,7 @@
     if (ch.splits > 1) ++g_last_launches[2];
 #define LBX_ROWS(BM_, BN_) launch_rows_t<BM_, BN_, B_KINNER>(al, grid, st, Ad, Bm, ldb, Co, P, m_beg, m_end, K, N, epi, aux, tiles_n, (unsigned)ntiles, ch.k_per_split)
 #define LBX_ROWS8(BM_, BN_) launch_rows8_t<BM_, BN_, B_KINNER>(al, grid, st, Ad, Bm, ldb, Co, P, m_beg, m_end, K, N, epi, aux, tiles_n, (unsigned)ntiles, ch.k_per_split)
-#define LBX_ROWS_DMA(BM_, BN_) launch_rows_dma_t<BM_, BN_, B_KINNER>(grid, st, Ad, Bm, ldb, Co, P, m_beg, m_end, K, N, epi, aux, tiles_n, ntiles_k, ch.k_per_split, sp, rj)
+#define LBX_ROWS_DMA(BM_, BN_) launch_rows_dma_t<BM_, BN_, B_KINNER>(grid, st, Ad, Bm, ldb, Co, P, m_beg, m_end, K, N, epi, aux, tiles_n, ntiles_k, ch.k_per_split, sp, rj, seg)
     if (dma_ok && al && dma_mode() != 0) {
         g_last_family = 1;
         DmaStream sp;
@@ -738,10 +739,10 @@
             g_last_family = 3;
             if (ch.bn == 128)
                 hipLaunchKernelGGL((gemm_rows_dma8_kernel<128, B_KINNER>), grid, dim3(512), 0, st, Ad, Bm, ldb, Co, P, m_beg, m_end, K, N, epi, aux, tiles_n,
-                                   ntiles_k, ch.k_per_split, sp, rj);
+                                   ntiles_k, ch.k_per_split, sp, rj, seg);
             else
                 hipLaunchKernelGGL((gemm_rows_dma8_kernel<64, B_KINNER>), grid, dim3(512), 0, st, Ad, Bm, ldb, Co, P, m_beg, m_end, K, N, epi, aux, tiles_n,
-                                   ntiles_k, ch.k_per_split, sp, rj);
+                                   ntiles_k, ch.k_per_split, sp, rj, seg);
         } else
         if (ch.bm == 128 && ch.bn == 128) LBX_ROWS_DMA(128, 128);
         else if (ch.bm == 128) LBX_ROWS_DMA(128, 64);
@@ -771,7 +772,7 @@
 
 template <bool B_KINNER>
 int launch_rows(lidbox_rows_t A, const float* Bm, long ldb, lidbox_rows_out_t Cd, int K, int N, int epi,
-                const float* aux, void* ws, size_t ws_bytes, hipStream_t st, Carry* carry = nullptr) {
+                const float* aux, void* ws, size_t ws_bytes, hipStream_t st, Carry* carry = nullptr, const KSegD& seg = KSegD{}) {
     const long M = (long)A.batch * A.rows_per_batch;
     g_last_launches[0] = g_last_launches[1] = g_last_launches[2] = 0;
     g_last_family = 0;
@@ -783,6 +784,11 @@
     RowsD Ad = to_dev(A);
     RowsOutD Co{Cd.base, Cd.batch_stride, Cd.row_stride, Cd.batch, Cd.rows_per_batch};
     float* P = (float*)ws;
+    const bool segmented = seg.steps != KSegD{}.steps;
+    if (segmented && !(al && dma_mode() != 0 && sk_extent_ok(A, K) && sk_b_extent_ok(B_KINNER, K, N, ldb))) {
+        lidbox_set_error("lidbox_gemm_nt: a segmented contraction needs 16-byte aligned operands with 32-bit extents on the LDS-DMA kernels");
+        return LIDBOX_E_INVALID;
+    }
 
     if (al && !getenv("LIDBOX_GEMM_PLAN") && aligned16(ws) && !sk_tuned_out(B_KINNER ? 1 : 0, M, N, K) &&
         sk_b_extent_ok(B_KINNER, K, N, ldb)) {
@@ -805,7 +811,7 @@
                 const unsigned ep = sk_next_epoch();
 #define LBX_SKP(MASK_, ACC_)                                                                                                \
     hipLaunchKernelGGL((gemm_skp_rows_kernel<B_KINNER, MASK_, ACC_>), dim3(sk.P), dim3(256), (MASK_ || ACC_) ? SKP_LDS_BYTES : SK_LDS_BYTES, st, Ad, Bm, ldb, Co, M, K, \
-                       N, epi, aux, sk.pl, ep, counters, slabs, dummy)
+                       N, epi, aux, sk.pl, ep, counters, slabs, dummy, seg)
                 if (has_mask && accum) LBX_SKP(true, true);
                 else if (has_mask) LBX_SKP(true, false);
                 else if (accum) LBX_SKP(false, true);
@@ -824,7 +830,7 @@
             unsigned* counters = (unsigned*)ws;
             float* slabs = (float*)((char*)ws + SK_COUNTER_BYTES);
             hipLaunchKernelGGL((gemm_sk_rows_kernel<B_KINNER>), dim3(sk.P), dim3(256), SK_LDS_BYTES, st, Ad, Bm, ldb, Co, M, K, N, epi,
-                               aux, sk.pl, sk_next_epoch(), counters, slabs);
+                               aux, sk.pl, sk_next_epoch(), counters, slabs, seg);
             LBX_LAUNCH_OK();
             return LIDBOX_OK;
         }
@@ -834,7 +840,7 @@
     if (dma_ok && dma_mode() != 0 && ch.splits == 1 && aligned16(ws)) {
         const DmaStreamPlan spl = dma_stream_plan(ch.bm, ch.bn, M, N, K);
         if (spl.g > 1 && wsb >= spl.ws_need)
-            return launch_rows_range<B_KINNER>(ch, al, Ad, Bm, ldb, Co, 0, M, K, N, epi, aux, P, st, dma_ok, &spl, ws, carry);
+            return launch_rows_range<B_KINNER>(ch, al, Ad, Bm, ldb, Co, 0, M, K, N, epi, aux, P, st, dma_ok, &spl, ws, carry, seg);
     }
     const bool no_tail_split = ch.no_tail_split || getenv("LIDBOX_GEMM_NO_TAIL_SPLIT") != nullptr;
     if (!no_tail_split && ch.splits == 1) {
@@ -856,14 +862,14 @@
                                            (double)rem.k_per_split / BK);
                 if (rem.splits > 1) split += 5.0 + (double)m_rem * N * 4.0 * (rem.splits + 1) / 3.0e6;
                 if (split < 0.97 * whole) {
-                    int rc = launch_rows_range<B_KINNER>(ch, al, Ad, Bm, ldb, Co, 0, m_main, K, N, epi, aux, P, st, dma_ok, nullptr, nullptr, carry);
+                    int rc = launch_rows_range<B_KINNER>(ch, al, Ad, Bm, ldb, Co, 0, m_main, K, N, epi, aux, P, st, dma_ok, nullptr, nullptr, carry, seg);
                     if (rc) return rc;
-                    return launch_rows_range<B_KINNER>(rem, al, Ad, Bm, ldb, Co, m_main, M, K, N, epi, aux, P, st, dma_ok);
+                    return launch_rows_range<B_KINNER>(rem, al, Ad, Bm, ldb, Co, m_main, M, K, N, epi, aux, P, st, dma_ok, nullptr, nullptr, nullptr, seg);
                 }
             }
         }
     }
-    return launch_rows_range<B_KINNER>(ch, al, Ad, Bm, ldb, Co, 0, M, K, N, epi, aux, P, st, dma_ok, nullptr, nullptr, carry);
+    return launch_rows_range<B_KINNER>(ch, al, Ad, Bm, ldb, Co, 0, M, K, N, epi, aux, P, st, dma_ok, nullptr, nullptr, carry, seg);
 }
 
 struct TnPlan {
@@ -996,11 +1002,36 @@
 }
 
 
+namespace {
+
+int nt_segments(const char* fn, int& epilogue, int K, int N, long ldb, KSegD& seg, long& ldb_min) {
+    const int Q = (epilogue >> 16) & 15, s = (epilogue >> 20) & 15;
+    ldb_min = K;
+    const int high = epilogue >> 24;
+    if ((epilogue >> 16) == 0) return LIDBOX_OK;
+    epilogue &= 0xffff;
+    if (high != 0 || Q < 1 || Q > 8 || s < 1 || s > 8 || K < 1 || K % Q != 0 || (K / Q) % SK_BK != 0) {
+        lidbox_set_error("%s: invalid argument: LIDBOX_EPI_SEGMENTS(Q, s) needs 1 <= Q, s <= 8 and K = Q segments of a multiple of %d", fn, SK_BK);
+        return LIDBOX_E_INVALID;
+    }
+    ldb_min = K / Q;
+    if (Q > 1) {
+        seg.steps = K / Q / SK_BK;
+        seg.stride = -(long)s * N * ldb;
+    }
+    return LIDBOX_OK;
+}
+
+}
+
 extern "C" int lidbox_gemm_nt(lidbox_rows_t A, const float* Bm, long ldb, lidbox_rows_out_t C, int K, int N,
                               int epilogue, const float* aux, void* workspace, size_t workspace_bytes,
                               lidbox_stream_t stream) {
-    if (validate_rows_call(__func__, A, Bm, ldb, C, K, N, epilogue, aux, K)) return LIDBOX_E_INVALID;
-    return launch_rows<true>(A, Bm, ldb, C, K, N, epilogue, aux, workspace, workspace_bytes, (hipStream_t)stream);
+    KSegD seg;
+    long ldb_min;
+    if (nt_segments(__func__, epilogue, K, N, ldb, seg, ldb_min)) return LIDBOX_E_INVALID;
+    if (validate_rows_call(__func__, A, Bm, ldb, C, K, N, epilogue, aux, ldb_min)) return LIDBOX_E_INVALID;
+    return launch_rows<true>(A, Bm, ldb, C, K, N, epilogue, aux, workspace, workspace_bytes, (hipStream_t)stream, nullptr, seg);
 }
 
 extern "C" size_t lidbox_gemm_tn_workspace(int M, int K1, int N) {
@@ -1155,7 +1186,10 @@
 extern "C" int lidbox_gemm_nt_carry(lidbox_rows_t A, const float* Bm, long ldb, lidbox_rows_out_t C, int K, int N, int epilogue,
                                     const float* aux, void* workspace, size_t workspace_bytes, const lidbox_reduce_job_t* jobs,
                                     int njobs, lidbox_stream_t stream) {
-    if (validate_rows_call(__func__, A, Bm, ldb, C, K, N, epilogue, aux, K)) return LIDBOX_E_INVALID;
+    KSegD seg;
+    long ldb_min;
+    if (nt_segments(__func__, epilogue, K, N, ldb, seg, ldb_min)) return LIDBOX_E_INVALID;
+    if (validate_rows_call(__func__, A, Bm, ldb, C, K, N, epilogue, aux, ldb_min)) return LIDBOX_E_INVALID;
     ReduceJob js[MAX_CARRY];
     const int m = jobs_in(jobs, njobs, js);
     LBX_ARG(m >= 0, "at most 2 non-empty jobs per call");
@@ -1164,7 +1198,7 @@
     Carry carry;
     carry.jobs = js;
     carry.njobs = (m > 0 && getenv("LIDBOX_GEMM_NO_CARRY") == nullptr) ? m : 0;
-    int rc = launch_rows<true>(A, Bm, ldb, C, K, N, epilogue, aux, workspace, workspace_bytes, (hipStream_t)stream, &carry);
+    int rc = launch_rows<true>(A, Bm, ldb, C, K, N, epilogue, aux, workspace, workspace_bytes, (hipStream_t)stream, &carry, seg);
     if (rc) return rc;
     g_last_carried = carry.carried ? m : 0;
     if (!carry.carried) return run_reduce_jobs(js, m, (hipStream_t)stream);
@@ -1203,6 +1237,7 @@
                                        const lidbox_reduce_job_t* jobs, int njobs, lidbox_reduce_job_t* job_out, lidbox_stream_t stream) {
     hipStream_t st = (hipStream_t)stream;
     if (job_out) memset(job_out, 0, sizeof *job_out);
+    LBX_ARG((epilogue >> 16) == 0, "LIDBOX_EPI_SEGMENTS is for lidbox_gemm_nt / lidbox_gemm_nt_carry");
     ReduceJob pend[MAX_CARRY];
     const int npend = jobs_in(jobs, njobs, pend);
     LBX_ARG(npend >= 0 && npend < MAX_CARRY, "at most 1 non-empty pending job per call");
diff --git a/lidbox_amd/csrc/gemm_dma.h b/lidbox_amd/csrc/gemm_dma.h
--- a/lidbox_amd/csrc/gemm_dma.h
+++ b/lidbox_amd/csrc/gemm_dma.h
@@ -127,7 +127,7 @@
 __device__ __forceinline__ void rows_dma_body(const RowsD& A, const float* __restrict__ Bm, long ldb, const RowsOutD& Cd, float* __restrict__ P,
                                               long m_beg, long M, int K, int N, int epi, const float* __restrict__ aux, int tiles_n,
                                               unsigned ntiles, int k_per_split, const DmaStream& sp, unsigned bx, unsigned by, int partial,
-                                              float* smem) {
+                                              float* smem, const KSegD& seg) {
     constexpr int MI = BM / 64, NJ = BN / 64;
     constexpr int A_ST = BM * SK_BK, B_ST = SK_BK * BN, ST = A_ST + B_ST;
     constexpr int PA = BM / 64, PB = BN / 64;
@@ -172,6 +172,7 @@
     }
     DmaInner<BN> obi;
     DmaOuter<BN> obo;
+    KSegWalk bseg;
     if (B_KINNER) {
         long roff[PB];
 #pragma unroll
@@ -180,7 +181,7 @@
             if (r >= N) r = n0;
             roff[i] = r * ldb;
         }
-        obi.init(Bm, roff, kbeg, lane, wn);
+        obi.init(bseg.start(Bm, seg, kbeg), roff, 0, lane, wn);
     } else {
         obo.init(Bm, ldb, n0, N, kbeg, lane, wv, wn);
     }
@@ -207,7 +208,7 @@
     };
     auto next = [&]() {
         oa.advance();
-        if (B_KINNER) obi.advance();
+        if (B_KINNER) bseg.advance(obi.sb);
         else obo.advance();
     };
     auto ra = [&](const float* st, int s2, float (&v)[MI][4]) { oa.template read<MI>(st, lane, s2, v); };
@@ -311,14 +312,14 @@
 template <int BM, int BN, bool B_KINNER>
 __global__ __launch_bounds__(256, (BM * BN >= 16384 ? 3 : (BM * BN >= 8192 ? 4 : 6))) void gemm_rows_dma_kernel(
     RowsD A, const float* __restrict__ Bm, long ldb, RowsOutD Cd, float* __restrict__ P, long m_beg, long M, int K, int N, int epi,
-    const float* __restrict__ aux, int tiles_n, unsigned ntiles, int k_per_split, DmaStream sp, ReduceJobs rj) {
+    const float* __restrict__ aux, int tiles_n, unsigned ntiles, int k_per_split, DmaStream sp, ReduceJobs rj, KSegD seg) {
     __shared__ __attribute__((aligned(16))) float smem[DMA_STAGES * dma_stage_floats<BM, BN>()];
     if (blockIdx.x < rj.total) {
         if (blockIdx.y == 0) reduce_jobs_run(rj, blockIdx.x);
         return;
     }
     rows_dma_body<BM, BN, B_KINNER>(A, Bm, ldb, Cd, P, m_beg, M, K, N, epi, aux, tiles_n, ntiles, k_per_split, sp, blockIdx.x - rj.total,
-                                    blockIdx.y, gridDim.y > 1 ? 1 : 0, smem);
+                                    blockIdx.y, gridDim.y > 1 ? 1 : 0, smem, seg);
 }
 
 template <int COLS>
@@ -515,7 +516,7 @@
     const unsigned bx = blockIdx.x - rj.total, nb = gridDim.x - rj.total;
     if (bx < rows_blocks) {
         rows_dma_body<64, 64, true>(r.A, r.Bm, r.ldb, r.Cd, r.P, 0, r.M, r.K, r.N, r.epi, r.aux, r.tiles_n, r.ntiles, r.k_per_split, r.sp,
-                                    bx % r.nx, bx / r.nx, r.partial, smem);
+                                    bx % r.nx, bx / r.nx, r.partial, smem, KSegD{});
     } else {
         tn_dma_body<64, 64>(t.A, t.Bd, t.P, t.Pc, t.M, t.K1, t.N, t.tiles_n, t.ntiles, t.rows_per_split, bx - rows_blocks, nb - rows_blocks, smem);
     }
diff --git a/lidbox_amd/csrc/gemm_dma8.h b/lidbox_amd/csrc/gemm_dma8.h
--- a/lidbox_amd/csrc/gemm_dma8.h
+++ b/lidbox_amd/csrc/gemm_dma8.h
@@ -104,7 +104,7 @@
 __global__ __launch_bounds__(512, BN == 64 ? 8 : 4) void gemm_rows_dma8_kernel(RowsD A, const float* __restrict__ Bm, long ldb, RowsOutD Cd,
                                                                               float* __restrict__ P, long m_beg, long M, int K, int N, int epi,
                                                                               const float* __restrict__ aux, int tiles_n, unsigned ntiles,
-                                                                              int k_per_split, DmaStream sp, ReduceJobs rj) {
+                                                                              int k_per_split, DmaStream sp, ReduceJobs rj, KSegD seg) {
     constexpr int BM = 128, NJ = BN / 64;
     constexpr int A_ST = BM * SK_BK, B_ST = SK_BK * BN, ST = A_ST + B_ST;
     __shared__ __attribute__((aligned(16))) float smem[DMA_STAGES * ST];
@@ -148,10 +148,11 @@
     }
     DmaInner8<BN> obi;
     DmaOuter8<BN> obo;
+    KSegWalk bseg;
     if (B_KINNER) {
         long r = n0 + 16 * (wv % (BN / 16)) + (lane >> 2);
         if (r >= N) r = n0;
-        obi.init(Bm, r * ldb, kbeg, lane, wv, wn, 32 * NJ);
+        obi.init(bseg.start(Bm, seg, kbeg), r * ldb, 0, lane, wv, wn, 32 * NJ);
     } else {
         obo.init(Bm, ldb, n0, N, kbeg, lane, wv, wn);
     }
@@ -173,7 +174,7 @@
         if (B_KINNER) { if (tail) obi.issue_tail(d, ktail, lane); else obi.issue(d); }
         else { if (tail) obo.issue_tail(d, ktail, lane); else obo.issue(d); }
     };
-    auto adv_b = [&]() { if (B_KINNER) obi.advance(); else obo.advance(); };
+    auto adv_b = [&]() { if (B_KINNER) bseg.advance(obi.sb); else obo.advance(); };
     auto rb = [&](const float* stg, int s2, float (&v)[NJ][4]) {
         if (B_KINNER) obi.template read<NJ>(stg, lane, s2, v);
         else obo.template read<NJ>(stg, lane, s2, v);
diff --git a/lidbox_amd/csrc/gemm_sk.h b/lidbox_amd/csrc/gemm_sk.h
--- a/lidbox_amd/csrc/gemm_sk.h
+++ b/lidbox_amd/csrc/gemm_sk.h
@@ -48,6 +48,27 @@
             const f32x4_t x = *reinterpret_cast<const f32x4_t*>(st + rd + b * 32 * 16 + slot * 4);
             v[b][0] = x[0]; v[b][1] = x[1]; v[b][2] = x[2]; v[b][3] = x[3];
         }
+    }
+};
+
+struct KSegD {
+    int steps = 0x7fffffff;
+    long stride = 0;
+};
+struct KSegWalk {
+    int left, steps;
+    long jump;
+    __device__ __forceinline__ const float* start(const float* base, const KSegD& sg, int k0) {
+        const int s = __builtin_amdgcn_readfirstlane(k0 / SK_BK);
+        const int q = s / sg.steps, r = s - q * sg.steps;
+        steps = sg.steps;
+        left = sg.steps - r;
+        jump = sg.stride - (long)sg.steps * SK_BK;
+        return base + (long)q * sg.stride + r * SK_BK;
+    }
+    __device__ __forceinline__ void advance(const float*& sb) {
+        sb += SK_BK;
+        if (--left == 0) { sb += jump; left = steps; }
     }
 };
 
@@ -277,7 +298,7 @@
 __global__ __launch_bounds__(256, SK_WGCU) void gemm_sk_rows_kernel(RowsD A, const float* __restrict__ Bm, long ldb, RowsOutD Cd,
                                                                     long M, int K, int N, int epi, const float* __restrict__ aux,
                                                                     SkPlan pl, unsigned epoch, unsigned* __restrict__ counters,
-                                                                    float* __restrict__ slabs) {
+                                                                    float* __restrict__ slabs, KSegD seg) {
     extern __shared__ __attribute__((aligned(16))) float sk_smem[];
     const int tid = threadIdx.x, lane = tid & 63;
     const int wv = __builtin_amdgcn_readfirstlane(tid >> 6);
@@ -306,6 +327,7 @@
         }
         SkInner obi;
         SkOuter obo;
+        KSegWalk bseg;
         if (B_KINNER) {
             long roff[2];
 #pragma unroll
@@ -314,7 +336,7 @@
                 if (r >= N) r = n0;
                 roff[i] = r * ldb;
             }
-            obi.init(Bm, roff, kb * SK_BK, lane, wn);
+            obi.init(bseg.start(Bm, seg, kb * SK_BK), roff, 0, lane, wn);
         } else {
             obo.init(Bm, ldb, n0, N, kb * SK_BK, lane, wv, wn);
         }
@@ -339,7 +361,7 @@
         };
         auto next = [&]() {
             oa.advance();
-            if (B_KINNER) obi.advance();
+            if (B_KINNER) bseg.advance(obi.sb);
             else obo.advance();
         };
         auto ra = [&](const float* st, int s2, float (&v)[2][4]) { oa.read(st, lane, s2, v); };
@@ -558,7 +580,7 @@
 __global__ __launch_bounds__(256, SKP_WGCU) void gemm_skp_rows_kernel(RowsD A, const float* __restrict__ Bm, long ldb, RowsOutD Cd,
                                                                       long M, int K, int N, int epi, const float* __restrict__ aux,
                                                                       SkPlan pl, unsigned epoch, unsigned* __restrict__ counters,
-                                                                      float* __restrict__ slabs, float* __restrict__ dummy) {
+                                                                      float* __restrict__ slabs, float* __restrict__ dummy, KSegD seg) {
     extern __shared__ __attribute__((aligned(16))) float sk_smem[];
     const int tid = threadIdx.x, lane = tid & 63;
     const int wv = __builtin_amdgcn_readfirstlane(tid >> 6);
@@ -678,6 +700,7 @@
         }
         SkInner obi;
         SkOuter obo;
+        KSegWalk bseg;
         if (B_KINNER) {
             long roff[2];
 #pragma unroll
@@ -686,7 +709,7 @@
                 if (r >= N) r = n0;
                 roff[i] = r * ldb;
             }
-            obi.init(Bm, roff, kb * SK_BK, lane, wn);
+            obi.init(bseg.start(Bm, seg, kb * SK_BK), roff, 0, lane, wn);
         } else {
             obo.init(Bm, ldb, n0, N, kb * SK_BK, lane, wv, wn);
         }
@@ -711,7 +734,7 @@
         };
         auto next = [&]() {
             oa.advance();
-            if (B_KINNER) obi.advance();
+            if (B_KINNER) bseg.advance(obi.sb);
             else obo.advance();
         };
         auto ra = [&](const float* st, int s2, float (&v)[2][4]) { oa.read(st, lane, s2, v); };
diff --git a/lidbox_amd/csrc/gemm_tuned.h b/lidbox_amd/csrc/gemm_tuned.h
--- a/lidbox_amd/csrc/gemm_tuned.h
+++ b/lidbox_amd/csrc/gemm_tuned.h
@@ -10,15 +10,14 @@
 
 const TunedGemm TUNED_GEMM[] = {
     {1, 8448, 512, 1500, 128, 64, 1, 0, 8},
-    {1, 25344, 1024, 512, 64, 128, 1, 1, 4},
     {1, 25344, 1000, 500, 128, 64, 1, 0, 8},
     {0, 50688, 512, 200, 64, 64, 1, 0, 4},
-    {1, 25344, 512, 512, 64, 64, 1, 1, 4},
+    {1, 25344, 512, 1024, 128, 128, 1, 0, 8},
+    {1, 25344, 512, 512, 128, 64, 1, 0, 8},
     {0, 8448, 512, 1536, 64, 64, 1, 1, 4},
     {1, 8448, 1536, 512, 64, 128, 1, 1, 4},
     {2, 8448, 512, 512, 64, 64, 24, 0, 4},
     {0, 8448, 1500, 512, 64, 64, 1, 1, 4},
-    {1, 50688, 1024, 512, 64, 64, 1, 1, 4},
     {0, 16896, 512, 1536, 64, 64, 1, 1, 4},
     {1, 16896, 1536, 512, 64, 128, 1, 1, 4},
     {1, 512, 3000, 512, 64, 64, 1, 1, 4},
@@ -27,7 +26,6 @@
     {0, 25344, 512, 200, 64, 64, 1, 1, 4},
     {2, 25344, 512, 200, 64, 64, 48, 0, 4},
     {0, 12672, 512, 1536, 64, 64, 1, 0, 4},
-    {1, 12672, 1024, 512, 64, 64, 1, 0, 4},
     {0, 4224, 512, 1536, 64, 64, 1, 0, 4},
     {2, 4224, 512, 512, 64, 64, 16, 0, 4},
     {1, 4224, 512, 1500, 64, 64, 1, 0, 4},
@@ -41,7 +39,6 @@
     {2, 2112, 1500, 512, 64, 64, 8, 0, 4},
     {0, 202752, 512, 200, 64, 128, 1, 0, 4},
     {0, 101376, 512, 1536, 128, 128, 1, 1, 4},
-    {1, 101376, 1024, 512, 64, 128, 1, 0, 4},
     {0, 33792, 512, 1536, 64, 128, 1, 1, 4},
     {1, 33792, 1536, 512, 128, 128, 1, 0, 4},
     {0, 33792, 512, 512, 64, 64, 1, 0, 4},
diff --git a/lidbox_amd/models/tdnn.py b/lidbox_amd/models/tdnn.py
--- a/lidbox_amd/models/tdnn.py
+++ b/lidbox_amd/models/tdnn.py
@@ -112,9 +112,9 @@
         self.rpads.append(0)
         chans = [model.input_dim] + [c.filters for c in convs]
         self.trail = [0] * len(chans)
-        if model.bf16_storage:
-            for i in range(1, len(convs) - 1):
-                self.trail[i + 1] = model._dgrad_trail(i, self.Ts[i])
+        dense_last = model.bf16_storage or model.attention is not None
+        for i in range(1, len(convs) - (1 if dense_last else 0)):
+            self.trail[i + 1] = model._dgrad_trail(i, self.Ts[i])
         self.act = [torch.zeros((B, self.pads[i] + self.Ts[i] + self.rpads[i] + self.trail[i], chans[i]), **f32) for i in range(len(chans))]
         self.dact = [None] + [torch.zeros_like(a) for a in self.act[1:]]
         self.act16 = [None] * len(self.act)
@@ -375,9 +375,15 @@
                 res.append((rho, Q, u_min, u_max))
         return res
 
+    def _dgrad_os_fp32_ok(self, i):
+        c = self.convs[i]
+        return (self.gemm.name == "float32" and not self.bf16_storage and i > 0 and c.d == 1 and c.k > c.s
+                and c.filters % nv.GEMM_K_STEP == 0)
+
     def _dgrad_trail(self, i, T):
         c = self.convs[i]
-        if not (c.d == 1 and c.k > c.s and self.shadow_dgrad_ok(i)) or T <= 0:
+        ok = self.shadow_dgrad_ok(i) if self.bf16_storage else self._dgrad_os_fp32_ok(i)
+        if not (c.d == 1 and c.k > c.s and ok) or T <= 0:
             return 0
         To = conv_out_len(T, c.s)
         return max(0, max(u_max for _, _, _, u_max in self._dgrad_residues(i, T)) - (To - 1))
@@ -592,7 +598,8 @@
                                           nv.ptr(ws.gemm_ws), ws.gemm_ws.numel(), st))
             cin = c.filters
         last = ws.act[-1]
-        T, C = last.shape[1], last.shape[2]
+        T, C = ws.Ts[-1], last.shape[2]
+        Tp = last.shape[1]
         att = self.attention
         if att is not None and ws.B * T > 0:
             n = ws.B * T
@@ -609,7 +616,7 @@
             nv.check(lib.lidbox_stats_pool_fwd_bf16(nv.ptr(ws.last16), ws.B, T, C, T * C16, C16, nv.ptr(ws.pooled), st))
         else:
             fn = lib.lidbox_stats_pool_fwd if self.pool == "stats" else lib.lidbox_avg_pool_fwd
-            nv.check(fn(nv.ptr(last), ws.B, T, C, T * C, C, nv.ptr(ws.pooled), st))
+            nv.check(fn(nv.ptr(last), ws.B, T, C, Tp * C, C, nv.ptr(ws.pooled), st))
         x, din = ws.pooled, ws.pooled.shape[1]
         for j, d in enumerate(self.denses):
             if stop_before_output and j == len(self.denses) - 1:
@@ -722,7 +729,8 @@
         att = self.attention
         last = ws.act[-1] if att is None else ws.hw
         dlast = ws.dact[-1] if att is None else ws.d_hw
-        T, C = last.shape[1], last.shape[2]
+        T, C = ws.Ts[-1], last.shape[2]
+        Tp = last.shape[1]
         relu_last = 1 if self.convs[-1].relu else 0
         pool_mask = relu_last if att is None else 0
         d16 = ws.dact16[-1] if att is None else None
@@ -732,15 +740,15 @@
                                                     pool_mask, nv.ptr(d16), T * d16.shape[2], d16.shape[2], st))
             ws.d16_fresh.add(len(self.convs))
         elif self.pool == "stats" and d16 is not None and B * T > 0:
-            nv.check(lib.lidbox_stats_pool_bwd_shadow(nv.ptr(last), nv.ptr(ws.pooled), nv.ptr(ws.dpooled), B, T, C, T * C, C,
+            nv.check(lib.lidbox_stats_pool_bwd_shadow(nv.ptr(last), nv.ptr(ws.pooled), nv.ptr(ws.dpooled), B, T, C, Tp * C, C,
                                                       pool_mask, None if self.bf16_only else nv.ptr(dlast), nv.ptr(d16),
                                                       T * d16.shape[2], d16.shape[2], st))
             ws.d16_fresh.add(len(self.convs))
         elif self.pool == "stats":
-            nv.check(lib.lidbox_stats_pool_bwd(nv.ptr(last), nv.ptr(ws.pooled), nv.ptr(ws.dpooled), B, T, C, T * C, C,
+            nv.check(lib.lidbox_stats_pool_bwd(nv.ptr(last), nv.ptr(ws.pooled), nv.ptr(ws.dpooled), B, T, C, Tp * C, C,
                                                pool_mask, nv.ptr(dlast), st))
         else:
-            nv.check(lib.lidbox_avg_pool_bwd(nv.ptr(last), nv.ptr(ws.dpooled), B, T, C, T * C, C, pool_mask,
+            nv.check(lib.lidbox_avg_pool_bwd(nv.ptr(last), nv.ptr(ws.dpooled), B, T, C, Tp * C, C, pool_mask,
                                              nv.ptr(dlast), st))
         if att is None or B * T == 0:
             return
@@ -844,6 +852,29 @@
             if d16 is not None:
                 ws.d16_fresh.add(i)
             return
+        Wp = self._p(c.name + ".W").value
+        if (self._dgrad_os_fp32_ok(i) and ws.trail[i + 1] >= self._dgrad_trail(i, ws.Ts[i]) and Wp % 16 == 0
+                and 4 * ws.dact[i + 1].numel() < 2 ** 31 * 1.8 and os.environ.get("LIDBOX_GEMM_DMA", "1") != "0"):
+            if pair_wgrad:
+                r = self._tn_region(ws)
+                job, tws = nv.ReduceJob(), ws.tn_regions[r]
+                nv.check(lib.lidbox_gemm_tn_partial(A_rows, dy, self._p(c.name + ".W", True), c.filters, K, c.filters, 0,
+                                                    self._p(c.name + ".b", True), nv.ptr(tws), tws.numel(), ctypes.byref(job), st))
+                if job.nblocks:
+                    ws.pending.append((job, r))
+            dnext, Co = ws.dact[i + 1], c.filters
+            for rho, Q, u_min, u_max in self._dgrad_residues(i, ws.Ts[i]):
+                nu, p0 = u_max - u_min + 1, u_min * c.s + rho
+                A = _rows(dnext.data_ptr() + 4 * (ws.pads[i + 1] + u_min - Q + 1) * Co, dnext.shape[1] * Co, Co, B, nu)
+                Cd = _rows(dprev.data_ptr() + 4 * p0 * cin, Tp * cin, c.s * cin, B, nu)
+                epi, mask = nv.EPI_NONE, None
+                if relu_prev:
+                    epi, mask = nv.EPI_RELU_MASK, ctypes.c_void_p(aprev.data_ptr() + 4 * p0 * cin)
+                Wb = ctypes.c_void_p(Wp + 4 * (rho + (Q - 1) * c.s) * cin * Co)
+                jobs, nj = self._take_jobs(ws, 2)
+                nv.check(lib.lidbox_gemm_nt_carry(A, Wb, Co, Cd, Q * Co, cin, epi | nv.EPI_SEGMENTS(Q, c.s), mask, gws, gws_n,
+                                                  jobs, nj, st))
+            return
         if use16 and (ngroups > 1 or "fused" not in self.wd16[i]) and c.filters % 8 != 0:
             use16, d16 = False, None
         if ngroups > 1 and To * c.s < Tp:
@@ -892,6 +923,8 @@
                                   A_rows, self._p(c.name + ".W", True), c.filters, K, self._p(c.name + ".b", True))
             else:
                 nv.check(self.gemm.nt(dy, Wg, c.filters, Cd, c.filters, ntaps * cin, epi, mask, gws, gws_n, st))
+        if i > 0 and not relu_prev and ws.pads[i] > 0:
+            nv.check(lib.lidbox_zero_2d(nv.ptr(dprev), 4 * Tp * cin, 4 * ws.pads[i] * cin, B, st))
         if i == 0:
             self._backward_frontend(ws)
 
```
